# mmacklin/tinsel

Hardware: AMD Instinct MI355X
Metric: Msamples/s (cornell.tin 1024x1024 maxDepth=4 spp=2126, wavefront path; Mrays/s alongside) (higher is better)
Workload: dtype f32; 1 GPU; cornell.tin 1024x1024 maxDepth=4, 1 pass(es) per step, pipeline=auto; scene_pack=tests/golden/cornell.pack, parallelism=1 GPU

## Files before the change

include/tinsel_hip.h:

```cpp
#ifndef TINSEL_HIP_H
#define TINSEL_HIP_H

#include <stddef.h>
#include <stdint.h>

#ifdef __cplusplus
extern "C" {
#endif


typedef struct tinsel_vec3 { float x, y, z; } tinsel_vec3;
typedef struct tinsel_vec4 { float x, y, z, w; } tinsel_vec4;

typedef struct tinsel_transform {
    tinsel_vec3 p;
    tinsel_vec4 r;
    float s;
} tinsel_transform;

typedef struct tinsel_bvh_node {
    tinsel_vec3 lower;
    tinsel_vec3 upper;
    uint32_t left_index;
    uint32_t right_index_leaf;
} tinsel_bvh_node;

typedef struct tinsel_camera {
    tinsel_vec3 position;
    tinsel_vec4 rotation;
    float fov;
    float shutter_start;
    float shutter_end;
} tinsel_camera;

typedef struct tinsel_texture {
    float* data;
    int32_t width, height, depth;
    int32_t _pad;
} tinsel_texture;

typedef struct tinsel_material {
    tinsel_vec3 emission;
    tinsel_vec3 color;
    tinsel_vec3 absorption;
    float eta;
    float metallic;
    float subsurface;
    float specular;
    float roughness;
    float specular_tint;
    float anisotropic;
    float sheen;
    float sheen_tint;
    float clearcoat;
    float clearcoat_gloss;
    float transmission;
    int32_t _pad0;
    tinsel_texture bump_map;
    float bump;
    tinsel_vec3 bump_tile;
} tinsel_material;

enum { TINSEL_GEOM_SPHERE = 0, TINSEL_GEOM_PLANE = 1, TINSEL_GEOM_MESH = 2 };

typedef struct tinsel_mesh_geometry {
    const tinsel_vec3* positions;
    const tinsel_vec3* normals;
    const int32_t* indices;
    const tinsel_bvh_node* nodes;
    const float* cdf;
    int32_t num_vertices;
    int32_t num_indices;
    int32_t num_nodes;
    float area;
    uint64_t id;
} tinsel_mesh_geometry;

typedef struct tinsel_primitive {
    tinsel_transform start_transform;
    tinsel_transform end_transform;
    int32_t type;
    int32_t _pad0;
    union {
        struct { float radius; } sphere;
        struct { float plane[4]; } plane;
        tinsel_mesh_geometry mesh;
    } geo;
    tinsel_material material;
    int32_t light_samples;
    int32_t _pad1;
} tinsel_primitive;

enum { TINSEL_FILTER_BOX = 0, TINSEL_FILTER_GAUSSIAN = 1 };

typedef struct tinsel_filter {
    int32_t type;
    float width;
    float falloff;
    float offset;
} tinsel_filter;

enum { TINSEL_MODE_NORMALS = 0, TINSEL_MODE_COMPLEXITY = 1, TINSEL_MODE_PATHTRACE = 2 };

typedef struct tinsel_options {
    int32_t mode;
    int32_t width;
    int32_t height;
    tinsel_filter filter;
    float exposure;
    float limit;
    float clamp;
    int32_t max_depth;
    int32_t max_samples;
} tinsel_options;

typedef struct tinsel_scene_desc {
    const tinsel_primitive* primitives;
    int32_t num_primitives;
    int32_t num_bvh_nodes;
    const tinsel_bvh_node* bvh_nodes;
    tinsel_vec3 sky_horizon;
    tinsel_vec3 sky_zenith;
    int32_t probe_valid;
    int32_t probe_width;
    int32_t probe_height;
    int32_t _pad;
    const tinsel_vec4* probe_data;
    const float* probe_pdf_x;
    const float* probe_cdf_x;
    const float* probe_pdf_y;
    const float* probe_cdf_y;
} tinsel_scene_desc;


typedef struct tinsel_hip tinsel_hip;

enum { TINSEL_PIPELINE_WAVEFRONT = 0, TINSEL_PIPELINE_MEGAKERNEL = 1, TINSEL_PIPELINE_WAVEFRONT_SPLIT = 2,
       TINSEL_PIPELINE_WAVEFRONT_PAIRED = 4,
       TINSEL_PIPELINE_AUTO = 3 };

tinsel_hip* tinsel_hip_create(const tinsel_scene_desc* scene, int device_index);

typedef struct tinsel_hip_tuning {
    uint32_t struct_bytes;
    int32_t flat_scan;
    int32_t lds_scene;
    int32_t walk;
    int32_t inline_max_tris;
    int32_t walk_min_tris;
    int64_t small_mesh_bytes;
    int64_t arena_lds_limit;
    int64_t batch_paths;
    int32_t grid_mult;
    int32_t bounce_share;
    int32_t repack;
    int32_t tail_split;
    float tail_share;
    int32_t tail_divide;
    int32_t shade_sorted;
    int32_t overlap;
    int32_t scene_walk;
    int32_t swalk_lds;
    int32_t accumulate;
    int32_t walk_block;
    int32_t walk_single;
    int32_t walk_lds_stack;
    int32_t walk_refill_min;
    int32_t walk_leaf_min;
    int32_t walk_grid_mult;
    int32_t quads_in_scan;
    int32_t bounce_fit;
} tinsel_hip_tuning;
enum { TINSEL_ACCUMULATE_AUTO = 0, TINSEL_ACCUMULATE_TILED = 1, TINSEL_ACCUMULATE_WIDE = 2, TINSEL_ACCUMULATE_PIPED = 3, TINSEL_ACCUMULATE_FULL_WINDOW = 4 };

void tinsel_hip_tuning_init(tinsel_hip_tuning* t);
tinsel_hip* tinsel_hip_create_tuned(const tinsel_scene_desc* scene, int device_index, const tinsel_hip_tuning* tuning);
int tinsel_hip_set_tuning(tinsel_hip* r, const tinsel_hip_tuning* tuning);
int tinsel_hip_get_tuning(tinsel_hip* r, tinsel_hip_tuning* out);

void tinsel_hip_destroy(tinsel_hip* r);

int tinsel_hip_init(tinsel_hip* r, int width, int height);

int tinsel_hip_init_external(tinsel_hip* r, int width, int height, float* device_accum);

int tinsel_hip_render(tinsel_hip* r, const tinsel_camera* camera, const tinsel_options* options,
                      float* out_rgba, int passes);

enum { TINSEL_LOOKAHEAD_OFF = 0, TINSEL_LOOKAHEAD_ON = 1, TINSEL_LOOKAHEAD_PIN_OUTPUT = 2 };
int tinsel_hip_set_lookahead(tinsel_hip* r, int enable);

int tinsel_hip_render_async(tinsel_hip* r, const tinsel_camera* camera, const tinsel_options* options,
                            int passes, void* stream);

float* tinsel_hip_accum_device_ptr(tinsel_hip* r);

int tinsel_hip_read_accum(tinsel_hip* r, float* out_rgba);

enum { TINSEL_BVH_REFERENCE = 0, TINSEL_BVH_LBVH = 1, TINSEL_BVH_PLOC = 2 };
int tinsel_hip_set_mesh_bvh(tinsel_hip* r, int mode, double* build_ms);

int tinsel_hip_refit_mesh(tinsel_hip* r, int primitive, const float* positions_xyz, int num_vertices, const float* normals_xyz);

enum { TINSEL_SCENE_BVH_NODES = 0, TINSEL_SCENE_BVH_DEVICE = 1 };
int tinsel_hip_set_primitive_transform(tinsel_hip* r, int index, const tinsel_transform* start, const tinsel_transform* end);
int tinsel_hip_rebuild_scene(tinsel_hip* r, int mode, const tinsel_bvh_node* nodes, int num_nodes, double* build_ms);

enum { TINSEL_PROBE_CDF = 0, TINSEL_PROBE_ALIAS = 1 };
int tinsel_hip_set_probe_sampling(tinsel_hip* r, int mode);

int tinsel_hip_set_russian_roulette(tinsel_hip* r, int start_bounce);

int tinsel_hip_write_accum(tinsel_hip* r, const float* rgba, uint32_t next_pass_index);

int tinsel_hip_present(tinsel_hip* r, const tinsel_options* options, int nlm_width, float nlm_falloff, float* out_rgba);
int tinsel_hip_present_async(tinsel_hip* r, const tinsel_options* options, int nlm_width, float nlm_falloff, void* stream);
const float* tinsel_hip_present_device_ptr(tinsel_hip* r);

int tinsel_image_quantize_rgb8(const float* rgba, int width, int height, unsigned char* rgb);

int tinsel_hip_set_shard(tinsel_hip* r, int rank, int world, int tile);

int tinsel_hip_set_pipeline(tinsel_hip* r, int pipeline);

enum { TINSEL_ARITH_EXACT = 0, TINSEL_ARITH_FAST = 1 };
int tinsel_hip_set_arithmetic(tinsel_hip* r, int mode);
int tinsel_hip_get_arithmetic(tinsel_hip* r);

int tinsel_hip_set_pass_index(tinsel_hip* r, uint32_t pass_index);
uint32_t tinsel_hip_get_pass_index(tinsel_hip* r);

void tinsel_hip_stats(tinsel_hip* r, unsigned long long* rays, unsigned long long* samples,
                      double* gpu_seconds);
void tinsel_hip_reset_stats(tinsel_hip* r);

typedef struct tinsel_kernel_time {
    char name[32];
    uint32_t launches;
    float total_ms;
    float busy_ms;
} tinsel_kernel_time;
int tinsel_hip_kernel_times(tinsel_hip* r, tinsel_kernel_time* out, int max_entries);
int tinsel_hip_kernel_time_bytes(void);
int tinsel_hip_enable_kernel_timing(tinsel_hip* r, int enable);

int tinsel_hip_stats_detail(tinsel_hip* r, unsigned long long* out8);
int tinsel_hip_set_detail_counters(tinsel_hip* r, int enable);

int tinsel_hip_render_cost(tinsel_hip* r, const tinsel_camera* camera, const tinsel_options* options,
                           uint32_t pass_begin, int passes, uint32_t* out_host);

#define TINSEL_FEATURE_ALBEDO 1u
#define TINSEL_FEATURE_NORMAL 2u
#define TINSEL_FEATURE_DEPTH  4u

int tinsel_hip_render_features(tinsel_hip* r, const tinsel_camera* camera, const tinsel_options* options,
                               uint32_t pass_begin, int passes, unsigned features, float* out_host);
int tinsel_hip_render_features_device(tinsel_hip* r, const tinsel_camera* camera, const tinsel_options* options,
                                      uint32_t pass_begin, int passes, unsigned features, float* out_dev, void* stream);

#define TINSEL_ID_MISS   (-1)
#define TINSEL_ID_EMPTY  (-2)
#define TINSEL_ID_MAX_SLOTS 8

int tinsel_hip_render_id_mattes(tinsel_hip* r, const tinsel_camera* camera, const tinsel_options* options,
                                uint32_t pass_begin, int passes, int slots, int32_t* out_ids_host, float* out_weights_host);
int tinsel_hip_render_id_mattes_device(tinsel_hip* r, const tinsel_camera* camera, const tinsel_options* options,
                                       uint32_t pass_begin, int passes, int slots, int32_t* out_ids_dev, float* out_weights_dev, void* stream);

#define TINSEL_MAX_LIGHT_GROUPS 8

int tinsel_hip_render_light_groups(tinsel_hip* r, const tinsel_camera* camera, const tinsel_options* options,
                                   uint32_t pass_begin, int passes, int num_groups, const int32_t* group_of_primitive, int env_group,
                                   float* out_host);
int tinsel_hip_render_light_groups_device(tinsel_hip* r, const tinsel_camera* camera, const tinsel_options* options,
                                          uint32_t pass_begin, int passes, int num_groups, const int32_t* group_of_primitive, int env_group,
                                          float* out_dev, void* stream);

typedef struct tinsel_hip_denoise_params {
    int radius;
    int patch_radius;
    float k_color, k_albedo, k_normal, k_depth;
    int demodulate;
    float albedo_floor;
} tinsel_hip_denoise_params;

void tinsel_hip_denoise_params_init(tinsel_hip_denoise_params* p);

int tinsel_hip_denoise(tinsel_hip* r, const float* beauty_host, const float* planes_host,
                       unsigned features, int width, int height,
                       const tinsel_hip_denoise_params* p, float* out_host);
int tinsel_hip_denoise_device(tinsel_hip* r, const float* beauty_dev, const float* planes_dev,
                              unsigned features, int width, int height,
                              const tinsel_hip_denoise_params* p, float* out_dev, void* stream);

int tinsel_hip_present_image_device(tinsel_hip* r, const float* image_dev,
                                    const tinsel_options* options, int nlm_width,
                                    float nlm_falloff, void* stream);

typedef struct tinsel_ray     { float ox, oy, oz, time;  float dx, dy, dz, tmax; } tinsel_ray;
typedef struct tinsel_ray_hit { float t; int32_t primitive; float nx, ny, nz; uint32_t reserved[3]; } tinsel_ray_hit;

#define TINSEL_QUERY_CLOSEST  0
#define TINSEL_QUERY_OCCLUDED 1

int tinsel_hip_trace_rays(tinsel_hip* r, int mode, long long n, const tinsel_ray* rays_host, void* out_host);
int tinsel_hip_trace_rays_device(tinsel_hip* r, int mode, long long n, const tinsel_ray* rays_dev, void* out_dev, void* stream);
int tinsel_hip_trace_camera(tinsel_hip* r, const tinsel_camera* camera, int width, int height, float time, tinsel_ray_hit* out_host);

typedef struct tinsel_path_start { float ox, oy, oz, time;  float dx, dy, dz, reserved0;  uint32_t rng1, rng2, reserved1, reserved2; } tinsel_path_start;

int tinsel_hip_trace_radiance(tinsel_hip* r, long long n, const tinsel_path_start* starts_host, int max_depth, float* out_rgbx_host);
int tinsel_hip_trace_radiance_device(tinsel_hip* r, long long n, const tinsel_path_start* starts_dev, int max_depth, float* out_rgbx_dev, void* stream);

typedef struct tinsel_gather_point { float px, py, pz, time;  float nx, ny, nz;  uint32_t seed; } tinsel_gather_point;

#define TINSEL_GATHER_COSINE 0
#define TINSEL_GATHER_SPHERE 1

int tinsel_hip_gather_radiance(tinsel_hip* r, int mode, long long n, const tinsel_gather_point* points_host, int samples, int max_depth,
                               float* out_rgbx_host, tinsel_path_start* starts_out_host );
int tinsel_hip_gather_radiance_device(tinsel_hip* r, int mode, long long n, const tinsel_gather_point* points_dev, int samples, int max_depth,
                                      float* out_rgbx_dev, tinsel_path_start* starts_out_dev , void* stream);

#define TINSEL_GATHER_SH_MAX_ORDER 2

int tinsel_hip_gather_sh(tinsel_hip* r, int mode, int order, long long n, const tinsel_gather_point* points_host,
                         int samples, int max_depth, float* out_host, tinsel_path_start* starts_out_host );
int tinsel_hip_gather_sh_device(tinsel_hip* r, int mode, int order, long long n, const tinsel_gather_point* points_dev,
                                int samples, int max_depth, float* out_dev, tinsel_path_start* starts_out_dev , void* stream);

int tinsel_hip_reserve(tinsel_hip* r, int passes, int max_depth);

int tinsel_hip_set_batch_paths(tinsel_hip* r, unsigned long long max_paths);

long long tinsel_hip_read_batch_radiance(tinsel_hip* r, float* out_rgbx, unsigned long long max_paths);

int tinsel_hip_leaf(tinsel_hip* r, int op, int index, int n, const float* in, int in_stride, const uint32_t* seeds,
                    float* out, int out_stride, const tinsel_camera* camera, int width, int height);

int tinsel_hip_mesh_tree(tinsel_hip* r, int primitive, void* out_nodes, int capacity, int* out_meta);

int tinsel_hip_stack_entries(tinsel_hip* r);
int tinsel_hip_nee_per_path(tinsel_hip* r);
int tinsel_hip_walked_prims(tinsel_hip* r);
int tinsel_hip_walk_tops(tinsel_hip* r, int* out_counts, int capacity);
int tinsel_hip_queue_counts(tinsel_hip* r, uint32_t* out, int max_bounces);
int tinsel_hip_bounce_plan(tinsel_hip* r, uint32_t* out2);
unsigned int tinsel_hip_scene_features(const tinsel_scene_desc* scene);
int tinsel_hip_scene_slim(const tinsel_scene_desc* scene);
enum { TINSEL_BOUNCE_MEDIA = 1, TINSEL_BOUNCE_PROBE = 2, TINSEL_BOUNCE_MOTION = 4, TINSEL_BOUNCE_MESH_WALK = 8, TINSEL_BOUNCE_SPHERE = 16,
       TINSEL_BOUNCE_TRANSMISSION = 32, TINSEL_BOUNCE_POOLS = 64, TINSEL_BOUNCE_SHARE = 128, TINSEL_BOUNCE_SORT = 256, TINSEL_BOUNCE_ROULETTE = 512 };

const char* tinsel_hip_last_error(void);


typedef struct tinsel_hip_group tinsel_hip_group;

tinsel_hip_group* tinsel_hip_group_create(const tinsel_scene_desc* scene, int num_gpus, int tile);
tinsel_hip_group* tinsel_hip_group_create_tuned(const tinsel_scene_desc* scene, int num_gpus, int tile, const tinsel_hip_tuning* tuning);
void tinsel_hip_group_destroy(tinsel_hip_group* g);
int tinsel_hip_group_init(tinsel_hip_group* g, int width, int height);
int tinsel_hip_group_render(tinsel_hip_group* g, const tinsel_camera* camera, const tinsel_options* options, float* out_rgba, int passes);
int tinsel_hip_group_set_lookahead(tinsel_hip_group* g, int enable);
int tinsel_hip_group_present(tinsel_hip_group* g, const tinsel_options* options, int nlm_width, float nlm_falloff, float* out_rgba);
int tinsel_hip_group_size(tinsel_hip_group* g);
tinsel_hip* tinsel_hip_group_member(tinsel_hip_group* g, int rank);

#define TINSEL_HIP_COMM_ID_BYTES 128
int tinsel_hip_comm_unique_id(unsigned char* id_bytes, int capacity);
int tinsel_hip_comm_init(tinsel_hip* r, const unsigned char* id_bytes, int rank, int world);
int tinsel_hip_comm_size(tinsel_hip* r);
int tinsel_hip_comm_reduce_accum(tinsel_hip* r, float* out_device, int root, void* stream);

int tinsel_hip_plan_regions(unsigned long long slots, int num_cus, int nee_per_path, int fused, unsigned int* out);

int tinsel_hip_selftest_arith(int device_index, int op, int variant, unsigned long long* out_counts, unsigned int* out_first_bad);
int tinsel_hip_selftest_sort(int device_index, unsigned long long* keys, unsigned long long n, int begin_bit, int end_bit);
int tinsel_hip_selftest_scan(int device_index, const int* in, int* out, unsigned long long n);
int tinsel_hip_accumulate_support(int filter_type, float filter_width, float filter_falloff, float filter_offset, float* out_arg_zero);
int tinsel_hip_selftest_accumulate(int device_index, int width, int height, int filter_type, float filter_width, float filter_falloff, float filter_offset,
                                   float clamp, const unsigned int* pass_seeds, int passes, const float* radiance, float* accum, int choice, int form,
                                   int* out_form);

int tinsel_hip_ubench(int device_index, int kind, unsigned long long bytes, int steps, double* out_ms, double* out_units);


#define TINSEL_PACK_MAGIC "TINPACK1"

typedef struct tinsel_pack_header {
    char magic[8];
    uint32_t version;
    uint32_t num_primitives;
    uint32_t num_bvh_nodes;
    uint32_t num_meshes;
    uint64_t total_bytes;
    uint64_t off_primitives;
    uint64_t off_bvh_nodes;
    uint64_t off_probe_data;
    uint64_t off_probe_pdf_x;
    uint64_t off_probe_cdf_x;
    uint64_t off_probe_pdf_y;
    uint64_t off_probe_cdf_y;
    int32_t probe_width;
    int32_t probe_height;
    tinsel_vec3 sky_horizon;
    tinsel_vec3 sky_zenith;
    tinsel_camera camera;
    tinsel_options options;
    uint8_t _reserved[48];
} tinsel_pack_header;

int tinsel_pack_open(void* blob, size_t size, tinsel_scene_desc* out_scene,
                     tinsel_camera* out_camera, tinsel_options* out_options);

#ifdef __cplusplus
}

static_assert(sizeof(tinsel_vec3) == 12, "Vec3");
static_assert(sizeof(tinsel_transform) == 32, "Transform");
static_assert(sizeof(tinsel_bvh_node) == 32, "BVHNode");
static_assert(sizeof(tinsel_camera) == 40, "Camera");
static_assert(sizeof(tinsel_texture) == 24, "Texture");
static_assert(sizeof(tinsel_material) == 128, "Material");
static_assert(offsetof(tinsel_material, eta) == 36, "Material.eta");
static_assert(offsetof(tinsel_material, transmission) == 80, "Material.transmission");
static_assert(offsetof(tinsel_material, bump_map) == 88, "Material.bumpMap");
static_assert(offsetof(tinsel_material, bump) == 112, "Material.bump");
static_assert(sizeof(tinsel_mesh_geometry) == 64, "MeshGeometry");
static_assert(offsetof(tinsel_mesh_geometry, num_vertices) == 40, "MeshGeometry.numVertices");
static_assert(offsetof(tinsel_mesh_geometry, area) == 52, "MeshGeometry.area");
static_assert(offsetof(tinsel_mesh_geometry, id) == 56, "MeshGeometry.id");
static_assert(sizeof(tinsel_primitive) == 272, "Primitive");
static_assert(offsetof(tinsel_primitive, type) == 64, "Primitive.type");
static_assert(offsetof(tinsel_primitive, geo) == 72, "Primitive.geo");
static_assert(offsetof(tinsel_primitive, material) == 136, "Primitive.material");
static_assert(offsetof(tinsel_primitive, light_samples) == 264, "Primitive.lightSamples");
static_assert(sizeof(tinsel_filter) == 16, "Filter");
static_assert(sizeof(tinsel_options) == 48, "Options");
static_assert(offsetof(tinsel_options, max_depth) == 40, "Options.maxDepth");
static_assert(sizeof(tinsel_pack_header) == 256, "pack header");
static_assert(sizeof(tinsel_hip_tuning) == 128, "tuning");
static_assert(sizeof(tinsel_ray) == 32, "ray");
static_assert(sizeof(tinsel_ray_hit) == 32, "ray hit");
static_assert(sizeof(tinsel_path_start) == 48, "path start");
static_assert(sizeof(tinsel_gather_point) == 32, "gather point");
#endif

#endif
```

tinsel_amd/abi.py:

```python
import ctypes as C


class Vec3(C.Structure):
    _fields_ = [("x", C.c_float), ("y", C.c_float), ("z", C.c_float)]

    def __iter__(self):
        return iter((self.x, self.y, self.z))


class Vec4(C.Structure):
    _fields_ = [("x", C.c_float), ("y", C.c_float), ("z", C.c_float), ("w", C.c_float)]

    def __iter__(self):
        return iter((self.x, self.y, self.z, self.w))


class Transform(C.Structure):
    _fields_ = [("p", Vec3), ("r", Vec4), ("s", C.c_float)]


class BVHNode(C.Structure):
    _fields_ = [("lower", Vec3), ("upper", Vec3), ("left_index", C.c_uint32), ("right_index_leaf", C.c_uint32)]


# ... 3 lines not shown


LEAF_BIT = 0x80000000
MESH_TREE_META = ("root", "numInternal", "numTris", "stackNeed", "topCount", "twoLeaves", "inArena")


class Camera(C.Structure):
    _fields_ = [("position", Vec3), ("rotation", Vec4), ("fov", C.c_float),
                ("shutter_start", C.c_float), ("shutter_end", C.c_float)]


class Texture(C.Structure):
    _fields_ = [("data", C.c_void_p), ("width", C.c_int32), ("height", C.c_int32),
                ("depth", C.c_int32), ("_pad", C.c_int32)]


class Material(C.Structure):
    _fields_ = [("emission", Vec3), ("color", Vec3), ("absorption", Vec3),
                ("eta", C.c_float), ("metallic", C.c_float), ("subsurface", C.c_float),
                ("specular", C.c_float), ("roughness", C.c_float), ("specular_tint", C.c_float),
                ("anisotropic", C.c_float), ("sheen", C.c_float), ("sheen_tint", C.c_float),
                ("clearcoat", C.c_float), ("clearcoat_gloss", C.c_float), ("transmission", C.c_float),
                ("_pad0", C.c_int32), ("bump_map", Texture), ("bump", C.c_float), ("bump_tile", Vec3)]


class MeshGeometry(C.Structure):
    _fields_ = [("positions", C.c_void_p), ("normals", C.c_void_p), ("indices", C.c_void_p),
                ("nodes", C.c_void_p), ("cdf", C.c_void_p),
                ("num_vertices", C.c_int32), ("num_indices", C.c_int32), ("num_nodes", C.c_int32),
                ("area", C.c_float), ("id", C.c_uint64)]


class _Sphere(C.Structure):
    _fields_ = [("radius", C.c_float)]


class _Plane(C.Structure):
    _fields_ = [("plane", C.c_float * 4)]


class _Geo(C.Union):
    _fields_ = [("sphere", _Sphere), ("plane", _Plane), ("mesh", MeshGeometry)]


class Primitive(C.Structure):
    _fields_ = [("start_transform", Transform), ("end_transform", Transform),
                ("type", C.c_int32), ("_pad0", C.c_int32), ("geo", _Geo),
                ("material", Material), ("light_samples", C.c_int32), ("_pad1", C.c_int32)]


class Filter(C.Structure):
    _fields_ = [("type", C.c_int32), ("width", C.c_float), ("falloff", C.c_float), ("offset", C.c_float)]


class Options(C.Structure):
    _fields_ = [("mode", C.c_int32), ("width", C.c_int32), ("height", C.c_int32), ("filter", Filter),
                ("exposure", C.c_float), ("limit", C.c_float), ("clamp", C.c_float),
                ("max_depth", C.c_int32), ("max_samples", C.c_int32)]

    def copy(self):
        o = Options()
        C.memmove(C.byref(o), C.byref(self), C.sizeof(Options))
        return o


class SceneDesc(C.Structure):
    _fields_ = [("primitives", C.c_void_p), ("num_primitives", C.c_int32), ("num_bvh_nodes", C.c_int32),
                ("bvh_nodes", C.c_void_p), ("sky_horizon", Vec3), ("sky_zenith", Vec3),
                ("probe_valid", C.c_int32), ("probe_width", C.c_int32), ("probe_height", C.c_int32),
                ("_pad", C.c_int32), ("probe_data", C.c_void_p), ("probe_pdf_x", C.c_void_p),
                ("probe_cdf_x", C.c_void_p), ("probe_pdf_y", C.c_void_p), ("probe_cdf_y", C.c_void_p)]


class PackHeader(C.Structure):
    _fields_ = [("magic", C.c_char * 8), ("version", C.c_uint32), ("num_primitives", C.c_uint32),
                ("num_bvh_nodes", C.c_uint32), ("num_meshes", C.c_uint32), ("total_bytes", C.c_uint64),
                ("off_primitives", C.c_uint64), ("off_bvh_nodes", C.c_uint64), ("off_probe_data", C.c_uint64),
                ("off_probe_pdf_x", C.c_uint64), ("off_probe_cdf_x", C.c_uint64),
                ("off_probe_pdf_y", C.c_uint64), ("off_probe_cdf_y", C.c_uint64),
                ("probe_width", C.c_int32), ("probe_height", C.c_int32),
                ("sky_horizon", Vec3), ("sky_zenith", Vec3), ("camera", Camera), ("options", Options),
                ("_reserved", C.c_uint8 * 48)]


class KernelTime(C.Structure):
    _fields_ = [("name", C.c_char * 32), ("launches", C.c_uint32), ("total_ms", C.c_float), ("busy_ms", C.c_float)]


class Ray(C.Structure):
    _fields_ = [("ox", C.c_float), ("oy", C.c_float), ("oz", C.c_float), ("time", C.c_float),
                ("dx", C.c_float), ("dy", C.c_float), ("dz", C.c_float), ("tmax", C.c_float)]


class RayHit(C.Structure):
    _fields_ = [("t", C.c_float), ("primitive", C.c_int32), ("nx", C.c_float), ("ny", C.c_float), ("nz", C.c_float),
                ("reserved", C.c_uint32 * 3)]


RAY_DTYPE = [("ox", "<f4"), ("oy", "<f4"), ("oz", "<f4"), ("time", "<f4"), ("dx", "<f4"), ("dy", "<f4"), ("dz", "<f4"), ("tmax", "<f4")]
RAY_HIT_DTYPE = [("t", "<f4"), ("primitive", "<i4"), ("nx", "<f4"), ("ny", "<f4"), ("nz", "<f4"), ("reserved", "<u4", (3,))]
QUERY_CLOSEST, QUERY_OCCLUDED = 0, 1


class PathStart(C.Structure):
    _fields_ = [("ox", C.c_float), ("oy", C.c_float), ("oz", C.c_float), ("time", C.c_float),
                ("dx", C.c_float), ("dy", C.c_float), ("dz", C.c_float), ("reserved0", C.c_float),
                ("rng1", C.c_uint32), ("rng2", C.c_uint32), ("reserved1", C.c_uint32), ("reserved2", C.c_uint32)]


PATH_START_DTYPE = [("ox", "<f4"), ("oy", "<f4"), ("oz", "<f4"), ("time", "<f4"), ("dx", "<f4"), ("dy", "<f4"), ("dz", "<f4"), ("reserved0", "<f4"),
                    ("rng1", "<u4"), ("rng2", "<u4"), ("reserved1", "<u4"), ("reserved2", "<u4")]


class GatherPoint(C.Structure):
    _fields_ = [("px", C.c_float), ("py", C.c_float), ("pz", C.c_float), ("time", C.c_float),
                ("nx", C.c_float), ("ny", C.c_float), ("nz", C.c_float), ("seed", C.c_uint32)]


GATHER_POINT_DTYPE = [("px", "<f4"), ("py", "<f4"), ("pz", "<f4"), ("time", "<f4"), ("nx", "<f4"), ("ny", "<f4"), ("nz", "<f4"), ("seed", "<u4")]
GATHER_COSINE, GATHER_SPHERE = 0, 1
GATHER_SH_MAX_ORDER = 2
FEATURE_ALBEDO, FEATURE_NORMAL, FEATURE_DEPTH = 1, 2, 4
FEATURE_NAMES = ("albedo", "normal", "depth")
ID_MISS, ID_EMPTY, ID_MAX_SLOTS = -1, -2, 8
MAX_LIGHT_GROUPS = 8


class DenoiseParams(C.Structure):
    _fields_ = [("radius", C.c_int32), ("patch_radius", C.c_int32),
                ("k_color", C.c_float), ("k_albedo", C.c_float), ("k_normal", C.c_float), ("k_depth", C.c_float),
                ("demodulate", C.c_int32), ("albedo_floor", C.c_float)]

    def as_dict(self):
        return {k: getattr(self, k) for k, _ in self._fields_}


class KernelTimeV1(C.Structure):
    _fields_ = [("name", C.c_char * 32), ("launches", C.c_uint32), ("total_ms", C.c_float)]


BOUNCE_GENERAL, BOUNCE_COUNT, BOUNCE_FIT_CLOSED, BOUNCE_FIT_DEFERRED = 0, 1, 2, 3
BOUNCE_MEDIA, BOUNCE_PROBE, BOUNCE_MOTION, BOUNCE_MESH_WALK, BOUNCE_SPHERE = 1, 2, 4, 8, 16
BOUNCE_TRANSMISSION, BOUNCE_POOLS, BOUNCE_SHARE, BOUNCE_SORT, BOUNCE_ROULETTE = 32, 64, 128, 256, 512


class Tuning(C.Structure):
    _fields_ = [("struct_bytes", C.c_uint32),
                ("flat_scan", C.c_int32), ("lds_scene", C.c_int32), ("walk", C.c_int32), ("inline_max_tris", C.c_int32), ("walk_min_tris", C.c_int32),
                ("small_mesh_bytes", C.c_int64), ("arena_lds_limit", C.c_int64),
                ("batch_paths", C.c_int64), ("grid_mult", C.c_int32), ("bounce_share", C.c_int32), ("repack", C.c_int32),
                ("tail_split", C.c_int32), ("tail_share", C.c_float), ("tail_divide", C.c_int32),
                ("shade_sorted", C.c_int32), ("overlap", C.c_int32), ("scene_walk", C.c_int32), ("swalk_lds", C.c_int32), ("accumulate", C.c_int32),
                ("walk_block", C.c_int32), ("walk_single", C.c_int32), ("walk_lds_stack", C.c_int32), ("walk_refill_min", C.c_int32), ("walk_leaf_min", C.c_int32),
                ("walk_grid_mult", C.c_int32), ("quads_in_scan", C.c_int32), ("bounce_fit", C.c_int32)]
    CREATE_FIELDS = ("flat_scan", "lds_scene", "walk", "inline_max_tris", "walk_min_tris", "small_mesh_bytes", "arena_lds_limit")
    _DEFAULTS = dict(flat_scan=-1, lds_scene=-1, walk=-1, inline_max_tris=-1, walk_min_tris=-1, small_mesh_bytes=-1, arena_lds_limit=-1,
                     batch_paths=0, grid_mult=0, bounce_share=-1, repack=-1, tail_split=-1, tail_share=0.0, tail_divide=4,
                     shade_sorted=-1, overlap=-1, scene_walk=-1, swalk_lds=-1, accumulate=0,
                     walk_block=0, walk_single=-1, walk_lds_stack=-1, walk_refill_min=0, walk_leaf_min=0, walk_grid_mult=0, quads_in_scan=-1, bounce_fit=-1)

    def __init__(self, **over):
        super().__init__()
        self.struct_bytes = C.sizeof(Tuning)
        for k, v in self._DEFAULTS.items():
            setattr(self, k, v)
        for k, v in over.items():
            if k not in self._DEFAULTS:
                raise TypeError("tinsel_hip_tuning has no field %r" % k)
            setattr(self, k, v)

    def replace(self, **over):
        t = Tuning(**{k: getattr(self, k) for k in self._DEFAULTS})
        for k, v in over.items():
            if k not in self._DEFAULTS:
                raise TypeError("tinsel_hip_tuning has no field %r" % k)
            setattr(t, k, v)
        return t

    def as_dict(self):
        return {k: getattr(self, k) for k in self._DEFAULTS}


ACCUMULATE_AUTO, ACCUMULATE_TILED, ACCUMULATE_WIDE, ACCUMULATE_PIPED, ACCUMULATE_FULL_WINDOW = 0, 1, 2, 3, 4
ACCUMULATE_FORM_AUTO, ACCUMULATE_FORM_FULL_WINDOW, ACCUMULATE_FORM_SUPPORT = 0, 1, 2
ACCUMULATE_RAN_UNTILED, ACCUMULATE_RAN_TILED, ACCUMULATE_RAN_WIDE, ACCUMULATE_RAN_PIPED, ACCUMULATE_RAN_SUPPORT_TILED, ACCUMULATE_RAN_SUPPORT_WIDE = 0, 1, 2, 3, 4, 5
SELFTEST_ACCUMULATE_ARGTYPES = [C.c_int, C.c_int, C.c_int, C.c_int, C.c_float, C.c_float, C.c_float, C.c_float, C.c_void_p, C.c_int, C.c_void_p, C.c_void_p,
                                C.c_int, C.c_int, C.POINTER(C.c_int)]


def accumulate_arg_zero(offset):
    import math
    import numpy as np
    z = math.log(float(np.float32(offset))) - 1e-6
    f = np.float32(z)
    if float(f) > z:
        f = np.nextafter(f, np.float32(-np.inf))
    return f


def accumulate_takes_support_form(filter_type, width, falloff, offset):
    import numpy as np
    width, falloff, offset = np.float32(width), np.float32(falloff), np.float32(offset)
    if filter_type == FILTER_BOX or not (offset > 0 and np.isfinite(offset)) or not (falloff > 0 and np.isfinite(falloff)) or not (0 < width <= 1):
        return False
    return bool(-falloff <= accumulate_arg_zero(offset))
COMM_ID_BYTES = 128
MODE_NORMALS, MODE_COMPLEXITY, MODE_PATHTRACE = 0, 1, 2
BVH_REFERENCE, BVH_LBVH, BVH_PLOC = 0, 1, 2
SCENE_BVH_NODES, SCENE_BVH_DEVICE = 0, 1
ARITH_EXACT, ARITH_FAST = 0, 1
PROBE_CDF, PROBE_ALIAS = 0, 1
LOOKAHEAD_OFF, LOOKAHEAD_ON, LOOKAHEAD_PIN_OUTPUT = 0, 1, 2
FILTER_BOX, FILTER_GAUSSIAN = 0, 1
GEOM_SPHERE, GEOM_PLANE, GEOM_MESH = 0, 1, 2
PIPELINE_WAVEFRONT, PIPELINE_MEGAKERNEL, PIPELINE_WAVEFRONT_SPLIT, PIPELINE_AUTO, PIPELINE_WAVEFRONT_PAIRED = 0, 1, 2, 3, 4

assert C.sizeof(Transform) == 32 and C.sizeof(BVHNode) == 32 and C.sizeof(Camera) == 40 and C.sizeof(Node64) == 64
assert C.sizeof(Material) == 128 and C.sizeof(MeshGeometry) == 64 and C.sizeof(Primitive) == 272
assert C.sizeof(Filter) == 16 and C.sizeof(Options) == 48 and C.sizeof(PackHeader) == 256
assert C.sizeof(Ray) == 32 and C.sizeof(RayHit) == 32 and C.sizeof(DenoiseParams) == 32
assert Primitive.geo.offset == 72 and Primitive.material.offset == 136 and Primitive.light_samples.offset == 264
```

tinsel_amd/csrc/tn_host_api.h:

```cpp
#pragma once

extern "C" {

int tinsel_hip_init(tinsel_hip* r, int width, int height)
{
    if (r)
        lookahead_release(r);
    if (!r || width <= 0 || height <= 0)
        return fail("init: bad arguments");
    HIP_TRY(hipSetDevice(r->device));
    HIP_TRY(hipDeviceSynchronize());
    r->accum = nullptr;
    if (r->accumOwn.alloc((size_t)width*height))
        return -1;
    r->accum = r->accumOwn.get();
    HIP_TRY(hipMemset(r->accum, 0, sizeof(float4)*(size_t)width*height));
    HIP_TRY(hipStreamSynchronize(nullptr));
    r->width = width;
    r->height = height;
    return 0;
}

int tinsel_hip_init_external(tinsel_hip* r, int width, int height, float* device_accum)
{
// ... 563 lines not shown
    return 0;
}

void tinsel_hip_stats(tinsel_hip* r, unsigned long long* rays, unsigned long long* samples, double* gpu_seconds)
{
    unsigned long long s[8] = { 0 };
    if (r && r->statsDev)
        (void)read_stats(r, s);
    if (rays) *rays = s[0];
    if (samples) *samples = s[1];
    if (gpu_seconds) *gpu_seconds = r ? r->gpuSeconds : 0.0;
}

int tinsel_hip_stats_detail(tinsel_hip* r, unsigned long long* out8)
{
    if (!r || !out8)
        return fail("stats_detail: bad arguments");
    return read_stats(r, out8);
}

int tinsel_hip_set_detail_counters(tinsel_hip* r, int enable)
{
    lookahead_cancel(r);
    if (!r)
        return fail("set_detail_counters: null");
    r->countDetail = enable != 0;
    return 0;
}

void tinsel_hip_reset_stats(tinsel_hip* r)
{
    lookahead_cancel(r);
    if (!r)
        return;
    (void)hipSetDevice(r->device);
    (void)hipDeviceSynchronize();
    (void)hipMemset(r->statsDev.get(), 0, sizeof(unsigned long long)*kStatShards*kStatWords);
    (void)hipStreamSynchronize(nullptr);
    r->gpuSeconds = 0.0;
}

int tinsel_hip_enable_kernel_timing(tinsel_hip* r, int enable)
{
    lookahead_cancel(r);
    if (!r)
        return fail("enable_kernel_timing: null");
    r->timing = enable != 0;
    return 0;
}

int tinsel_hip_kernel_time_bytes(void) { return (int)sizeof(tinsel_kernel_time); }

int tinsel_hip_kernel_times(tinsel_hip* r, tinsel_kernel_time* out, int max_entries)
{
    lookahead_cancel(r);
    if (!r || !out)
        return fail("kernel_times: bad arguments");
    HIP_TRY(hipSetDevice(r->device));
    HIP_TRY(hipDeviceSynchronize());
    float total[KN_COUNT] = { 0 };
    uint32_t launches[KN_COUNT] = { 0 };
    std::vector<std::pair<float, float>> intervals[KN_COUNT];
    for (const TimedSpan& s : r->spans)
    {
        float ms = 0.0f, at = 0.0f;
        if (hipEventElapsedTime(&ms, s.start, s.stop) == hipSuccess)
        {
            total[s.kernel] += ms;
            launches[s.kernel]++;
            if (hipEventElapsedTime(&at, r->spans.front().start, s.start) == hipSuccess)
                intervals[s.kernel].push_back(std::make_pair(at, at + ms));
        }
    }
    float busy[KN_COUNT] = { 0 };
    for (int k = 0; k < KN_COUNT; ++k)
    {
        std::sort(intervals[k].begin(), intervals[k].end());
        float end = -1e30f;
        for (const auto& iv : intervals[k])
        {
            if (iv.second > end)
                busy[k] += iv.second - std::max(iv.first, end);
            end = std::max(end, iv.second);
        }
        if (intervals[k].size() != launches[k])
            busy[k] = total[k];
    }
    int n = 0;
    double sum = 0.0;
    for (int k = 0; k < KN_COUNT && n < max_entries; ++k)
    {
        if (!launches[k])
            continue;
        memset(&out[n], 0, sizeof(out[n]));
        strncpy(out[n].name, kKernelNames[k], sizeof(out[n].name) - 1);
        out[n].launches = launches[k];
        out[n].total_ms = total[k];
        out[n].busy_ms = busy[k];
        sum += total[k];
        ++n;
    }
    r->gpuSeconds += sum*1e-3;
    return n;
}

int tinsel_hip_reserve(tinsel_hip* r, int passes, int max_depth)
{
    lookahead_cancel(r);
    if (!r || !r->accum || passes < 1 || max_depth < 1)
        return fail("reserve: bad arguments (Init first)");
    HIP_TRY(hipSetDevice(r->device));
    const size_t perPass = slots_per_pass(r, r->width, r->height);
    return ensure_batch(r, plan_batch(r, perPass, passes_per_batch(batch_slots(r), perPass, passes),  false), max_depth);
}

int tinsel_hip_set_batch_paths(tinsel_hip* r, unsigned long long max_paths)
{
    lookahead_cancel(r);
    if (!r || max_paths < 1024)
        return fail("set_batch_paths: bad arguments");
    r->maxBatchSlots = (size_t)max_paths;
    r->batchSlotsExplicit = true;
    r->tune.batch_paths = (int64_t)max_paths;
    return 0;
}

int tinsel_hip_set_tuning(tinsel_hip* r, const tinsel_hip_tuning* tuning)
{
    if (!r || !tuning)
        return fail("set_tuning: null argument");
    lookahead_cancel(r);
    tinsel_hip_tuning t = tuning_from_caller(tuning);
    if (t.grid_mult < 0 || t.grid_mult > 256 || (t.walk_block != 0 && t.walk_block != 256 && t.walk_block != 1024) ||
        t.accumulate < TINSEL_ACCUMULATE_AUTO || t.accumulate > TINSEL_ACCUMULATE_FULL_WINDOW || t.walk_refill_min > 64 || t.walk_leaf_min > 64 || t.walk_grid_mult < 0 || t.walk_grid_mult > 64 ||
        (t.tail_split > 0 && (!(t.tail_share >= 0.0f) || t.tail_divide < 1)) || (t.batch_paths != 0 && t.batch_paths < 1024))
        return fail("set_tuning: a field is out of range");
    HIP_TRY(hipSetDevice(r->device));
    HIP_TRY(hipDeviceSynchronize());
    const tinsel_hip_tuning was = r->tune;
    t.flat_scan = was.flat_scan; t.lds_scene = was.lds_scene; t.walk = was.walk; t.inline_max_tris = was.inline_max_tris;
    t.walk_min_tris = was.walk_min_tris; t.small_mesh_bytes = was.small_mesh_bytes; t.arena_lds_limit = was.arena_lds_limit;
    r->tune = t;
    if (t.batch_paths > 0)
    {
        r->maxBatchSlots = (size_t)t.batch_paths;
        r->batchSlotsExplicit = true;
    }
    else
    {
        r->maxBatchSlots = 8u << 20;
        r->batchSlotsExplicit = false;
    }
    free_batch(r);
    return 0;
}

int tinsel_hip_get_tuning(tinsel_hip* r, tinsel_hip_tuning* out)
{
    if (!r || !out)
        return fail("get_tuning: null argument");
    *out = r->tune;
    return 0;
}

long long tinsel_hip_read_batch_radiance(tinsel_hip* r, float* out_rgbx, unsigned long long max_paths)
{
    lookahead_cancel(r);
    if (!r || !out_rgbx)
        return fail("read_batch_radiance: bad arguments");
    HIP_TRY(hipSetDevice(r->device));
    HIP_TRY(hipDeviceSynchronize());
    const size_t n = std::min<size_t>((size_t)max_paths, r->lastBatchSlots);
    if (n)
        HIP_TRY(hipMemcpy(out_rgbx, r->ps.rad, sizeof(float4)*n, hipMemcpyDeviceToHost));
    return (long long)n;
}

int tinsel_hip_leaf(tinsel_hip* r, int op, int index, int n, const float* in, int in_stride, const uint32_t* seeds,
                    float* out, int out_stride, const tinsel_camera* camera, int width, int height)
{
    lookahead_cancel(r);
    if (!r || n <= 0 || !out || out_stride <= 0 || op < 0 || op > kLeafDisplay)
        return fail("leaf: bad arguments");
    if ((op == kLeafBsdfEval || op == kLeafBsdfSample || op == kLeafPrimIntersect || op == kLeafPrimSample) &&
        (index < 0 || index >= r->scene.numPrims))
        return fail("leaf: primitive index out of range");
    HIP_TRY(hipSetDevice(r->device));
    DevBuf<float> dIn, dOut;
    DevBuf<uint32_t> dSeeds;
    CameraParams cam;
    memset(&cam, 0, sizeof(cam));
    if (camera && width > 0 && height > 0)
        make_camera(*camera, width, height, cam);
    if (in && in_stride > 0 && dIn.upload(in, (size_t)n*in_stride))
        return fail("leaf: input upload failed");
    if (seeds && dSeeds.upload(seeds, (size_t)n))
        return fail("leaf: seed upload failed");
    if (dOut.alloc((size_t)n*out_stride))
        return fail("leaf: output allocation failed");
    hipLaunchKernelGGL(k_leaf, dim3((n + kBlock - 1)/kBlock), dim3(kBlock), stack_bytes(r), nullptr, r->scene, op, index, n, dIn.get(), in_stride,
                       dSeeds.get(), dOut.get(), out_stride, cam, r->stackNeed);
    if (hipDeviceSynchronize() != hipSuccess || hipGetLastError() != hipSuccess)
        return fail("leaf: kernel failed");
    if (hipMemcpy(out, dOut.get(), sizeof(float)*(size_t)n*out_stride, hipMemcpyDeviceToHost) != hipSuccess)
        return fail("leaf: download failed");
    return 0;
}

int tinsel_hip_stack_entries(tinsel_hip* r) { return r ? r->stackNeed : 0; }

int tinsel_hip_mesh_tree(tinsel_hip* r, int primitive, void* out_nodes, int capacity, int* out_meta)
{
    lookahead_cancel(r);
    if (!r || !out_meta || capacity < 0 || primitive < 0 || primitive >= r->scene.numPrims || r->primMesh[(size_t)primitive] < 0)
        return fail("mesh_tree: bad arguments (a mesh primitive and a meta array of 7 ints)");
    const DevMesh& dm = r->meshesNow[(size_t)r->primMesh[(size_t)primitive]];
    const int meta[7] = { (int)dm.root, dm.numInternal, dm.numTris, dm.stackNeed, dm.topCount, dm.twoLeaves, dm.inArena };
    memcpy(out_meta, meta, sizeof(meta));
    if (!out_nodes)
        return dm.numInternal;
    if (capacity < dm.numInternal)
        return fail("mesh_tree: capacity is smaller than the tree's node count");
    const unsigned char* src = dm.inArena ? r->scene.arena + dm.offNodes : reinterpret_cast<const unsigned char*>(dm.nodes);
    HIP_TRY(hipSetDevice(r->device));
    HIP_TRY(hipDeviceSynchronize());
    if (dm.numInternal > 0)
        HIP_TRY(hipMemcpy(out_nodes, src, sizeof(Node64)*(size_t)dm.numInternal, hipMemcpyDeviceToHost));
    return dm.numInternal;
}
int tinsel_hip_walked_prims(tinsel_hip* r) { return (r && r->walkEnabled) ? r->walkPrims.count : 0; }
int tinsel_hip_nee_per_path(tinsel_hip* r) { return r ? r->neePerPath : 0; }

int tinsel_hip_walk_tops(tinsel_hip* r, int* out_counts, int capacity)
{
    if (!r || !out_counts || capacity < 0)
        return fail("walk_tops: bad arguments");
    const int n = r->walkEnabled ? r->walkPrims.count : 0;
    if (capacity < n)
        return fail("walk_tops: capacity is smaller than the number of walked primitives");
    const WalkPlan w = plan_walk(r);
    for (int k = 0; k < n; ++k)
        out_counts[k] = w.job.topCount[k];
    return n;
}

unsigned int tinsel_hip_scene_features(const tinsel_scene_desc* scene)
{
    if (!scene || !scene->primitives)
        return 0u;
    uint32_t f = scene->probe_valid ? kFeatProbe : 0u;
    for (int i = 0; i < scene->num_primitives; ++i)
    {
        const tinsel_primitive& p = scene->primitives[i];
        const tinsel_material& m = p.material;
        f |= (m.absorption.x != 0.0f || m.absorption.y != 0.0f || m.absorption.z != 0.0f) ? kFeatMedia : 0u;
        f |= m.transmission != 0.0f ? kFeatTransmission : 0u;
        f |= memcmp(&p.start_transform, &p.end_transform, sizeof(tinsel_transform)) != 0 ? kFeatMotion : 0u;
        f |= p.type == TINSEL_GEOM_SPHERE ? kFeatSphere : 0u;
        if (p.type == TINSEL_GEOM_MESH)
        {
            const tinsel_bvh_node* n = p.geo.mesh.nodes;
            const bool twoLeaves = n && p.geo.mesh.num_nodes == 3 && !ref_is_leaf(n[0]) && n[0].left_index < 3u && ref_right(n[0]) < 3u &&
                                   ref_is_leaf(n[n[0].left_index]) && ref_is_leaf(n[ref_right(n[0])]);
            f |= twoLeaves ? 0u : kFeatMeshWalk;
        }
    }
    return f;
}

int tinsel_hip_scene_slim(const tinsel_scene_desc* scene)
{
    if (!scene || !scene->primitives)
        return 0;
    bool anySubsurface = false;
    for (int i = 0; i < scene->num_primitives; ++i)
        anySubsurface = anySubsurface || !is_plus_zero(scene->primitives[i].material.subsurface);
    return scene_slim(tinsel_hip_scene_features(scene), anySubsurface) ? 1 : 0;
}

int tinsel_hip_bounce_plan(tinsel_hip* r, uint32_t* out2)
{
    if (!r || !out2)
        return fail("bounce_plan: bad arguments");
    if (r->lastBounceKind < 0)
        return fail("bounce_plan: the fused kernel has not run yet");
    out2[0] = (uint32_t)r->lastBounceKind;
    out2[1] = r->lastBounceFeatures;
    return 0;
}

int tinsel_hip_queue_counts(tinsel_hip* r, uint32_t* out, int max_bounces)
{
    if (!r || !out || max_bounces < 1)
        return fail("queue_counts: bad arguments");
    if (r->batchPipeline < 0 || r->batchDepth < 1)
        return fail("queue_counts: nothing rendered yet");
    HIP_TRY(hipSetDevice(r->device));
    HIP_TRY(hipDeviceSynchronize());
    const int n = std::min(max_bounces, std::min(r->batchDepth, r->lastFp.maxDepth));
    if (r->lastPipeline == TINSEL_PIPELINE_MEGAKERNEL || r->batchPipeline != r->lastPipeline)
        return fail("queue_counts: the last batch did not run a wavefront pipeline");
    const tinsel_hip::DenseLane& lane = r->lane[r->lastLane];
    const bool split = r->lastPipeline == TINSEL_PIPELINE_WAVEFRONT_SPLIT && r->neePerPath > 0;
    const size_t W = lane.regions;
    std::vector<uint32_t> seg(W*(size_t)n*4, 0u);
    uint32_t* const src[4] = { lane.ss.segFront, lane.ss.segBack, lane.ss.neeFront, lane.ss.neeBack };
    for (int a = 0; a < (split ? 4 : 2); ++a)
        HIP_TRY(hipMemcpy(seg.data() + (size_t)a*W*n, src[a], W*(size_t)n*sizeof(uint32_t), hipMemcpyDeviceToHost));
    for (int b = 0; b < n; ++b)
    {
        unsigned long long live = 0, nee = 0;
        for (size_t g = 0; g < W; ++g)
        {
            live += seg[(size_t)b*W + g] + seg[W*n + (size_t)b*W + g];
            nee += seg[2*W*n + (size_t)b*W + g] + seg[3*W*n + (size_t)b*W + g];
        }
        out[b] = (b == 0 && r->lastPipeline == TINSEL_PIPELINE_WAVEFRONT) ? lane.paths : (uint32_t)live;
        out[max_bounces + b] = (uint32_t)nee;
    }
    return n;
}


int tinsel_hip_plan_regions(unsigned long long slots, int num_cus, int nee_per_path, int fused, unsigned int* out)
{
    if (!out || slots == 0 || slots >= 0xffffffffull || num_cus < 1 || num_cus > 4096)
        return fail("plan_regions: bad arguments");
    RegionSpec s = region_spec(tuning_defaults(), num_cus, nee_per_path, fused != 0, kBounceWaves);
    s.capacity = (size_t)slots + s.maxRegions*kWave;
    RegionCut c;
    const int rc = cut_regions(s, (size_t)slots, streaming_grid(s, (size_t)slots), c) ? 0 : fail("render: path buffers too small for this batch");
    out[0] = c.numRegions; out[1] = c.regionLen; out[2] = c.bigRegions; out[3] = c.shortLen;
    out[4] = (unsigned int)c.grid(); out[5] = (unsigned int)s.maxRegions;
    return rc;
}

int tinsel_hip_selftest_arith(int device_index, int op, int variant, unsigned long long* out_counts, unsigned int* out_first_bad)
{
    if (!out_counts || !out_first_bad || op < 0 || op > 2)
        return fail("selftest_arith: bad arguments");
    if (variant < 0)
        variant = op == 0 ? kRcpVariant : op == 1 ? kSqrtVariant : kRsqrtVariant;
    HIP_TRY(hipSetDevice(device_index));
    DevBuf<unsigned long long> countsDev;
    DevBuf<uint32_t> firstDev;
    if (countsDev.alloc(260))
        return -1;
    if (firstDev.alloc(1))
        return fail("selftest_arith: allocation failed");
    unsigned long long* const counts = countsDev.get();
    uint32_t* const first = firstDev.get();
    (void)hipMemset(counts, 0, 260*sizeof(unsigned long long));
    (void)hipMemset(first, 0xff, sizeof(uint32_t));
    bool known = true;
    switch (op*100 + variant)
    {
    case 0: launch_selftest_arith<0, 0>(counts, first); break;
    case 1: launch_selftest_arith<0, 1>(counts, first); break;
    case 11: launch_selftest_arith<0, 11>(counts, first); break;
    case 100: launch_selftest_arith<1, 0>(counts, first); break;
    case 101: launch_selftest_arith<1, 1>(counts, first); break;
    case 111: launch_selftest_arith<1, 11>(counts, first); break;
    case 121: launch_selftest_arith<1, 21>(counts, first); break;
    case 200: launch_selftest_arith<2, 0>(counts, first); break;
    case 201: launch_selftest_arith<2, 1>(counts, first); break;
    case 202: launch_selftest_arith<2, 2>(counts, first); break;
    case 203: launch_selftest_arith<2, 3>(counts, first); break;
    default: known = false; break;
    }
    if (!known)
        return fail("selftest_arith: unknown variant");
    if (hipDeviceSynchronize() != hipSuccess || hipGetLastError() != hipSuccess ||
             hipMemcpy(out_counts, counts, 260*sizeof(unsigned long long), hipMemcpyDeviceToHost) != hipSuccess ||
             hipMemcpy(out_first_bad, first, sizeof(uint32_t), hipMemcpyDeviceToHost) != hipSuccess)
        return fail("selftest_arith: kernel failed");
    return 0;
}

int tinsel_hip_selftest_sort(int device_index, unsigned long long* keys, unsigned long long n, int begin_bit, int end_bit)
{
    if (!keys || n == 0 || n >= (1ull << 31) || begin_bit < 0 || end_bit > 64 || begin_bit >= end_bit || (begin_bit & 7) || (end_bit & 7))
        return fail("selftest_sort: bad arguments");
    HIP_TRY(hipSetDevice(device_index));
    DevBuf<unsigned long long> a, b;
    DevBuf<int> scratch;
    if (a.alloc((size_t)n) || b.alloc((size_t)n) || scratch.alloc(sort_scratch_ints((size_t)n)))
        return fail("selftest_sort: allocation failed");
    if (hipMemcpy(a.get(), keys, n*8, hipMemcpyHostToDevice) != hipSuccess)
        return fail("selftest_sort: upload failed");
    radix_sort_keys(a.get(), b.get(), (size_t)n, begin_bit, end_bit, scratch.get(), nullptr);
    if (hipDeviceSynchronize() != hipSuccess || hipGetLastError() != hipSuccess || hipMemcpy(keys, b.get(), n*8, hipMemcpyDeviceToHost) != hipSuccess)
        return fail("selftest_sort: kernels failed");
    return 0;
}

int tinsel_hip_selftest_scan(int device_index, const int* in, int* out, unsigned long long n)
{
    if (!in || !out || n == 0 || n >= (1ull << 31))
        return fail("selftest_scan: bad arguments");
    HIP_TRY(hipSetDevice(device_index));
    DevBuf<int> a, scratch;
    if (a.alloc((size_t)n) || scratch.alloc(scan_scratch_ints((size_t)n)))
        return fail("selftest_scan: allocation failed");
    if (hipMemcpy(a.get(), in, n*sizeof(int), hipMemcpyHostToDevice) != hipSuccess)
        return fail("selftest_scan: upload failed");
    exclusive_scan(a.get(), a.get(), (size_t)n, scratch.get(), nullptr);
    if (hipDeviceSynchronize() != hipSuccess || hipGetLastError() != hipSuccess || hipMemcpy(out, a.get(), n*sizeof(int), hipMemcpyDeviceToHost) != hipSuccess)
        return fail("selftest_scan: kernels failed");
    return 0;
}

int tinsel_hip_accumulate_support(int filter_type, float filter_width, float filter_falloff, float filter_offset, float* out_arg_zero)
{
    float z = 0.0f;
    const bool takes = accumulate_support_rule(filter_type, filter_width, filter_falloff, filter_offset, &z);
    if (out_arg_zero)
        *out_arg_zero = z;
    return takes ? 1 : 0;
}

// ... 208 lines not shown
```

tinsel_amd/csrc/tn_host_create.h:

```cpp
#pragma once

namespace {

void comm_release(tinsel_hip* r);


struct SceneBuild
{
    tinsel_hip* r;
    DevScene& sc;
    const tinsel_scene_desc* desc;
    const tinsel_hip_tuning& tune;
    int P;
    std::vector<Prim64> prims;
    std::vector<Mat128> mats;
    std::vector<Moving64> moving;
    std::vector<DevMesh> meshes;
    std::vector<int32_t> lights;
    std::map<uint64_t, uint32_t> meshIndex;
    ArenaBuilder arena;
    int maxMeshNeed = 0;
    int totalLightSamples = 0;
    bool sceneHasBigMesh = false;
    SceneLevel lvl;
// ... 25 lines not shown
    void mark_walked_and_quads();
    int assemble_arena();
    void set_scene_flags();
    int upload_probe();
    int stats_and_fit();
};

void create_limits(tinsel_hip* r, int device_index, const tinsel_hip_tuning* tuning)
{
    r->device = device_index;
    r->tune = tuning_from_caller(tuning);
    hipDeviceProp_t prop;
    if (hipGetDeviceProperties(&prop, device_index) == hipSuccess)
    {
        r->numCUs = prop.multiProcessorCount;
        r->sharedMemLimit = (int)prop.sharedMemPerBlock;
    }
    prepare_kernels_once(r);
    if (!r->prepRefused.empty() && r->sharedMemLimit > 65536)
    {
        fprintf(stderr, "tinsel_hip: the runtime refused %d B of dynamic LDS for %s: planning within 65536 B per workgroup\n", r->sharedMemLimit, r->prepRefused.c_str());
        r->sharedMemLimit = 65536;
        r->segPrefixLds = std::min(r->segPrefixLds, 65536 - 1024);
    }

    if (r->tune.batch_paths >= 65536)
    {
        r->maxBatchSlots = (size_t)r->tune.batch_paths;
        r->batchSlotsExplicit = true;
    }
}

int SceneBuild::add_mesh(const tinsel_mesh_geometry& g, Prim64& o)
{
    const int numTris = g.num_indices/3;
    if (numTris <= 0 || !g.positions || !g.normals || !g.indices || !g.nodes || !g.cdf)
        return fail("create: mesh primitive with missing arrays");
    ConvertedBvh cb;
    if (!convert_bvh(g.nodes, g.num_nodes, numTris, lives_in_arena(mesh_bytes_estimate(g), numTris) ? 0 : kWalkTopNodes, cb))
        return fail("create: malformed mesh BVH");
    std::vector<Tri48> tris((size_t)numTris);
    for (int t = 0; t < numTris; ++t)
    {
        const int i0 = g.indices[t*3 + 0], i1 = g.indices[t*3 + 1], i2 = g.indices[t*3 + 2];
        if (i0 < 0 || i1 < 0 || i2 < 0 || i0 >= g.num_vertices || i1 >= g.num_vertices || i2 >= g.num_vertices)
            return fail("create: mesh index out of range");
        Tri48& T = tris[(size_t)t];
        T.ax = g.positions[i0].x; T.ay = g.positions[i0].y; T.az = g.positions[i0].z; T.i0 = i0;
        T.bx = g.positions[i1].x; T.by = g.positions[i1].y; T.bz = g.positions[i1].z; T.i1 = i1;
        T.cx = g.positions[i2].x; T.cy = g.positions[i2].y; T.cz = g.positions[i2].z; T.i2 = i2;
    }

    DevMesh dm;
    memset(&dm, 0, sizeof(dm));
    dm.root = cb.root;
    dm.numTris = numTris;
    dm.stackNeed = cb.maxLeafDepth + 1;
    dm.topCount = cb.topCount;
    dm.numInternal = (int32_t)cb.nodes.size();
    dm.twoLeaves = (cb.nodes.size() == 1 && !(cb.root & kLeafBit) && (cb.nodes[0].left & kLeafBit) && (cb.nodes[0].right & kLeafBit)) ? 1 : 0;
    const size_t meshBytes = cb.nodes.size()*sizeof(Node64) + tris.size()*sizeof(Tri48) + (size_t)g.num_vertices*12 + (size_t)numTris*4;
    if (lives_in_arena(meshBytes, numTris))
    {
        dm.inArena = 1;
        dm.offNodes = (uint32_t)arena.add(cb.nodes.data(), cb.nodes.size());
        dm.offTris = (uint32_t)arena.add(tris.data(), tris.size());
        dm.offNormals = (uint32_t)arena.add(&g.normals[0].x, (size_t)g.num_vertices*3);
        dm.offCdf = (uint32_t)arena.add(g.cdf, (size_t)numTris);
    }
    else
    {
        dm.nodes = r->sceneMem.upload(cb.nodes.data(), cb.nodes.size());
        dm.tris = r->sceneMem.upload(tris.data(), tris.size());
        dm.normals = r->sceneMem.upload(&g.normals[0].x, (size_t)g.num_vertices*3);
        dm.cdf = r->sceneMem.upload(g.cdf, (size_t)numTris);
        if ((!cb.nodes.empty() && !dm.nodes) || !dm.tris || !dm.normals || !dm.cdf)
            return fail("create: device allocation failed (mesh)");
    }
    if (dm.stackNeed > maxMeshNeed)
        maxMeshNeed = dm.stackNeed;
    r->meshNumVertices.push_back(g.num_vertices);
    r->meshIndices.emplace_back(g.indices, g.indices + (size_t)numTris*3);
    r->meshRootLo.push_back(V3(g.nodes[0].lower.x, g.nodes[0].lower.y, g.nodes[0].lower.z));
    r->meshRootHi.push_back(V3(g.nodes[0].upper.x, g.nodes[0].upper.y, g.nodes[0].upper.z));
    r->meshArea.push_back(g.area);
    o.mesh = (uint32_t)meshes.size();
    meshIndex[g.id] = o.mesh;
    meshes.push_back(dm);
    return 0;
}

int SceneBuild::add_primitives()
{
    for (int i = 0; i < P; ++i)
    {
        const tinsel_primitive& p = desc->primitives[i];
        Prim64& o = prims[(size_t)i];
        memset(&o, 0, sizeof(o));

        make_material(p, mats[(size_t)i]);
        r->primEndScale.push_back(p.end_transform.s);
        if (p.light_samples > 0)
        {
            if (p.type == TINSEL_GEOM_PLANE)
                return fail("create: a plane cannot be a light (PrimitiveSample asserts, intersection.h:871-875)");
            lights.push_back(i);
            totalLightSamples += p.light_samples;
        }

        const bool isStatic = memcmp(&p.start_transform, &p.end_transform, sizeof(tinsel_transform)) == 0;
        const Xform xs = to_xform(p.start_transform), xe = to_xform(p.end_transform);
        r->primStart.push_back(xs);
        r->primEnd.push_back(xe);
        set_prim_pose(o, xs, xe, isStatic);
        o.moving = (uint32_t)i;
        moving[(size_t)i] = make_moving(xs, xe);

        if (p.type == TINSEL_GEOM_SPHERE)
        {
            o.type = kPrimSphere;
            o.g0 = p.geo.sphere.radius;
        }
        else if (p.type == TINSEL_GEOM_PLANE)
        {
            o.type = kPrimPlane;
            o.g0 = p.geo.plane.plane[0]; o.g1 = p.geo.plane.plane[1]; o.g2 = p.geo.plane.plane[2]; o.g3 = p.geo.plane.plane[3];
        }
        else if (p.type == TINSEL_GEOM_MESH)
        {
            o.type = kPrimMesh;
            const tinsel_mesh_geometry& g = p.geo.mesh;
            auto it = meshIndex.find(g.id);
            if (it != meshIndex.end())
                o.mesh = it->second;
            else if (add_mesh(g, o))
                return -1;
        }
        else
            return fail("create: unknown primitive type");
    }
    r->primMesh.assign((size_t)P, -1);
    r->lightPrims = lights;
    for (int i = 0; i < P; ++i)
    {
        set_prim_derived(prims[(size_t)i]);
        if (prims[(size_t)i].type == kPrimMesh)
            r->primMesh[(size_t)i] = (int)prims[(size_t)i].mesh;
    }
    return 0;
}

int SceneBuild::scene_level()
{
    if (!build_scene_level(std::vector<tinsel_bvh_node>(desc->bvh_nodes, desc->bvh_nodes + desc->num_bvh_nodes), prims, {}, lvl))
        return fail("create: malformed scene BVH");
    const int need = lvl.bvh.maxLeafDepth + 1 + maxMeshNeed;
    r->stackNeed = pick_stack(need);
    if (r->stackNeed < 0)
        return fail("create: BVH too deep for the 156-entry LDS traversal stack");
    flatScan = lvl.everyPrimHasALeaf && P <= 64 && tune.flat_scan != 0;
    return 0;
}

void SceneBuild::mark_walked_and_quads()
{
    const int walkMinTris = tune.walk_min_tris >= 0 ? tune.walk_min_tris : kInlineMaxTris + 1;
    r->binPrims.count = 0;
    r->walkPrims.count = 0;
    if (flatScan)
        for (int k = 0; k < P && r->binPrims.count < 7; ++k)
            if (prims[(size_t)k].type == kPrimMesh && !meshes[prims[(size_t)k].mesh].inArena)
            {
                r->binPrims.prim[r->binPrims.count++] = k;
                if (meshes[prims[(size_t)k].mesh].numTris >= walkMinTris)
                {
                    prims[(size_t)k].flags |= kPrimWalked | ((uint32_t)r->walkPrims.count << kPrimWalkLaneShift);
                    r->walkPrimMesh[r->walkPrims.count] = (int)prims[(size_t)k].mesh;
                    r->walkPrims.prim[r->walkPrims.count++] = k;
                }
            }
    for (int k = 0; k < P; ++k)
        if (prims[(size_t)k].type == kPrimMesh && meshes[prims[(size_t)k].mesh].twoLeaves && meshes[prims[(size_t)k].mesh].inArena)
        {
            const DevMesh& qm = meshes[prims[(size_t)k].mesh];
            if (((qm.offNodes | qm.offTris | qm.offNormals | qm.offCdf) & 127u) != 0u || ((qm.offNodes | qm.offTris | qm.offNormals | qm.offCdf) >> 7) > 0xffffu)
                continue;
            Prim64& qp = prims[(size_t)k];
            qp.flags |= kPrimQuadArena;
            const uint32_t w0 = (qm.offNodes >> 7) | ((qm.offTris >> 7) << 16), w1 = (qm.offNormals >> 7) | ((qm.offCdf >> 7) << 16);
            memcpy(&qp.g0, &w0, 4); memcpy(&qp.g1, &w1, 4);
        }
    r->walkEnabled = tune.walk != 0;
#ifdef TN_WALK_PROF
    if (r->walkProf.alloc(16) == 0)
        (void)hipMemset(r->walkProf.get(), 0, 16*sizeof(unsigned long long));
#endif
}

int SceneBuild::assemble_arena()
{
    const size_t offNodes = arena.add(lvl.bvh.nodes.data(), lvl.bvh.nodes.size());
    const size_t offPrims = arena.add(prims.data(), prims.size());
    const size_t offMats = arena.add(mats.data(), mats.size());
    const size_t offMoving = arena.add(moving.data(), moving.size());
    std::vector<LightRec> lightRecs(lights.size());
    for (size_t l = 0; l < lights.size(); ++l)
        lightRecs[l] = { lights[l], mats[(size_t)lights[l]].lightSamples, mats[(size_t)lights[l]].rcpLightSamples, 0 };
    const size_t offLights = arena.add(lightRecs.data(), lightRecs.size());
    const size_t offMeshes = arena.add(meshes.data(), meshes.size());

    int alwaysHitPlanes = 0;
    bool anyMeshInHbm = false;
    for (int k = 0; k < P; ++k)
    {
        alwaysHitPlanes += (prims[(size_t)k].type == kPrimPlane && lvl.boxes[(size_t)k].alwaysHit) ? 1 : 0;
        anyMeshInHbm = anyMeshInHbm || (prims[(size_t)k].type == kPrimMesh && !meshes[prims[(size_t)k].mesh].inArena);
    }
    if (flatScan && (alwaysHitPlanes >= 4 || anyMeshInHbm))
    {
        for (int k = 0; k < P; ++k)
            if (prims[(size_t)k].type == kPrimPlane && lvl.boxes[(size_t)k].alwaysHit)
                r->planeTablePrims.push_back(k);
        mark_plane_table(lvl, prims, r->planeTablePrims);
    }
    std::vector<float> planeEq = lvl.planeEq;
    std::vector<int32_t> planeIdx = r->planeTablePrims;
    while (planeIdx.size() % 4)
    {
        planeEq.insert(planeEq.end(), { 0.0f, 0.0f, 0.0f, 0.0f });
        planeIdx.push_back(0);
    }
    const size_t offBoxes = arena.add(lvl.boxes.data(), lvl.boxes.size());
    const size_t offPlaneEq = arena.add(planeEq.data(), planeEq.size());
    const size_t offPlaneIdx = arena.add(planeIdx.data(), planeIdx.size());
    arena.bytes.resize((arena.bytes.size() + 127) & ~size_t(127), 0);

    unsigned char* arenaDev = r->sceneMem.upload(arena.bytes.data(), arena.bytes.size());
    if (!arenaDev)
        return fail("create: device allocation failed (scene arena)");
    DevMesh* hm = reinterpret_cast<DevMesh*>(&arena.bytes[offMeshes]);
    for (size_t m = 0; m < meshes.size(); ++m)
    {
        if (hm[m].inArena)
        {
            hm[m].nodes = reinterpret_cast<const Node64*>(arenaDev + hm[m].offNodes);
            hm[m].tris = reinterpret_cast<const Tri48*>(arenaDev + hm[m].offTris);
            hm[m].normals = reinterpret_cast<const float*>(arenaDev + hm[m].offNormals);
            hm[m].cdf = reinterpret_cast<const float*>(arenaDev + hm[m].offCdf);
        }
    }
    if (!meshes.empty() && hipMemcpy(arenaDev + offMeshes, hm, sizeof(DevMesh)*meshes.size(), hipMemcpyHostToDevice) != hipSuccess)
        return fail("create: device allocation failed (scene arena)");
    r->meshesRef.assign(hm, hm + meshes.size());
    r->meshesNow = r->meshesRef;

    sc.arena = arenaDev;
    sc.arenaBytes = (uint32_t)arena.bytes.size();
    const size_t ldsLimit = tune.arena_lds_limit >= 0 ? (size_t)tune.arena_lds_limit : kArenaLdsLimit;
    sc.arenaLdsBytes = (arena.bytes.size() <= ldsLimit && tune.lds_scene != 0) ? sc.arenaBytes : 0u;
    sc.nodes = reinterpret_cast<const Node64*>(arenaDev + offNodes);
    sc.prims = reinterpret_cast<const Prim64*>(arenaDev + offPrims);
    sc.mats = reinterpret_cast<const Mat128*>(arenaDev + offMats);
    sc.moving = reinterpret_cast<const Moving64*>(arenaDev + offMoving);
    sc.lights = reinterpret_cast<const LightRec*>(arenaDev + offLights);
    sc.meshes = reinterpret_cast<const DevMesh*>(arenaDev + offMeshes);
    sc.numMeshes = (int)meshes.size();
    sc.primBoxes = reinterpret_cast<const PrimBox*>(arenaDev + offBoxes);
    sc.planeEq = reinterpret_cast<const float4*>(arenaDev + offPlaneEq);
    sc.planeIdx = reinterpret_cast<const int32_t*>(arenaDev + offPlaneIdx);
    sc.numPlanes = (int32_t)r->planeTablePrims.size();
    adopt_scene_level(r, lvl);
    r->arenaOffNodes = offNodes;
    r->arenaOffBoxes = offBoxes;
    r->arenaOffPrims = offPrims;
    r->arenaOffMoving = offMoving;
    r->arenaOffMats = offMats;
    r->primsHost = prims;
    return 0;
}

void SceneBuild::set_scene_flags()
{
    sc.hasMedia = 0;
    for (const Mat128& mm : mats)
        if (mm.absorption[0] != 0.0f || mm.absorption[1] != 0.0f || mm.absorption[2] != 0.0f)
            sc.hasMedia = 1;
    r->anyTransmission = std::any_of(mats.begin(), mats.end(), [](const Mat128& mm) { return mm.transmission != 0.0f; });
    r->anySubsurface = std::any_of(mats.begin(), mats.end(), [](const Mat128& mm) { return !is_plus_zero(mm.subsurface); });
    sc.flatScan = flatScan ? 1 : 0;
    {
        int meshPrimCount = 0;
        for (int k = 0; k < P; ++k)
            meshPrimCount += prims[(size_t)k].type == kPrimMesh ? 1 : 0;
        sc.deferMeshes = (meshPrimCount >= 2) ? 1 : 0;
    }
    {
        int planes = 0;
        for (int k = 0; k < P; ++k)
            planes += lvl.boxes[(size_t)k].alwaysHit ? 1 : 0;
        sc.sortQueues = (sc.flatScan && planes <= 2 && planes < P) ? 1 : 0;
    }
    for (int i = 0; i < P && !r->sceneEnclosed; ++i)
        for (int j = i + 1; j < P && !r->sceneEnclosed; ++j)
            if (prims[(size_t)i].type == kPrimPlane && prims[(size_t)j].type == kPrimPlane)
            {
                const Prim64 &a = prims[(size_t)i], &b = prims[(size_t)j];
                const float d = a.g0*b.g0 + a.g1*b.g1 + a.g2*b.g2;
                const float la = sqrtf(a.g0*a.g0 + a.g1*a.g1 + a.g2*a.g2), lb = sqrtf(b.g0*b.g0 + b.g1*b.g1 + b.g2*b.g2);
                r->sceneEnclosed = la > 0.0f && lb > 0.0f && d < -0.99f*la*lb;
            }
    bool all = sc.arenaLdsBytes != 0;
    for (const DevMesh& dmesh : meshes)
        all = all && dmesh.inArena;
    sc.allInArena = all ? 1 : 0;
    sc.numPrims = P;
    sc.numLights = (int)lights.size();
    sc.horizon[0] = desc->sky_horizon.x; sc.horizon[1] = desc->sky_horizon.y; sc.horizon[2] = desc->sky_horizon.z;
    sc.zenith[0] = desc->sky_zenith.x; sc.zenith[1] = desc->sky_zenith.y; sc.zenith[2] = desc->sky_zenith.z;
}

int SceneBuild::upload_probe()
{
    const size_t n = (size_t)desc->probe_width*desc->probe_height;
    if (!desc->probe_data || !desc->probe_pdf_x || !desc->probe_cdf_x || !desc->probe_pdf_y || !desc->probe_cdf_y || n == 0)
        return fail("create: probe marked valid but arrays missing");
    sc.probe.data = (const float4*)r->sceneMem.upload((const float*)desc->probe_data, n*4);
    sc.probe.pdfX = r->sceneMem.upload(desc->probe_pdf_x, n);
    sc.probe.cdfX = r->sceneMem.upload(desc->probe_cdf_x, n);
    sc.probe.pdfY = r->sceneMem.upload(desc->probe_pdf_y, (size_t)desc->probe_height);
    sc.probe.cdfY = r->sceneMem.upload(desc->probe_cdf_y, (size_t)desc->probe_height);
    sc.probe.width = desc->probe_width;
    sc.probe.height = desc->probe_height;
    sc.probe.valid = 1;
    if (!sc.probe.data || !sc.probe.pdfX || !sc.probe.cdfX || !sc.probe.pdfY || !sc.probe.cdfY)
        return fail("create: device allocation failed (probe)");
    return 0;
}

int SceneBuild::stats_and_fit()
{
    r->neePerPath = totalLightSamples + (r->scene.probe.valid ? 1 : 0);
    r->scene.totalLightSamples = r->neePerPath;
    if (r->statsDev.alloc((size_t)kStatShards*kStatWords) ||
        hipMemset(r->statsDev.get(), 0, sizeof(unsigned long long)*kStatShards*kStatWords) != hipSuccess)
        return fail("create: device allocation failed (stats)");
    if (stack_bytes(r) > (size_t)r->sharedMemLimit && r->scene.arenaLdsBytes)
    {
        r->scene.arenaLdsBytes = 0;
        r->scene.allInArena = 0;
    }
    if (stack_bytes(r) > (size_t)r->sharedMemLimit)
        return fail("create: the traversal stacks of this scene need " + std::to_string(stack_bytes(r)) + " B of LDS per workgroup, the device offers " + std::to_string(r->sharedMemLimit));
    return 0;
}

}

extern "C" {


const char* tinsel_hip_last_error(void) { return g_error.c_str(); }

void tinsel_hip_tuning_init(tinsel_hip_tuning* t)
{
    if (t)
        *t = tuning_defaults();
}

tinsel_hip* tinsel_hip_create(const tinsel_scene_desc* desc, int device_index) { return tinsel_hip_create_tuned(desc, device_index, nullptr); }

tinsel_hip* tinsel_hip_create_tuned(const tinsel_scene_desc* desc, int device_index, const tinsel_hip_tuning* tuning)
{
    if (!desc || !desc->primitives || desc->num_primitives <= 0 || !desc->bvh_nodes || desc->num_bvh_nodes <= 0)
    {
        fail("create: empty scene (Scene::Build must have run)");
        return nullptr;
    }

    int ndev = 0;
    if (hipGetDeviceCount(&ndev) != hipSuccess || ndev <= 0)
    {
        fail("create: no HIP device visible -- this library has no CPU fallback");
        return nullptr;
    }
    if (device_index < 0 || device_index >= ndev)
    {
        fail("create: bad device index");
        return nullptr;
    }
    HIP_TRY_NULL(hipSetDevice(device_index));

    std::unique_ptr<tinsel_hip> r(new tinsel_hip());
    create_limits(r.get(), device_index, tuning);
    memset(&r->scene, 0, sizeof(r->scene));
    SceneBuild b(r.get(), desc);
    if (b.add_primitives() || b.scene_level())
        return nullptr;
    b.mark_walked_and_quads();
    if (b.assemble_arena())
        return nullptr;
    b.set_scene_flags();
    if ((desc->probe_valid && b.upload_probe()) || b.stats_and_fit())
        return nullptr;
    return r.release();
}

void tinsel_hip_destroy(tinsel_hip* r)
{
    if (!r)
        return;
    (void)hipSetDevice(r->device);
    lookahead_release(r);
    (void)hipDeviceSynchronize();
    comm_release(r);
    if (r->walkProf)
    {
        unsigned long long wp[16] = { 0 };
        (void)hipMemcpy(wp, r->walkProf.get(), sizeof(wp), hipMemcpyDeviceToHost);
        const double tot = (double)(wp[0] + wp[1] + wp[2] + wp[3] + wp[4]);
        fprintf(stderr, "k_walk profile: cycles refill %.1f%% node %.1f%% tri %.1f%% pop %.1f%% loop %.1f%% | iterations %llu refills %llu node-phases %llu tri-phases %llu | "
                "lanes/node-phase %.1f lanes/tri-phase %.1f lanes/refill %.1f | waves %llu cycles/wave %.0f cycles/iteration %.0f cycles/refill %.0f cycles/node-phase %.0f cycles/tri-phase %.0f\n",
                100.0*wp[0]/tot, 100.0*wp[1]/tot, 100.0*wp[2]/tot, 100.0*wp[3]/tot, 100.0*wp[4]/tot, wp[5], wp[6], wp[7], wp[8],
                (double)wp[9]/std::max(1ull, wp[7]), (double)wp[10]/std::max(1ull, wp[8]), (double)wp[11]/std::max(1ull, wp[6]),
// ... 8 lines not shown
```

tinsel_amd/csrc/tn_host_scene.h:

```cpp
#pragma once

namespace {

void primitive_bounds(const tinsel_hip* r, int i, V3& lower, V3& upper)
{
    const Prim64& p = r->primsHost[(size_t)i];
    V3 lo, hi;
    if (p.type == kPrimSphere)      { lo = V3(-p.g0); hi = V3(p.g0); }
    else if (p.type == kPrimPlane)  { lo = V3(-1.e+8f); hi = V3(1.e+8f); }
    else                            { lo = r->meshRootLo[(size_t)r->primMesh[(size_t)i]]; hi = r->meshRootHi[(size_t)r->primMesh[(size_t)i]]; }
    V3 sl, su, el, eu;
    transform_bounds(r->primStart[(size_t)i], lo, hi, sl, su);
    transform_bounds(r->primEnd[(size_t)i], lo, hi, el, eu);
    lower = V3(minT(sl.x, el.x), minT(sl.y, el.y), minT(sl.z, el.z));
    upper = V3(maxT(su.x, eu.x), maxT(su.y, eu.y), maxT(su.z, eu.z));
}

void node64_to_reference(const std::vector<Node64>& nodes, uint32_t ref, float lminx, float lminy, float lminz, float lmaxx, float lmaxy, float lmaxz,
                         std::vector<tinsel_bvh_node>& out, uint32_t at)
{
    tinsel_bvh_node& me = out[at];
    me.lower.x = lminx; me.lower.y = lminy; me.lower.z = lminz;
    me.upper.x = lmaxx; me.upper.y = lmaxy; me.upper.z = lmaxz;
    if (ref & kLeafBit)
    {
        me.left_index = ref & ~kLeafBit;
        me.right_index_leaf = 0x80000000u;
        return;
    }
    const Node64 n = nodes[ref];
    const uint32_t l = (uint32_t)out.size();
    out.push_back(tinsel_bvh_node());
    out.push_back(tinsel_bvh_node());
    out[at].left_index = l;
    out[at].right_index_leaf = l + 1u;
    node64_to_reference(nodes, n.left, n.lminx, n.lminy, n.lminz, n.lmaxx, n.lmaxy, n.lmaxz, out, l);
    node64_to_reference(nodes, n.right, n.rminx, n.rminy, n.rminz, n.rmaxx, n.rmaxy, n.rmaxz, out, l + 1u);
}

void union_ancestors(std::vector<tinsel_bvh_node>& tree)
{
    std::vector<uint32_t> order, stack(1, 0u);
    while (!stack.empty())
    {
        const uint32_t k = stack.back();
        stack.pop_back();
        order.push_back(k);
        if (!ref_is_leaf(tree[k]))
        {
            stack.push_back(tree[k].left_index);
            stack.push_back(ref_right(tree[k]));
        }
    }
    for (size_t q = order.size(); q-- > 0; )
    {
        tinsel_bvh_node& n = tree[order[q]];
        if (ref_is_leaf(n))
            continue;
        const tinsel_bvh_node& a = tree[n.left_index];
        const tinsel_bvh_node& b = tree[ref_right(n)];
        n.lower.x = minT(a.lower.x, b.lower.x); n.lower.y = minT(a.lower.y, b.lower.y); n.lower.z = minT(a.lower.z, b.lower.z);
        n.upper.x = maxT(a.upper.x, b.upper.x); n.upper.y = maxT(a.upper.y, b.upper.y); n.upper.z = maxT(a.upper.z, b.upper.z);
    }
}

struct SceneLevel
{
    std::vector<tinsel_bvh_node> tree;
    ConvertedBvh bvh;
    std::vector<PrimBox> boxes;
    std::vector<float> planeEq;
    unsigned long long scanMask = 0;
    bool everyPrimHasALeaf = true;
};

void mark_plane_table(SceneLevel& lvl, const std::vector<Prim64>& prims, const std::vector<int32_t>& planeTable)
{
    lvl.planeEq.assign(planeTable.size()*4, 0.0f);
    for (size_t t = 0; t < planeTable.size(); ++t)
    {
        const int32_t k = planeTable[t];
        if (lvl.boxes[(size_t)k].alwaysHit)
        {
            lvl.boxes[(size_t)k].alwaysHit = 2u;
            const Prim64& pp = prims[(size_t)k];
            lvl.planeEq[t*4 + 0] = pp.g0; lvl.planeEq[t*4 + 1] = pp.g1; lvl.planeEq[t*4 + 2] = pp.g2; lvl.planeEq[t*4 + 3] = pp.g3;
        }
    }
    lvl.scanMask = 0;
    for (size_t k = 0; k < lvl.boxes.size() && k < 64; ++k)
        if (lvl.boxes[k].alwaysHit != 2u)
            lvl.scanMask |= 1ull << k;
}

bool build_scene_level(std::vector<tinsel_bvh_node> tree, const std::vector<Prim64>& prims, const std::vector<int32_t>& planeTable, SceneLevel& out)
{
    const int P = (int)prims.size();
    if (!convert_bvh(tree.data(), (int)tree.size(), P, 0, out.bvh))
        return false;
    out.boxes.assign((size_t)P, PrimBox());
    std::vector<char> seen((size_t)P, 0);
    for (const tinsel_bvh_node& nd : tree)
        if (ref_is_leaf(nd) && nd.left_index < (uint32_t)P)
        {
            out.boxes[nd.left_index] = make_prim_box(nd);
            seen[nd.left_index] = 1;
        }
    out.everyPrimHasALeaf = std::find(seen.begin(), seen.end(), 0) == seen.end();
    mark_plane_table(out, prims, planeTable);
    out.tree = std::move(tree);
    return true;
}

void adopt_scene_level(tinsel_hip* r, SceneLevel& lvl)
{
    r->scene.root = lvl.bvh.root;
    r->scene.scanMask = lvl.scanMask;
    r->sceneStackNeed = lvl.bvh.maxLeafDepth + 1;
    r->sceneBvhHost = std::move(lvl.tree);
}

int upload_scene_level(tinsel_hip* r, SceneLevel& lvl)
{
    unsigned char* arenaDev = const_cast<unsigned char*>(r->scene.arena);
    if (!lvl.bvh.nodes.empty())
        HIP_TRY(hipMemcpy(arenaDev + r->arenaOffNodes, lvl.bvh.nodes.data(), sizeof(Node64)*lvl.bvh.nodes.size(), hipMemcpyHostToDevice));
    HIP_TRY(hipMemcpy(arenaDev + r->arenaOffBoxes, lvl.boxes.data(), sizeof(PrimBox)*lvl.boxes.size(), hipMemcpyHostToDevice));
    if (!lvl.planeEq.empty())
        HIP_TRY(hipMemcpy(const_cast<float4*>(r->scene.planeEq), lvl.planeEq.data(), sizeof(float)*lvl.planeEq.size(), hipMemcpyHostToDevice));
    adopt_scene_level(r, lvl);
    return 0;
}

int fitting_stack(const tinsel_hip* r, int sceneNeed, const std::vector<DevMesh>& meshes)
{
    int maxMeshNeed = 0;
    for (const DevMesh& dm : meshes)
        maxMeshNeed = std::max(maxMeshNeed, dm.stackNeed);
    const int stack = pick_stack(sceneNeed + maxMeshNeed);
    return stack >= 0 && stack_bytes(r, stack) <= (size_t)r->sharedMemLimit ? stack : -1;
}

template <class Build>
int timed_build(double* ms, Build&& build)
{
    Event e0, e1;
    if (e0.create(true) || e1.create(true))
        return -1;
    (void)hipEventRecord(e0, nullptr);
    const int rc = build();
    (void)hipEventRecord(e1, nullptr);
    (void)hipEventSynchronize(e1);
    float t = 0.0f;
    (void)hipEventElapsedTime(&t, e0, e1);
    if (!rc && ms)
        *ms = t;
    return rc;
}

int write_mesh_prim_area(tinsel_hip* r, int p)
{
    const float area = r->meshArea[(size_t)r->primMesh[(size_t)p]]*r->primEndScale[(size_t)p];
    const float rcpArea = 1.0f/area;
    unsigned char* mat = const_cast<unsigned char*>(r->scene.arena) + r->arenaOffMats + sizeof(Mat128)*(size_t)p;
    HIP_TRY(hipMemcpy(mat + offsetof(Mat128, area), &area, sizeof(float), hipMemcpyHostToDevice));
    HIP_TRY(hipMemcpy(mat + offsetof(Mat128, rcpArea), &rcpArea, sizeof(float), hipMemcpyHostToDevice));
    return 0;
}

}

extern "C" {

int tinsel_hip_set_mesh_bvh(tinsel_hip* r, int mode, double* build_ms)
{
    lookahead_cancel(r);
    if (!r || (mode != TINSEL_BVH_REFERENCE && mode != TINSEL_BVH_LBVH && mode != TINSEL_BVH_PLOC))
        return fail("set_mesh_bvh: bad arguments");
    HIP_TRY(hipSetDevice(r->device));
    HIP_TRY(hipDeviceSynchronize());
    if (build_ms)
        *build_ms = 0.0;

    std::vector<DevMesh> next = r->meshesRef;
    DevPool built;
    const int rc = mode == TINSEL_BVH_REFERENCE ? 0 : timed_build(build_ms, [&] {
        int rc = 0;
        for (size_t m = 0; m < next.size() && !rc; ++m)
            if (!next[m].inArena && next[m].numTris >= 2)
                rc = build_device_bvh(built, r->meshesRef[m], next[m], mode);
        return rc;
    });
    const int stack = rc ? -1 : fitting_stack(r, r->sceneStackNeed, next);
    if (stack < 0)
        return rc ? rc : fail("set_mesh_bvh: tree too deep for the LDS traversal stack (previous trees kept)");
    if (!next.empty())
        HIP_TRY(hipMemcpy((void*)r->scene.meshes, next.data(), sizeof(DevMesh)*next.size(), hipMemcpyHostToDevice));
    r->meshesNow = next;
    r->stackNeed = stack;
    r->bvhMode = mode;
    r->lbvhTrees = std::move(built);
    return 0;
}

int tinsel_hip_refit_mesh(tinsel_hip* r, int primitive, const float* positions_xyz, int num_vertices, const float* normals_xyz)
{
    lookahead_cancel(r);
    if (!r || !positions_xyz || primitive < 0 || primitive >= r->scene.numPrims || r->primMesh[(size_t)primitive] < 0)
        return fail("refit_mesh: bad arguments (a mesh primitive and its new positions)");
    const int mi = r->primMesh[(size_t)primitive];
    DevMesh& dm = r->meshesNow[(size_t)mi];
    if (num_vertices != r->meshNumVertices[(size_t)mi])
        return fail("refit_mesh: the topology must not change (vertex count differs)");
    HIP_TRY(hipSetDevice(r->device));
    HIP_TRY(hipDeviceSynchronize());

    const int numTris = dm.numTris;
    const int numNodes = numTris - 1;
    {
        DevBuf<float> posDev, own;
        DevBuf<int> gen;
        if (posDev.upload(positions_xyz, 3*(size_t)num_vertices))
            return fail("refit_mesh: upload failed");
        hipLaunchKernelGGL(k_refit_tris, dim3((unsigned)((numTris + 255)/256)), dim3(256), 0, nullptr, const_cast<Tri48*>(dm.tris), numTris, posDev.get());
        if (normals_xyz && hipMemcpy(const_cast<float*>(dm.normals), normals_xyz, sizeof(float)*3*(size_t)num_vertices, hipMemcpyHostToDevice) != hipSuccess)
            return fail("refit_mesh: normals upload failed");
        if (numNodes > 0)
        {
            if (own.alloc(6*(size_t)numNodes) || gen.alloc((size_t)numNodes))
                return fail("refit_mesh: device allocation failed");
            const DevMesh* trees[2] = { &dm, r->meshesRef[(size_t)mi].nodes != dm.nodes ? &r->meshesRef[(size_t)mi] : nullptr };
            for (const DevMesh* tree : trees)
                if (tree && refit_device_bvh(*tree, dm.tris, own.get(), gen.get()))
                    return -1;
        }
        if (hipDeviceSynchronize() != hipSuccess || hipGetLastError() != hipSuccess)
            return fail("refit_mesh: kernels failed");
    }

    const std::vector<int32_t>& idx = r->meshIndices[(size_t)mi];
    std::vector<float> cdf((size_t)numTris);
    float totalArea = 0.0f;
    for (int t = 0; t < numTris; ++t)
    {
        const float* a = positions_xyz + (size_t)idx[(size_t)t*3 + 0]*3;
        const float* b = positions_xyz + (size_t)idx[(size_t)t*3 + 1]*3;
        const float* c = positions_xyz + (size_t)idx[(size_t)t*3 + 2]*3;
        const V3 ab(b[0] - a[0], b[1] - a[1], b[2] - a[2]), ac(c[0] - a[0], c[1] - a[1], c[2] - a[2]);
        const float area = 0.5f*length(cross(ab, ac));
        totalArea += area;
        cdf[(size_t)t] = totalArea;
    }
    for (int t = 0; t < numTris; ++t)
        cdf[(size_t)t] /= totalArea;
    HIP_TRY(hipMemcpy(const_cast<float*>(dm.cdf), cdf.data(), sizeof(float)*(size_t)numTris, hipMemcpyHostToDevice));
    r->meshArea[(size_t)mi] = totalArea;
    for (int p = 0; p < r->scene.numPrims; ++p)
        if (r->primMesh[(size_t)p] == mi && write_mesh_prim_area(r, p))
            return -1;

    V3 lo(kFltMax, kFltMax, kFltMax), hi(-kFltMax, -kFltMax, -kFltMax);
    for (size_t k = 0; k < (size_t)numTris*3; ++k)
    {
        const float* v = positions_xyz + (size_t)idx[k]*3;
        lo = V3(minT(lo.x, v[0]), minT(lo.y, v[1]), minT(lo.z, v[2]));
        hi = V3(maxT(hi.x, v[0]), maxT(hi.y, v[1]), maxT(hi.z, v[2]));
    }
    r->meshRootLo[(size_t)mi] = lo;
    r->meshRootHi[(size_t)mi] = hi;
    std::vector<tinsel_bvh_node> tree = r->sceneBvhHost;
    for (tinsel_bvh_node& nd : tree)
        if (ref_is_leaf(nd) && nd.left_index < (uint32_t)r->scene.numPrims && r->primMesh[nd.left_index] == mi)
        {
            V3 l, u;
            primitive_bounds(r, (int)nd.left_index, l, u);
            nd.lower.x = l.x; nd.lower.y = l.y; nd.lower.z = l.z;
            nd.upper.x = u.x; nd.upper.y = u.y; nd.upper.z = u.z;
        }
    union_ancestors(tree);
    SceneLevel lvl;
    if (!build_scene_level(std::move(tree), r->primsHost, r->planeTablePrims, lvl))
        return fail("refit_mesh: the scene BVH could not be refitted");
    return upload_scene_level(r, lvl);
}

int tinsel_hip_set_primitive_transform(tinsel_hip* r, int index, const tinsel_transform* start, const tinsel_transform* end)
{
    lookahead_cancel(r);
    if (!r || !start || !end || index < 0 || index >= r->scene.numPrims)
        return fail("set_primitive_transform: bad arguments");
    HIP_TRY(hipSetDevice(r->device));
    HIP_TRY(hipDeviceSynchronize());
    const Xform xs = to_xform(*start), xe = to_xform(*end);
    const bool isStatic = memcmp(start, end, sizeof(tinsel_transform)) == 0;
    r->primStart[(size_t)index] = xs;
    r->primEnd[(size_t)index] = xe;
    r->primEndScale[(size_t)index] = xe.s;
    Prim64& o = r->primsHost[(size_t)index];
    set_prim_pose(o, xs, xe, isStatic);
    set_prim_derived(o);
    const Moving64 mv = make_moving(xs, xe);
    unsigned char* arenaDev = const_cast<unsigned char*>(r->scene.arena);
    HIP_TRY(hipMemcpy(arenaDev + r->arenaOffPrims + sizeof(Prim64)*(size_t)index, &o, sizeof(Prim64), hipMemcpyHostToDevice));
    HIP_TRY(hipMemcpy(arenaDev + r->arenaOffMoving + sizeof(Moving64)*(size_t)index, &mv, sizeof(Moving64), hipMemcpyHostToDevice));
    if (o.type == kPrimMesh && write_mesh_prim_area(r, index))
        return -1;
    r->sceneDirty = true;
    return 0;
}

int tinsel_hip_rebuild_scene(tinsel_hip* r, int mode, const tinsel_bvh_node* nodes, int num_nodes, double* build_ms)
{
    lookahead_cancel(r);
    if (!r || (mode != TINSEL_SCENE_BVH_NODES && mode != TINSEL_SCENE_BVH_DEVICE) || (mode == TINSEL_SCENE_BVH_NODES && (!nodes || num_nodes <= 0)))
        return fail("rebuild_scene: bad arguments");
    HIP_TRY(hipSetDevice(r->device));
    HIP_TRY(hipDeviceSynchronize());
    if (build_ms)
        *build_ms = 0.0;
    const int P = r->scene.numPrims;

    std::vector<tinsel_bvh_node> ref;
    if (mode == TINSEL_SCENE_BVH_NODES)
        ref.assign(nodes, nodes + num_nodes);
    else
    {
        std::vector<V3> lo((size_t)P), hi((size_t)P);
        for (int i = 0; i < P; ++i)
            primitive_bounds(r, i, lo[(size_t)i], hi[(size_t)i]);
        ref.resize(1);
        if (P == 1)
            node64_to_reference({}, kLeafBit | 0u, lo[0].x, lo[0].y, lo[0].z, hi[0].x, hi[0].y, hi[0].z, ref, 0u);
        else
        {
            std::vector<Tri48> items((size_t)P);
            for (int i = 0; i < P; ++i)
            {
                Tri48& T = items[(size_t)i];
                T.ax = lo[(size_t)i].x; T.ay = lo[(size_t)i].y; T.az = lo[(size_t)i].z; T.i0 = i;
                T.bx = hi[(size_t)i].x; T.by = hi[(size_t)i].y; T.bz = hi[(size_t)i].z; T.i1 = i;
                T.cx = lo[(size_t)i].x; T.cy = lo[(size_t)i].y; T.cz = lo[(size_t)i].z; T.i2 = i;
            }
            DevBuf<Tri48> itemsDev;
            DevPool tree;
            if (itemsDev.alloc((size_t)P))
                return -1;
            std::vector<Node64> built((size_t)P - 1);
            DevMesh fake, out;
            memset(&fake, 0, sizeof(fake));
            fake.tris = itemsDev.get();
            fake.numTris = P;
            fake.inArena = 1;
            if (hipMemcpy(itemsDev.get(), items.data(), sizeof(Tri48)*(size_t)P, hipMemcpyHostToDevice) != hipSuccess)
                return fail("rebuild_scene: upload failed");
            if (timed_build(build_ms, [&] { return build_device_bvh(tree, fake, out, TINSEL_BVH_PLOC); }))
                return -1;
            if (hipMemcpy(built.data(), out.nodes, sizeof(Node64)*((size_t)P - 1), hipMemcpyDeviceToHost) != hipSuccess)
                return fail("rebuild_scene: read-back failed");
            const Node64& rt = built[0];
            ref.reserve((size_t)2*P - 1);
            node64_to_reference(built, 0u, minT(rt.lminx, rt.rminx), minT(rt.lminy, rt.rminy), minT(rt.lminz, rt.rminz),
                                maxT(rt.lmaxx, rt.rmaxx), maxT(rt.lmaxy, rt.rmaxy), maxT(rt.lmaxz, rt.rmaxz), ref, 0u);
        }
    }

    SceneLevel lvl;
    if (!build_scene_level(std::move(ref), r->primsHost, r->planeTablePrims, lvl))
        return fail("rebuild_scene: malformed scene BVH");
    if ((int)lvl.bvh.nodes.size() != (P > 1 ? P - 1 : 0))
        return fail("rebuild_scene: the scene BVH must have one leaf per primitive");
    if (!lvl.everyPrimHasALeaf)
        return fail("rebuild_scene: a primitive has no leaf in the scene BVH");
    const int stack = fitting_stack(r, lvl.bvh.maxLeafDepth + 1, r->meshesNow);
    if (stack < 0)
        return fail("rebuild_scene: tree too deep for the LDS traversal stack (previous tree kept)");
    if (upload_scene_level(r, lvl))
        return -1;
    r->stackNeed = stack;
    r->sceneDirty = false;
    return 0;
}

}
```

tinsel_amd/csrc/tn_host_state.h:

```cpp
#pragma once

inline tinsel_hip_tuning tuning_defaults()
{
    tinsel_hip_tuning t;
    memset(&t, 0, sizeof(t));
    t.struct_bytes = (uint32_t)sizeof(t);
    t.flat_scan = t.lds_scene = t.walk = t.inline_max_tris = t.walk_min_tris = -1;
    t.small_mesh_bytes = t.arena_lds_limit = -1;
    t.batch_paths = 0;
    t.grid_mult = 0;
    t.bounce_share = t.repack = t.tail_split = t.shade_sorted = t.overlap = t.scene_walk = t.swalk_lds = -1;
    t.tail_share = 0.0f;
    t.tail_divide = 4;
    t.accumulate = TINSEL_ACCUMULATE_AUTO;
    t.walk_block = 0;
    t.walk_single = t.walk_lds_stack = t.quads_in_scan = t.bounce_fit = -1;
    t.walk_refill_min = t.walk_leaf_min = t.walk_grid_mult = 0;
    return t;
}

inline tinsel_hip_tuning tuning_from_caller(const tinsel_hip_tuning* in)
{
    tinsel_hip_tuning t = tuning_defaults();
    if (in && in->struct_bytes >= sizeof(uint32_t))
        memcpy(&t, in, std::min<size_t>(in->struct_bytes, sizeof(t)));
    t.struct_bytes = (uint32_t)sizeof(t);
    return t;
}

struct tinsel_hip
{
    int device = 0;
    int numCUs = 256;
    tinsel_hip_tuning tune = tuning_defaults();

    DevPool sceneMem;
    DevScene scene;
    int stackNeed = 16;
    int neePerPath = 0;

    std::vector<DevMesh> meshesRef, meshesNow;
    std::vector<int> meshNumVertices;
    std::vector<std::vector<int32_t>> meshIndices;
    std::vector<int> primMesh;
    std::vector<int32_t> lightPrims;
    std::vector<float> primEndScale;
    std::vector<Prim64> primsHost;
    size_t arenaOffPrims = 0, arenaOffMoving = 0, arenaOffMats = 0;
    std::vector<V3> meshRootLo, meshRootHi;
    std::vector<float> meshArea;
    bool sceneDirty = false;
    std::vector<Xform> primStart, primEnd;
    std::vector<tinsel_bvh_node> sceneBvhHost;
    size_t arenaOffNodes = 0, arenaOffBoxes = 0;
    std::vector<int32_t> planeTablePrims;
    int sceneStackNeed = 1;
    std::string prepRefused;
    bool sceneEnclosed = false;
    int bvhMode = TINSEL_BVH_REFERENCE;
    int rrStart = 0;
    bool anyTransmission = false;
    bool anySubsurface = false;
    int lastBounceKind = -1;
    uint32_t lastBounceFeatures = 0;
    DevPool lbvhTrees;

    int width = 0, height = 0;
    float4* accum = nullptr;
    DevBuf<float4> accumOwn;

    DevBuf<int> accTilesDev;
    int accTilesCount = 0;
    int accTilesKey[6] = { 0, 0, 0, 0, 0, 0 };

    DevBuf<float4> display[3];
    const float4* presented = nullptr;

    size_t batchSlots = 0;
    int batchNee = -1;
    int batchDepth = -1;
    DevPool batchMem;
    PathState ps;
    QueueCtl ctl;
    int batchPipeline = -1;
    BinPrims binPrims = { 0, { 0, 0, 0, 0, 0, 0, 0 } };
    BinPrims walkPrims = { 0, { 0, 0, 0, 0, 0, 0, 0 } };
    int walkPrimMesh[7] = { 0, 0, 0, 0, 0, 0, 0 };
    struct DenseLane
    {
        SplitState ss;
        size_t splitCap = 0;
        uint32_t splitMaxRegions = 0;
        uint32_t* regionOrder = nullptr;
        uint32_t* regionOrderNee = nullptr;
        uint32_t* walkList = nullptr;
        uint32_t* segPrefix = nullptr;
        float4* walkRec = nullptr;
        uint32_t regions = 0, paths = 0;
    } lane[2];
    DevBuf<uint32_t> walkOverflow[2];
    int lastLane = 0;
    int batchLanes = 1;
    size_t batchStateSlots = 0;
    struct LaneSync
    {
        Stream stream;
        Event fork, join, accDone;
        int create() { return stream.create() || fork.create() || join.create() || accDone.create() ? -1 : 0; }
    } laneSync;
    bool walkEnabled = true;
    DevBuf<unsigned long long> walkProf;
    DevBuf<uint2> probeAlias;
    int sharedMemLimit = 65536;
    DevBuf<uint32_t> passSeedsDev;
    size_t passSeedsCount = 0;
    uint32_t passSeedsBase = 0;
    const uint32_t* passSeeds = nullptr;
    Event passSeedsReady;
    hipStream_t passSeedsStream = nullptr;
    DevBuf<unsigned long long> statsDev;
    DevBuf<unsigned char> queryRaysDev, queryOutDev;
    static constexpr uint32_t kQueryCursors = 64;
    struct QueryCursors
    {
        DevBuf<uint32_t> words;
        Event done[kQueryCursors];
        bool used[kQueryCursors] = {};
        uint32_t next = 0;
        int create()
        {
            if (words.alloc(kQueryCursors))
                return -1;
            for (Event& e : done)
                if (e.create())
                    return -1;
            return 0;
        }
    };
    std::unique_ptr<QueryCursors> queryCursors;
    Event batchFence, queryFork[2];
    hipStream_t batchFenceStream = nullptr;
    bool batchFencePending = false;
    DevBuf<unsigned char> gatherRad, gatherStartsDev;
    DevBuf<unsigned char> featRec, featOut;
    DevBuf<uint32_t> featSeeds;
    Event featFence;
    hipStream_t featFenceStream = nullptr;
    bool featFencePending = false;
    DevBuf<unsigned char> idsRec, idsState, idsOut;
    DevBuf<uint32_t> idsSeeds;
    Event idsFence;
    hipStream_t idsFenceStream = nullptr;
    bool idsFencePending = false;
    DevBuf<unsigned char> groupsRec, groupsOut;
    DevBuf<uint32_t> groupsSeeds;
    DevBuf<int8_t> groupsTable;
    std::vector<int8_t> groupsTableHost;
    DevBuf<unsigned long long> groupsStats;
    Event groupsFence;
    hipStream_t groupsFenceStream = nullptr;
    bool groupsFencePending = false;
    DevBuf<float4> denoise[4];
    DevBuf<unsigned char> denoiseIn, denoiseOut;
    Event denoiseFence;
    hipStream_t denoiseFenceStream = nullptr;
    bool denoiseFencePending = false;

    size_t lastBatchSlots = 0;
    int lastPipeline = TINSEL_PIPELINE_WAVEFRONT;
    size_t maxBatchSlots = 8u << 20;
    bool batchSlotsExplicit = false;
    int pipeline = TINSEL_PIPELINE_AUTO;
    int arith = TINSEL_ARITH_EXACT;
    bool pathKernelsPrepared = false;
    int segPrefixLds = 0;
    bool countDetail = false;

    uint32_t passIndex = 0;
    Rng seedRng = Rng::seeded(1u);
    uint32_t seedRngIndex = 0;
    int shardRank = 0, shardWorld = 1, shardTile = 32;

    int lookahead = 0;
    FrameParams lastFp;
    struct SpecShot { DevBuf<float4> buf; Event ready; };
    std::vector<DevBuf<float4>> specFree;
    std::deque<SpecShot> specQueue;
    uint32_t specNextPass = 0;
    tinsel_camera specCamera;
    tinsel_options specOptions;
    int specPasses = 0;
    int lookaheadDepth = 0;
    Stream workStream, copyStream;
    PinnedOutput pinned;

    void* comm = nullptr;
    int commRank = 0, commWorld = 0;

    bool timing = false;
    std::vector<TimedSpan> spans;
    std::vector<Event> eventPool;
    double gpuSeconds = 0.0;
};
```

tinsel_amd/csrc/tn_isect.h:

```cpp
#pragma once

#include "tn_scene.h"

namespace tn {

template <int STRIDE>
struct LdsStack
{
    uint32_t* base;
    TN_D void set(int i, uint32_t v) { base[i*STRIDE] = v; }
    TN_D uint32_t get(int i) const { return base[i*STRIDE]; }
};

struct TraceCounters
{
    uint32_t internal;
    uint32_t tris;
    uint32_t prims;
};

#if TN_FAST
TN_D float minf_ref(float a, float b) { return fminf(a, b); }
TN_D float maxf_ref(float a, float b) { return fmaxf(a, b); }
#else
TN_D float minf_ref(float a, float b) { return a < b ? a : b; }
TN_D float maxf_ref(float a, float b) { return a > b ? a : b; }
#endif

TN_D bool ray_aabb(V3 pos, V3 rcp, float minx, float miny, float minz, float maxx, float maxy, float maxz, float& t)
{
    float l1 = (minx - pos.x)*rcp.x;
    float l2 = (maxx - pos.x)*rcp.x;
    float lmin = minf_ref(l1, l2);
    float lmax = maxf_ref(l1, l2);

    l1 = (miny - pos.y)*rcp.y;
    l2 = (maxy - pos.y)*rcp.y;
    lmin = maxf_ref(minf_ref(l1, l2), lmin);
    lmax = minf_ref(maxf_ref(l1, l2), lmax);

    l1 = (minz - pos.z)*rcp.z;
    l2 = (maxz - pos.z)*rcp.z;
    lmin = maxf_ref(minf_ref(l1, l2), lmin);
    lmax = minf_ref(maxf_ref(l1, l2), lmax);

    bool hit = ((lmax >= 0.f) & (lmax >= lmin));
    if (hit)
        t = lmin;
    return hit;
}

TN_D bool ray_aabb_minmax(V3 pos, V3 rcp, float minx, float miny, float minz, float maxx, float maxy, float maxz, float& t)
{
    float l1 = (minx - pos.x)*rcp.x;
    float l2 = (maxx - pos.x)*rcp.x;
    float lmin = fminf(l1, l2);
    float lmax = fmaxf(l1, l2);

    l1 = (miny - pos.y)*rcp.y;
    l2 = (maxy - pos.y)*rcp.y;
    lmin = fmaxf(fminf(l1, l2), lmin);
    lmax = fminf(fmaxf(l1, l2), lmax);

    l1 = (minz - pos.z)*rcp.z;
    l2 = (maxz - pos.z)*rcp.z;
    lmin = fmaxf(fminf(l1, l2), lmin);
    lmax = fminf(fmaxf(l1, l2), lmax);

    t = lmin;
    return (lmax >= 0.f) & (lmax >= lmin);
}

TN_D bool finite_bits(float x) { return (__float_as_uint(x) & 0x7f800000u) != 0x7f800000u; }

TN_D Node64 load_node(const Node64* nodes, uint32_t idx)
{
    const float4* p = reinterpret_cast<const float4*>(nodes + idx);
    float4 a = p[0], b = p[1], c = p[2], d = p[3];
    Node64 n;
    n.lminx = a.x; n.lminy = a.y; n.lminz = a.z; n.lmaxx = a.w;
    n.lmaxy = b.x; n.lmaxz = b.y; n.rminx = b.z; n.rminy = b.w;
    n.rminz = c.x; n.rmaxx = c.y; n.rmaxy = c.z; n.rmaxz = c.w;
    n.left = __float_as_uint(d.x);
    n.right = __float_as_uint(d.y);
    return n;
}

TN_D bool ray_sphere(V3 center, float radius, V3 o, V3 d, float& outT, V3& outN)
{
    V3 q = o - center;
    float a = 1.0f;
    float b = 2.0f*dot(q, d);
    float c = dot(q, q) - (radius*radius);

    float disc = b*b - 4.0f*a*c;
    if (disc < 0.0f)
        return false;

    float sgn = (b < 0.0f) ? -1.0f : 1.0f;
    float tt = -0.5f*(b + sgn*sqrtf_cr(disc));
    float t0 = tt/a;
    float t1 = c/tt;
    if (t1 < t0) { float tmp = t0; t0 = t1; t1 = tmp; }

    if (t0 < 0.0f && t1 < 0.0f)
        return false;
    if (t0 < 0.0f && t1 > 0.0f)
        t0 = t1;

    outN = normalize((o + d*t0) - center);
    outT = t0;
    return true;
}

TN_D bool ray_plane(V3 p, V3 dir, float px, float py, float pz, float pw, float& t)
{
    float d = px*dir.x + py*dir.y + pz*dir.z + pw*0.0f;
    if (d == 0.0f)
        return false;
    t = -(px*p.x + py*p.y + pz*p.z + pw*1.0f)/d;
    return t > 0.0f;
}

TN_D bool ray_tri(V3 p, V3 dir, V3 a, V3 b, V3 c, float& t, float& u, float& v, float& w, float& sign, V3& n)
{
    V3 ab = b - a;
    V3 ac = c - a;
    n = cross(ab, ac);

    V3 nd = -dir;
    float d = dot(nd, n);
    float ood = rcpf_cr(d);
    V3 ap = p - a;

    t = dot(ap, n)*ood;
    if (t < 0.0f)
        return false;

    V3 e = cross(nd, ap);
    v = dot(ac, e)*ood;
    if (v < 0.0f || v > 1.0f)
        return false;
    w = -dot(ab, e)*ood;
    if (w < 0.0f || v + w > 1.0f)
        return false;

    u = 1.0f - v - w;
    sign = d;
    return true;
}

struct MeshHit
{
    float t, u, v, w;
    int tri;
    V3 n;
};

template <bool COUNT>
TN_D bool ray_mesh_two_leaves(const Node64* mnodes, const Tri48* mtris, uint32_t mroot, V3 o, V3 d, V3 rcp, MeshHit& hit, TraceCounters& ctr)
{
    const Node64 nd = load_node(mnodes, mroot);
    if (COUNT) ctr.internal++;

    float tL, tR;
    const bool hL = ray_aabb(o, rcp, nd.lminx, nd.lminy, nd.lminz, nd.lmaxx, nd.lmaxy, nd.lmaxz, tL) && tL < kFltMax;
    const bool hR = ray_aabb(o, rcp, nd.rminx, nd.rminy, nd.rminz, nd.rmaxx, nd.rmaxy, nd.rmaxz, tR) && tR < kFltMax;

    uint32_t first = nd.left, second = nd.right;
    if (hL && hR && (tL < tR))
    {
        first = nd.right;
        second = nd.left;
    }
    float closestT = kFltMax;
    auto leaf = [&](uint32_t ref) {
        const int i = (int)(ref & ~kLeafBit);
        const float4* tp = reinterpret_cast<const float4*>(mtris + i);
        const float4 ta = tp[0], tb = tp[1], tc = tp[2];
        if (COUNT) ctr.tris++;
        float t, u, v, w, sign;
        V3 n;
        if (ray_tri(o, d, V3(ta.x, ta.y, ta.z), V3(tb.x, tb.y, tb.z), V3(tc.x, tc.y, tc.z), t, u, v, w, sign, n))
        {
            if (t > 0.0f && t < closestT)
            {
                closestT = t;
                hit.t = t; hit.u = u; hit.v = v; hit.w = w;
                hit.tri = i;
                hit.n = n*sign;
            }
        }
    };
    if (hR)
        leaf(second);
    if (hL)
        leaf(first);
    return closestT < kFltMax;
}

template <class Stack, bool COUNT, bool ANYHIT = false>
TN_D bool ray_mesh(const Node64* mnodes, const Tri48* mtris, uint32_t mroot, Stack& st, int sp, V3 o, V3 d, V3 rcp, MeshHit& hit, TraceCounters& ctr, float tStop = 0.0f)
{
    float closestT = kFltMax;
    float tmax = kFltMax;

    const int base = sp;
    st.set(sp++, mroot);

    while (sp > base)
    {
        uint32_t ref = st.get(--sp);

        if (ref & kLeafBit)
        {
            const int i = (int)(ref & ~kLeafBit);
            const float4* tp = reinterpret_cast<const float4*>(mtris + i);
            float4 ta = tp[0], tb = tp[1], tc = tp[2];
            if (COUNT) ctr.tris++;

            float t, u, v, w, sign;
            V3 n;
            if (ray_tri(o, d, V3(ta.x, ta.y, ta.z), V3(tb.x, tb.y, tb.z), V3(tc.x, tc.y, tc.z), t, u, v, w, sign, n))
            {
                if (t > 0.0f && t < closestT)
                {
                    closestT = t;
                    hit.t = t; hit.u = u; hit.v = v; hit.w = w;
                    hit.tri = i;
                    hit.n = n*sign;
                    if (ANYHIT && t < tStop)
                        break;
                }
            }
            tmax = closestT;
        }
        else
        {
            Node64 nd = load_node(mnodes, ref);
            if (COUNT) ctr.internal++;

            float tL, tR;
            bool hL = ray_aabb(o, rcp, nd.lminx, nd.lminy, nd.lminz, nd.lmaxx, nd.lmaxy, nd.lmaxz, tL) && tL < tmax;
            bool hR = ray_aabb(o, rcp, nd.rminx, nd.rminy, nd.rminz, nd.rmaxx, nd.rmaxy, nd.rmaxz, tR) && tR < tmax;

            uint32_t first = nd.left, second = nd.right;
            if (hL && hR && (tL < tR))
            {
                first = nd.right;
                second = nd.left;
            }
            if (hL)
                st.set(sp++, first);
            if (hR)
                st.set(sp++, second);
        }
    }
    return closestT < kFltMax;
}

TN_D Xform prim_pose(const DevScene& sc, const Prim64& p, float time)
{
    Xform x;
    if (p.flags & kPrimMoving)
    {
        const float4* mp = reinterpret_cast<const float4*>(sc.moving + p.moving);
        float4 a0 = mp[0], a1 = mp[1], b0 = mp[2], b1 = mp[3];
        Xform s, e;
        s.p = V3(a0.x, a0.y, a0.z); s.s = a0.w; s.r = { a1.x, a1.y, a1.z, a1.w };
        e.p = V3(b0.x, b0.y, b0.z); e.s = b0.w; e.r = { b1.x, b1.y, b1.z, b1.w };
        x = interpolate_xform(s, e, time);
    }
    else
    {
// ... 35 lines not shown
    {
        const Q4 c = qconj(x.r);
        lo = rs*qrotate(c, op);
        ld = rs*qrotate(c, d);
    }
    lrcp = rcp3_cr(ld);
}

template <class F4>
TN_D Prim64 unpack_prim(const F4& a, const F4& b, const F4& c, const F4& d)
{
    Prim64 p;
    p.px = a.x; p.py = a.y; p.pz = a.z; p.s = a.w;
    p.rx = b.x; p.ry = b.y; p.rz = b.z; p.rw = b.w;
    p.g0 = c.x; p.g1 = c.y; p.g2 = c.z; p.g3 = c.w;
    p.type = __float_as_uint(d.x); p.flags = __float_as_uint(d.y);
    p.mesh = __float_as_uint(d.z); p.moving = __float_as_uint(d.w);
    return p;
}

TN_D Prim64 load_prim(const Prim64* prims, int idx)
{
    const float4* pp = reinterpret_cast<const float4*>(prims + idx);
    float4 a = pp[0], b = pp[1], c = pp[2], d = pp[3];
    return unpack_prim(a, b, c, d);
}

TN_D Prim64 load_prim_uniform(ConstF4 prims, int idx)
{
    ConstF4 pp = prims + (size_t)idx*4;
    const ConstF4V a = pp[0], b = pp[1], c = pp[2], d = pp[3];
    return unpack_prim(a, b, c, d);
}

template <class SC, class Stack, bool COUNT, bool ANYHIT = false, bool UNIFORM = false>
TN_D bool prim_intersect(const SC& sc, int index, Stack& st, int sp, V3 o, V3 d, float time, float& outT, V3& outN, TraceCounters& ctr, float tStop = 0.0f,
                         V3 rcpWorld = V3(0.0f), bool haveRcpWorld = false, const Prim64* fetched = nullptr)
{
    Prim64 p = fetched ? *fetched : UNIFORM ? load_prim_uniform(sc.kPrims, index) : load_prim(sc.prims, index);
    if constexpr (!(SC::kFeatures & kFeatMotion))
        p.flags &= ~(uint32_t)kPrimMoving;
    if (COUNT) ctr.prims++;

    if (p.type == kPrimPlane)
    {
        bool hit = ray_plane(o, d, p.g0, p.g1, p.g2, p.g3, outT);
        if (hit)
            outN = V3(p.g0, p.g1, p.g2);
        return hit;
    }

    const Xform x = prim_pose(sc, p, time);

    if (p.type == kPrimSphere)
    {
        return ray_sphere(x.p, p.g0*x.s, o, d, outT, outN);
    }

    V3 lo, ld, lrcp;
    pose_inv_ray(p, x, o, d, lo, ld, lrcp, rcpWorld, haveRcpWorld);

    MeshHit h;
    const Tri48* mtris;
    const float* nr;
    if (!(SC::kWalkedOnly && !SC::kQuadsInline) && (p.flags & kPrimQuadArena))
    {
        const unsigned char* base = (SC::kLds || sc.arenaLdsBytes != 0u) ? sc.ldsBase : sc.arena;
        const QuadOffsets q = quad_offsets(__float_as_uint(p.g0), __float_as_uint(p.g1));
        mtris = reinterpret_cast<const Tri48*>(base + q.tris);
        nr = reinterpret_cast<const float*>(base + q.normals);
        if (!ray_mesh_two_leaves<COUNT>(reinterpret_cast<const Node64*>(base + q.nodes), mtris, 0u, lo, ld, lrcp, h, ctr))
            return false;
    }
    else
    {
    const DevMesh m = sc.meshes[p.mesh];
    mtris = mesh_tris(sc, m);
    nr = mesh_normals(sc, m);
    const bool fromRecord = SC::kQuadsInline ? (p.flags & kPrimWalked) != 0u
                          : SC::kWalkedOnly || (!COUNT && sc.walkRec != nullptr && (p.flags & kPrimWalked));
    if (fromRecord)
    {
        const uint32_t kb = (p.flags >> kPrimWalkLaneShift) & 7u;
        const float4* rp = sc.walkRec + (size_t)(sc.walkItem + kb)*2;
        const float4 ra = rp[0];
        if (!(ra.x < kFltMax))
            return false;
        const float4 rb = rp[1];
        h.t = ra.x; h.u = ra.y; h.v = ra.z; h.w = ra.w;
        h.n = V3(rb.x, rb.y, rb.z);
        h.tri = __float_as_int(rb.w);
    }
    else if (SC::kWalkedOnly && !SC::kQuadsInline)
        return false;
    else if (m.twoLeaves)
    {
        if (!ray_mesh_two_leaves<COUNT>(mesh_nodes(sc, m), mtris, m.root, lo, ld, lrcp, h, ctr))
            return false;
    }
    else if (SC::kWalkedOnly || !(SC::kFeatures & kFeatMeshWalk))
        return false;
    else if (!ray_mesh<Stack, COUNT, ANYHIT>(mesh_nodes(sc, m), mtris, m.root, st, sp, lo, ld, lrcp, h, ctr, tStop))
        return false;
    }

    const float4* tp = reinterpret_cast<const float4*>(mtris + h.tri);
    const int i0 = __float_as_int(tp[0].w), i1 = __float_as_int(tp[1].w), i2 = __float_as_int(tp[2].w);
    V3 n1(nr[i0*3 + 0], nr[i0*3 + 1], nr[i0*3 + 2]);
    V3 n2(nr[i1*3 + 0], nr[i1*3 + 1], nr[i1*3 + 2]);
    V3 n3(nr[i2*3 + 0], nr[i2*3 + 1], nr[i2*3 + 2]);

    V3 smooth = h.u*n1 + h.v*n2 + h.w*n3;
    if (dot(smooth, h.n) < 0.0f)
        smooth = smooth*(-1.0f);

    outT = h.t;
    outN = safe_normalize(pose_xform_vector(p, x, smooth), h.n);
    return true;
}

TN_D unsigned long long wave_uniform64(unsigned long long v)
{
    const uint32_t lo = (uint32_t)__builtin_amdgcn_readfirstlane((int)(uint32_t)v), hi = (uint32_t)__builtin_amdgcn_readfirstlane((int)(uint32_t)(v >> 32));
    return ((unsigned long long)hi << 32) | lo;
}

template <class SC, class Stack, bool COUNT, bool ANYHIT = false>
TN_D int trace_flat(const SC& sc, Stack& st, V3 o, V3 d, V3 rcp, float time, float& outT, V3& outN, bool& tie, TraceCounters& ctr, float tStop = 0.0f)
{
    float minT = kFltMax;
    int closest = -1;
    V3 cn;
    tie = false;

    auto accept = [&](int i, float t, V3 n) {
        if (t > 0.0f)
        {
            if (fabsf(t - minT) <= 1e-5f*fabsf(t))
                tie = true;
            if (t < minT)
            {
                minT = t;
                closest = i;
                cn = n;
            }
        }
    };

    unsigned long long meshes = 0;
    const bool finiteAll = __all(finite_bits(rcp.x) && finite_bits(rcp.y) && finite_bits(rcp.z) &&
                                 finite_bits(o.x) && finite_bits(o.y) && finite_bits(o.z));
    const int numPlanes = sc.numPlanes;
    int pk = 0;
    for (; pk + 4 <= numPlanes; pk += 4)
    {
        const ConstF4V e0 = sc.kPlaneEq[pk], e1 = sc.kPlaneEq[pk + 1], e2 = sc.kPlaneEq[pk + 2], e3 = sc.kPlaneEq[pk + 3];
        const ConstF4V id = sc.kPlaneIdx[pk >> 2];
        float t0, t1, t2, t3;
        const bool h0 = ray_plane(o, d, e0.x, e0.y, e0.z, e0.w, t0);
        const bool h1 = ray_plane(o, d, e1.x, e1.y, e1.z, e1.w, t1);
        const bool h2 = ray_plane(o, d, e2.x, e2.y, e2.z, e2.w, t2);
        const bool h3 = ray_plane(o, d, e3.x, e3.y, e3.z, e3.w, t3);
        if (h0) accept(__float_as_int(id.x), t0, V3(e0.x, e0.y, e0.z));
        if (h1) accept(__float_as_int(id.y), t1, V3(e1.x, e1.y, e1.z));
        if (h2) accept(__float_as_int(id.z), t2, V3(e2.x, e2.y, e2.z));
        if (h3) accept(__float_as_int(id.w), t3, V3(e3.x, e3.y, e3.z));
    }
    if (pk < numPlanes)
    {
        const ConstF4V id = sc.kPlaneIdx[pk >> 2];
        const int left = numPlanes - pk;
        if (left >= 2)
        {
            const ConstF4V e0 = sc.kPlaneEq[pk], e1 = sc.kPlaneEq[pk + 1];
            float t0, t1;
            const bool h0 = ray_plane(o, d, e0.x, e0.y, e0.z, e0.w, t0);
            const bool h1 = ray_plane(o, d, e1.x, e1.y, e1.z, e1.w, t1);
            if (h0) accept(__float_as_int(id.x), t0, V3(e0.x, e0.y, e0.z));
            if (h1) accept(__float_as_int(id.y), t1, V3(e1.x, e1.y, e1.z));
        }
        if (left & 1)
        {
            const ConstF4V e0 = sc.kPlaneEq[pk + (left & 2)];
            float t0;
            if (ray_plane(o, d, e0.x, e0.y, e0.z, e0.w, t0))
                accept(__float_as_int(left == 1 ? id.x : id.z), t0, V3(e0.x, e0.y, e0.z));
        }
    }
    for (unsigned long long todo = wave_uniform64(sc.scanMask); todo != 0ull; todo &= todo - 1ull)
    {
        const int i = (int)__builtin_ctzll(todo);
        ConstF4V b0 = sc.kBoxes[i*2], b1 = sc.kBoxes[i*2 + 1];
        ConstF4V ra = sc.kPrims[i*4], rb = sc.kPrims[i*4 + 1], rc = sc.kPrims[i*4 + 2], rd = sc.kPrims[i*4 + 3];
        asm volatile("" : "+s"(b0), "+s"(b1), "+s"(ra), "+s"(rb), "+s"(rc), "+s"(rd));
        Prim64 rec = unpack_prim(ra, rb, rc, rd);
        if (__float_as_uint(b1.z) == 0u)
        {
            float tb;
            if (!(finiteAll ? ray_aabb_minmax(o, rcp, b0.x, b0.y, b0.z, b0.w, b1.x, b1.y, tb) : ray_aabb(o, rcp, b0.x, b0.y, b0.z, b0.w, b1.x, b1.y, tb)))
                continue;
        }
        if (SC::kDefer != 0 && (SC::kDefer == 1 || sc.deferMeshes) && rec.type == (uint32_t)kPrimMesh)
        {
            meshes |= 1ull << i;
            continue;
        }
        float t;
        V3 n;
        const bool primHit = prim_intersect<SC, Stack, COUNT, ANYHIT, true>(sc, i, st, 0, o, d, time, t, n, ctr, tStop, rcp, true, &rec);
        if (primHit)
            accept(i, t, n);
        if (ANYHIT && minT < tStop)
        {
            meshes = 0;
            break;
        }
    }
    if (SC::kDefer != 0)
    {
        while (meshes)
        {
            const int i = (int)__builtin_ctzll(meshes);
            meshes &= meshes - 1ull;
            float t;
            V3 n;
            if (prim_intersect<SC, Stack, COUNT, ANYHIT>(sc, i, st, 0, o, d, time, t, n, ctr, tStop, rcp, true))
                accept(i, t, n);
            if (ANYHIT && minT < tStop)
                break;
        }
    }

    outT = minT;
    outN = face_forward(cn, -d);
    return closest;
}

template <class SC>
TN_D bool ray_meets_bounded_prim(const SC& sc, V3 o, V3 d)
{
    const V3 rcp = rcp3_cr(d);
    bool any = false;
    for (int i = 0; i < sc.numPrims; ++i)
    {
        const float4* bp = reinterpret_cast<const float4*>(sc.primBoxes + i);
        const float4 b0 = bp[0], b1 = bp[1];
        if (__float_as_uint(b1.z) != 0u)
            continue;
        float tb;
        any = any || ray_aabb(o, rcp, b0.x, b0.y, b0.z, b0.w, b1.x, b1.y, tb);
    }
    return any;
}

TN_D bool ray_sane(V3 o) { return fabsf(o.x) < 1e6f && fabsf(o.y) < 1e6f && fabsf(o.z) < 1e6f; }

TN_D float shadow_stop(float dist)
{
    return dist < 0.0f ? kFltMax : dist - 0.02f - 1e-5f*dist;
}

template <class SC, class Stack, bool COUNT, bool ANYHIT = false>
TN_D int trace(const SC& sc, Stack& st, V3 o, V3 d, float time, float& outT, V3& outN, TraceCounters& ctr, float tStop = 0.0f)
{
    float minT = kFltMax;
    int closest = -1;
    V3 cn;

    V3 rcp = rcp3_cr(d);

    if (!COUNT && sc.flatScan)
    {
        const bool sane = ray_sane(o);
        bool tie = false;
        int prim = -1;
        if (sane)
            prim = trace_flat<SC, Stack, COUNT, false>(sc, st, o, d, rcp, time, outT, outN, tie, ctr, 0.0f);
        if (sane && !tie)
            return prim;
    }

    int sp = 0;
    st.set(sp++, sc.root);

    while (sp)
    {
        uint32_t ref = st.get(--sp);

        if (ref & kLeafBit)
        {
            float t;
            V3 n;
            const int index = (int)(ref & ~kLeafBit);
            if (prim_intersect<SC, Stack, COUNT, ANYHIT>(sc, index, st, sp, o, d, time, t, n, ctr, tStop, rcp, true))
            {
                if (t < minT && t > 0.0f)
                {
                    minT = t;
                    closest = index;
                    cn = n;
                    if (ANYHIT && t < tStop)
                        break;
                }
            }
        }
        else
        {
            Node64 nd = load_node(sc.nodes, ref);
            if (COUNT) ctr.internal++;

            float tL, tR;
            bool hL = ray_aabb(o, rcp, nd.lminx, nd.lminy, nd.lminz, nd.lmaxx, nd.lmaxy, nd.lmaxz, tL);
            bool hR = ray_aabb(o, rcp, nd.rminx, nd.rminy, nd.rminz, nd.rmaxx, nd.rmaxy, nd.rmaxz, tR);

            uint32_t first = nd.left, second = nd.right;
            if (hL && hR && (tL < tR))
            {
                first = nd.right;
                second = nd.left;
            }
            if (hL)
// ... 13 lines not shown
```

tinsel_amd/csrc/tn_scene.h:

```cpp
#pragma once

#include "tn_math.h"

namespace tn {

constexpr uint32_t kLeafBit = 0x80000000u;
constexpr uint32_t kNoNode = 0xffffffffu;
struct alignas(64) Node64
{
    float lminx, lminy, lminz, lmaxx;
    float lmaxy, lmaxz, rminx, rminy;
    float rminz, rmaxx, rmaxy, rmaxz;
    uint32_t left, right;
    uint32_t pad0, pad1;
};
static_assert(sizeof(Node64) == 64, "Node64");

struct alignas(16) Tri48
{
    float ax, ay, az; int32_t i0;
    float bx, by, bz; int32_t i1;
    float cx, cy, cz; int32_t i2;
};
static_assert(sizeof(Tri48) == 48, "Tri48");

enum : uint32_t
{
    kPrimSphere = 0,
    kPrimPlane = 1,
    kPrimMesh = 2,
};

enum : uint32_t
{
    kPrimMoving = 1u,
    kPrimWalked = 2u,
    kPrimQuadArena = 8u,
    kPrimNoRot = 4u,
    kPrimWalkLaneShift = 8,
};

struct alignas(64) Prim64
{
    float px, py, pz, s;
    float rx, ry, rz, rw;
    float g0, g1, g2, g3;
    uint32_t type;
    uint32_t flags;
    uint32_t mesh;
    uint32_t moving;
};
static_assert(sizeof(Prim64) == 64, "Prim64");

struct QuadOffsets { uint32_t nodes, tris, normals, cdf; };
TN_HD QuadOffsets quad_offsets(uint32_t w0, uint32_t w1)
{
    QuadOffsets q = { (w0 & 0xffffu) << 7, (w0 >> 16) << 7, (w1 & 0xffffu) << 7, (w1 >> 16) << 7 };
    return q;
}

struct alignas(64) Moving64
{
    float spx, spy, spz, ss; float srx, sry, srz, srw;
    float epx, epy, epz, es; float erx, ery, erz, erw;
};
static_assert(sizeof(Moving64) == 64, "Moving64");

struct alignas(128) Mat128
{
    float emission[3]; float ior;
    float color[3];    float metallic;
    float absorption[3]; float subsurface;
    float cspec0[3];   float roughness;
    float sqrtColor[3]; float transmission;
    float clearcoat;
    float clearcoatAlpha;
    float area;
    int32_t lightSamples;
    float clearcoatA2;
    float clearcoatLogA2;
    float rcpArea, rcpLightSamples;
    float cbsdf, clight;
    float pad[2];
};
static_assert(sizeof(Mat128) == 128, "Mat128");

struct alignas(32) PrimBox
{
    float minx, miny, minz, maxx, maxy, maxz;
    uint32_t alwaysHit;
    uint32_t pad;
};
static_assert(sizeof(PrimBox) == 32, "PrimBox");

struct alignas(16) LightRec
{
    int32_t prim;
    int32_t lightSamples;
    float rcpLightSamples;
    int32_t pad;
};

struct DevMesh
{
    const Node64* nodes;
    const Tri48* tris;
    const float* normals;
    const float* cdf;
    uint32_t root;
    int32_t numTris;
    int32_t stackNeed;
    int32_t inArena;
    uint32_t offNodes, offTris, offNormals, offCdf;
    int32_t topCount;
    int32_t twoLeaves;
    int32_t numInternal;
    int32_t pad0;
};

struct DevProbe
{
    const float4* data;
    const float* pdfX;
    const float* cdfX;
    const float* pdfY;
    const float* cdfY;
    int32_t width, height;
    int32_t valid;
    int32_t pad;
    const uint2* alias;
};

struct DevScene
{
    const Node64* nodes;
    const Prim64* prims;
    const Mat128* mats;
    const Moving64* moving;
    const DevMesh* meshes;
    const LightRec* lights;
    uint32_t root;
    int32_t numPrims;
    int32_t numLights;
    int32_t totalLightSamples;
    float horizon[3];
    float zenith[3];
    DevProbe probe;
    const unsigned char* arena;
    uint32_t arenaBytes;
    uint32_t arenaLdsBytes;
    int32_t numMeshes;
    int32_t allInArena;
    const PrimBox* primBoxes;
    int32_t flatScan;
    int32_t hasMedia;
    int32_t sortQueues;
    int32_t deferMeshes;
    const float4* planeEq;
    const int32_t* planeIdx;
    int32_t numPlanes;
    unsigned long long scanMask;
};

typedef float ConstF4V __attribute__((ext_vector_type(4)));
typedef const __attribute__((address_space(4))) ConstF4V* ConstF4;

enum BounceFeature : uint32_t
{
    kFeatMedia = 1u,
    kFeatProbe = 2u,
    kFeatMotion = 4u,
    kFeatMeshWalk = 8u,
    kFeatSphere = 16u,
    kFeatTransmission = 32u,
    kFeatPools = 64u,
    kFeatShare = 128u,
    kFeatSort = 256u,
    kFeatRoulette = 512u,
    kFeatAll = 1023u
};

template <bool LDS, int WALKED_ONLY = 0, int DEFER = 2, bool MIXED = false, uint32_t FEATURES = kFeatAll>
struct SceneT : DevScene
{
    static constexpr uint32_t kFeatures = FEATURES;
    static constexpr bool kLds = LDS;
    static constexpr bool kMixed = MIXED;
    static constexpr bool kWalkedOnly = WALKED_ONLY != 0;
    static constexpr bool kQuadsInline = WALKED_ONLY == 2;
    static constexpr int kDefer = DEFER;
    const unsigned char* ldsBase;
    ConstF4 kPrims, kBoxes, kPlaneEq, kPlaneIdx;
    const float4* walkRec;
    uint32_t walkItem;
};

template <class SC> TN_D const Node64* mesh_nodes(const SC& sc, const DevMesh& m)
{
    if constexpr (SC::kLds && SC::kMixed) return m.inArena ? reinterpret_cast<const Node64*>(sc.ldsBase + m.offNodes) : m.nodes;
    else if constexpr (SC::kLds) return reinterpret_cast<const Node64*>(sc.ldsBase + m.offNodes); else return m.nodes;
}
template <class SC> TN_D const Tri48* mesh_tris(const SC& sc, const DevMesh& m)
{
    if constexpr (SC::kLds && SC::kMixed) return m.inArena ? reinterpret_cast<const Tri48*>(sc.ldsBase + m.offTris) : m.tris;
    else if constexpr (SC::kLds) return reinterpret_cast<const Tri48*>(sc.ldsBase + m.offTris); else return m.tris;
}
template <class SC> TN_D const float* mesh_normals(const SC& sc, const DevMesh& m)
{
    if constexpr (SC::kLds && SC::kMixed) return m.inArena ? reinterpret_cast<const float*>(sc.ldsBase + m.offNormals) : m.normals;
    else if constexpr (SC::kLds) return reinterpret_cast<const float*>(sc.ldsBase + m.offNormals); else return m.normals;
}
template <class SC> TN_D const float* mesh_cdf(const SC& sc, const DevMesh& m)
{
    if constexpr (SC::kLds && SC::kMixed) return m.inArena ? reinterpret_cast<const float*>(sc.ldsBase + m.offCdf) : m.cdf;
    else if constexpr (SC::kLds) return reinterpret_cast<const float*>(sc.ldsBase + m.offCdf); else return m.cdf;
}

}
```

tinsel_amd/renderer.py:

```python
import ctypes as C
import os

import numpy as np

from . import abi

_HERE = os.path.dirname(os.path.abspath(__file__))
LIB_PATH = os.environ.get("TINSEL_HIP_LIB", os.path.join(_HERE, "libtinsel_hip.so"))

_lib = None
DEFAULT_TUNING = None


class TinselHipError(RuntimeError):
    pass


def load_library():
    global _lib
    if _lib is not None:
        return _lib
    if not os.path.exists(LIB_PATH):
        raise TinselHipError(
            "%s is missing: build it with `python -m tinsel_amd.build` (hipcc, gfx950). "
            "There is no CPU fallback." % LIB_PATH)
    try:
        import torch
    except Exception:
        pass
    L = C.CDLL(LIB_PATH)
    vp, ci, cf = C.c_void_p, C.c_int, C.c_float
    L.tinsel_hip_create.restype = vp
    L.tinsel_hip_create.argtypes = [C.POINTER(abi.SceneDesc), ci]
    if hasattr(L, "tinsel_hip_create_tuned"):
        L.tinsel_hip_tuning_init.restype = None
        L.tinsel_hip_tuning_init.argtypes = [C.POINTER(abi.Tuning)]
        L.tinsel_hip_create_tuned.restype = vp
        L.tinsel_hip_create_tuned.argtypes = [C.POINTER(abi.SceneDesc), ci, C.POINTER(abi.Tuning)]
        L.tinsel_hip_set_tuning.argtypes = [vp, C.POINTER(abi.Tuning)]
        L.tinsel_hip_get_tuning.argtypes = [vp, C.POINTER(abi.Tuning)]
        L.tinsel_hip_group_create_tuned.restype = vp
        L.tinsel_hip_group_create_tuned.argtypes = [C.POINTER(abi.SceneDesc), ci, ci, C.POINTER(abi.Tuning)]
        L.tinsel_hip_comm_unique_id.argtypes = [vp, ci]
        L.tinsel_hip_comm_init.argtypes = [vp, vp, ci, ci]
        L.tinsel_hip_comm_size.argtypes = [vp]
        L.tinsel_hip_comm_reduce_accum.argtypes = [vp, vp, ci, vp]
    L.tinsel_hip_destroy.restype = None
    L.tinsel_hip_destroy.argtypes = [vp]
    L.tinsel_hip_init.argtypes = [vp, ci, ci]
    L.tinsel_hip_init_external.argtypes = [vp, ci, ci, vp]
    L.tinsel_hip_render.argtypes = [vp, C.POINTER(abi.Camera), C.POINTER(abi.Options), vp, ci]
    L.tinsel_hip_render_async.argtypes = [vp, C.POINTER(abi.Camera), C.POINTER(abi.Options), ci, vp]
    L.tinsel_hip_accum_device_ptr.restype = vp
    L.tinsel_hip_accum_device_ptr.argtypes = [vp]
    L.tinsel_hip_read_accum.argtypes = [vp, vp]
    L.tinsel_hip_set_shard.argtypes = [vp, ci, ci, ci]
    L.tinsel_hip_set_pipeline.argtypes = [vp, ci]
    L.tinsel_hip_set_pass_index.argtypes = [vp, C.c_uint32]
    L.tinsel_hip_get_pass_index.restype = C.c_uint32
    L.tinsel_hip_get_pass_index.argtypes = [vp]
    L.tinsel_hip_stats.restype = None
    L.tinsel_hip_stats.argtypes = [vp, C.POINTER(C.c_ulonglong), C.POINTER(C.c_ulonglong), C.POINTER(C.c_double)]
    L.tinsel_hip_reset_stats.restype = None
    L.tinsel_hip_reset_stats.argtypes = [vp]
    L.tinsel_hip_stats_detail.argtypes = [vp, vp]
    L.tinsel_hip_set_detail_counters.argtypes = [vp, ci]
    L.tinsel_hip_render_cost.argtypes = [vp, C.POINTER(abi.Camera), C.POINTER(abi.Options), C.c_uint32, ci, vp]
    L.tinsel_hip_trace_rays.argtypes = [vp, ci, C.c_longlong, vp, vp]
    L.tinsel_hip_trace_rays_device.argtypes = [vp, ci, C.c_longlong, vp, vp, vp]
    L.tinsel_hip_trace_camera.argtypes = [vp, C.POINTER(abi.Camera), ci, ci, cf, vp]
    if hasattr(L, "tinsel_hip_trace_radiance"):
        L.tinsel_hip_trace_radiance.argtypes = [vp, C.c_longlong, vp, ci, vp]
        L.tinsel_hip_trace_radiance_device.argtypes = [vp, C.c_longlong, vp, ci, vp, vp]
    if hasattr(L, "tinsel_hip_gather_radiance"):
        L.tinsel_hip_gather_radiance.argtypes = [vp, ci, C.c_longlong, vp, ci, ci, vp, vp]
        L.tinsel_hip_gather_radiance_device.argtypes = [vp, ci, C.c_longlong, vp, ci, ci, vp, vp, vp]
    if hasattr(L, "tinsel_hip_gather_sh"):
        L.tinsel_hip_gather_sh.argtypes = [vp, ci, ci, C.c_longlong, vp, ci, ci, vp, vp]
        L.tinsel_hip_gather_sh_device.argtypes = [vp, ci, ci, C.c_longlong, vp, ci, ci, vp, vp, vp]
    if hasattr(L, "tinsel_hip_render_features"):
        L.tinsel_hip_render_features.argtypes = [vp, C.POINTER(abi.Camera), C.POINTER(abi.Options), C.c_uint32, ci, C.c_uint, vp]
        L.tinsel_hip_render_features_device.argtypes = [vp, C.POINTER(abi.Camera), C.POINTER(abi.Options), C.c_uint32, ci, C.c_uint, vp, vp]
    if hasattr(L, "tinsel_hip_render_id_mattes"):
        L.tinsel_hip_render_id_mattes.argtypes = [vp, C.POINTER(abi.Camera), C.POINTER(abi.Options), C.c_uint32, ci, ci, vp, vp]
        L.tinsel_hip_render_id_mattes_device.argtypes = [vp, C.POINTER(abi.Camera), C.POINTER(abi.Options), C.c_uint32, ci, ci, vp, vp, vp]
    if hasattr(L, "tinsel_hip_render_light_groups"):
        L.tinsel_hip_render_light_groups.argtypes = [vp, C.POINTER(abi.Camera), C.POINTER(abi.Options), C.c_uint32, ci, ci, vp, ci, vp]
        L.tinsel_hip_render_light_groups_device.argtypes = [vp, C.POINTER(abi.Camera), C.POINTER(abi.Options), C.c_uint32, ci, ci, vp, ci, vp, vp]
    if hasattr(L, "tinsel_hip_denoise"):
        L.tinsel_hip_denoise_params_init.restype = None
        L.tinsel_hip_denoise_params_init.argtypes = [C.POINTER(abi.DenoiseParams)]
        L.tinsel_hip_denoise.argtypes = [vp, vp, vp, C.c_uint, ci, ci, C.POINTER(abi.DenoiseParams), vp]
        L.tinsel_hip_denoise_device.argtypes = [vp, vp, vp, C.c_uint, ci, ci, C.POINTER(abi.DenoiseParams), vp, vp]
        L.tinsel_hip_present_image_device.argtypes = [vp, vp, C.POINTER(abi.Options), ci, C.c_float, vp]
    L.tinsel_hip_kernel_times.argtypes = [vp, C.POINTER(abi.KernelTime), ci]
    L.tinsel_hip_enable_kernel_timing.argtypes = [vp, ci]
    L.tinsel_hip_set_batch_paths.argtypes = [vp, C.c_ulonglong]
    L.tinsel_hip_read_batch_radiance.restype = C.c_longlong
    L.tinsel_hip_read_batch_radiance.argtypes = [vp, vp, C.c_ulonglong]
    L.tinsel_hip_leaf.argtypes = [vp, ci, ci, ci, vp, ci, vp, vp, ci, C.POINTER(abi.Camera), ci, ci]
    L.tinsel_hip_write_accum.argtypes = [vp, vp, C.c_uint32]
    L.tinsel_hip_reserve.argtypes = [vp, ci, ci]
    L.tinsel_hip_set_russian_roulette.argtypes = [vp, ci]
    L.tinsel_hip_set_mesh_bvh.argtypes = [vp, ci, C.POINTER(C.c_double)]
    L.tinsel_hip_present.argtypes = [vp, C.POINTER(abi.Options), ci, C.c_float, vp]
    L.tinsel_hip_present_async.argtypes = [vp, C.POINTER(abi.Options), ci, C.c_float, vp]
    L.tinsel_hip_present_device_ptr.restype = vp
    L.tinsel_hip_present_device_ptr.argtypes = [vp]
    L.tinsel_image_quantize_rgb8.argtypes = [vp, ci, ci, vp]
    L.tinsel_hip_stack_entries.argtypes = [vp]
    if hasattr(L, "tinsel_hip_mesh_tree"):
        L.tinsel_hip_mesh_tree.argtypes = [vp, ci, vp, ci, C.POINTER(C.c_int)]
    L.tinsel_hip_nee_per_path.argtypes = [vp]
    L.tinsel_hip_walked_prims.argtypes = [vp]
    if hasattr(L, "tinsel_hip_walk_tops"):
        L.tinsel_hip_walk_tops.argtypes = [vp, C.POINTER(C.c_int), ci]
    if hasattr(L, "tinsel_hip_bounce_plan"):
        L.tinsel_hip_bounce_plan.argtypes = [vp, C.POINTER(C.c_uint32)]
        L.tinsel_hip_scene_features.restype = C.c_uint
        L.tinsel_hip_scene_features.argtypes = [C.POINTER(abi.SceneDesc)]
    if hasattr(L, "tinsel_hip_scene_slim"):
        L.tinsel_hip_scene_slim.argtypes = [C.POINTER(abi.SceneDesc)]
    if hasattr(L, "tinsel_hip_queue_counts"):
        L.tinsel_hip_queue_counts.argtypes = [vp, C.POINTER(C.c_uint32), C.c_int]
    L.tinsel_hip_set_lookahead.argtypes = [vp, ci]
    L.tinsel_hip_refit_mesh.argtypes = [vp, ci, vp, ci, vp]
    if hasattr(L, "tinsel_hip_rebuild_scene"):
        L.tinsel_hip_set_primitive_transform.argtypes = [vp, ci, C.POINTER(abi.Transform), C.POINTER(abi.Transform)]
        L.tinsel_hip_rebuild_scene.argtypes = [vp, ci, vp, ci, C.POINTER(C.c_double)]
    L.tinsel_hip_set_probe_sampling.argtypes = [vp, ci]
    L.tinsel_hip_set_arithmetic.argtypes = [vp, ci]
    L.tinsel_hip_get_arithmetic.argtypes = [vp]
    L.tinsel_hip_group_create.restype = vp
    L.tinsel_hip_group_create.argtypes = [C.POINTER(abi.SceneDesc), ci, ci]
    L.tinsel_hip_group_destroy.restype = None
    L.tinsel_hip_group_destroy.argtypes = [vp]
    L.tinsel_hip_group_init.argtypes = [vp, ci, ci]
    L.tinsel_hip_group_render.argtypes = [vp, C.POINTER(abi.Camera), C.POINTER(abi.Options), vp, ci]
    L.tinsel_hip_group_present.argtypes = [vp, C.POINTER(abi.Options), ci, C.c_float, vp]
    L.tinsel_hip_group_size.argtypes = [vp]
    L.tinsel_hip_group_member.restype = vp
    L.tinsel_hip_group_member.argtypes = [vp, ci]
    L.tinsel_hip_group_set_lookahead.argtypes = [vp, ci]
    L.tinsel_hip_ubench.argtypes = [ci, ci, C.c_ulonglong, ci, C.POINTER(C.c_double), C.POINTER(C.c_double)]
    L.tinsel_hip_selftest_arith.argtypes = [ci, ci, ci, C.POINTER(C.c_ulonglong), C.POINTER(C.c_uint)]
    if hasattr(L, "tinsel_hip_selftest_sort"):
        L.tinsel_hip_selftest_sort.argtypes = [ci, vp, C.c_ulonglong, ci, ci]
        L.tinsel_hip_selftest_scan.argtypes = [ci, vp, vp, C.c_ulonglong]
    if hasattr(L, "tinsel_hip_selftest_accumulate"):
        L.tinsel_hip_selftest_accumulate.argtypes = abi.SELFTEST_ACCUMULATE_ARGTYPES
        L.tinsel_hip_accumulate_support.argtypes = [ci, C.c_float, C.c_float, C.c_float, C.POINTER(C.c_float)]
    L.tinsel_hip_plan_regions.argtypes = [C.c_ulonglong, ci, ci, ci, C.POINTER(C.c_uint)]
    L.tinsel_hip_last_error.restype = C.c_char_p
    L.tinsel_pack_open.argtypes = [vp, C.c_size_t, C.POINTER(abi.SceneDesc), C.POINTER(abi.Camera), C.POINTER(abi.Options)]
    _lib = L
    return L


EXPORTED_SYMBOLS = [
    "tinsel_hip_bounce_plan", "tinsel_hip_scene_features", "tinsel_hip_scene_slim", "tinsel_hip_create", "tinsel_hip_destroy", "tinsel_hip_init", "tinsel_hip_init_external", "tinsel_hip_render",
    "tinsel_hip_render_async", "tinsel_hip_accum_device_ptr", "tinsel_hip_read_accum", "tinsel_hip_set_shard",
    "tinsel_hip_set_pipeline", "tinsel_hip_set_pass_index", "tinsel_hip_get_pass_index", "tinsel_hip_stats",
    "tinsel_hip_reset_stats", "tinsel_hip_stats_detail", "tinsel_hip_set_detail_counters", "tinsel_hip_render_cost", "tinsel_hip_kernel_times", "tinsel_hip_kernel_time_bytes",
    "tinsel_hip_enable_kernel_timing", "tinsel_hip_set_batch_paths", "tinsel_hip_stack_entries", "tinsel_hip_mesh_tree",
    "tinsel_hip_nee_per_path", "tinsel_hip_last_error", "tinsel_pack_open", "tinsel_hip_read_batch_radiance", "tinsel_hip_leaf",
    "tinsel_hip_write_accum", "tinsel_hip_reserve", "tinsel_hip_set_russian_roulette", "tinsel_hip_set_mesh_bvh", "tinsel_hip_present", "tinsel_hip_present_async", "tinsel_hip_present_device_ptr", "tinsel_image_quantize_rgb8",
    "tinsel_hip_walked_prims", "tinsel_hip_walk_tops", "tinsel_hip_queue_counts", "tinsel_hip_set_lookahead", "tinsel_hip_set_arithmetic", "tinsel_hip_get_arithmetic", "tinsel_hip_refit_mesh", "tinsel_hip_set_probe_sampling",
    "tinsel_hip_set_primitive_transform", "tinsel_hip_rebuild_scene",
    "tinsel_hip_group_create", "tinsel_hip_group_destroy", "tinsel_hip_group_init", "tinsel_hip_group_render", "tinsel_hip_group_present",
    "tinsel_hip_group_size", "tinsel_hip_group_member", "tinsel_hip_group_set_lookahead", "tinsel_hip_ubench",
    "tinsel_hip_selftest_arith", "tinsel_hip_selftest_sort", "tinsel_hip_selftest_scan", "tinsel_hip_selftest_accumulate", "tinsel_hip_accumulate_support", "tinsel_hip_plan_regions",
    "tinsel_hip_tuning_init", "tinsel_hip_create_tuned", "tinsel_hip_set_tuning", "tinsel_hip_get_tuning", "tinsel_hip_group_create_tuned",
    "tinsel_hip_comm_unique_id", "tinsel_hip_comm_init", "tinsel_hip_comm_size", "tinsel_hip_comm_reduce_accum",
    "tinsel_hip_trace_rays", "tinsel_hip_trace_rays_device", "tinsel_hip_trace_camera",
    "tinsel_hip_trace_radiance", "tinsel_hip_trace_radiance_device",
    "tinsel_hip_gather_radiance", "tinsel_hip_gather_radiance_device",
    "tinsel_hip_gather_sh", "tinsel_hip_gather_sh_device",
    "tinsel_hip_render_features", "tinsel_hip_render_features_device",
    "tinsel_hip_render_id_mattes", "tinsel_hip_render_id_mattes_device",
    "tinsel_hip_render_light_groups", "tinsel_hip_render_light_groups_device",
    "tinsel_hip_denoise_params_init", "tinsel_hip_denoise", "tinsel_hip_denoise_device", "tinsel_hip_present_image_device",
]


def rank_id_lists(ids, weights):
    ids, weights = np.asarray(ids, np.int32), np.asarray(weights, np.float32)
    empty = ids == abi.ID_EMPTY
    order = np.lexsort((ids, -weights.astype(np.float64), empty), axis=0)
    return np.take_along_axis(ids, order, 0), np.take_along_axis(weights, order, 0)


def matte(result, ids):
    wanted = np.isin(np.asarray(result["ids"]), np.atleast_1d(np.asarray(ids, np.int64)))
    wanted &= np.asarray(result["ids"]) != abi.ID_EMPTY
    total = np.asarray(result["total"], np.float32)
    s = np.where(wanted, np.asarray(result["weights"], np.float32), np.float32(0)).sum(axis=0, dtype=np.float32)
    out = np.zeros(total.shape, np.float32)
    np.divide(s, total, out=out, where=total != 0)
    return out


def merge_id_mattes(results, slots):
    results = list(results)
    slots = int(slots)
    if not results or not 1 <= slots:
        raise ValueError("merge_id_mattes: at least one result and one slot")
    H, W = np.asarray(results[0]["total"]).shape
    cap = sum(np.asarray(r["ids"]).shape[0] for r in results)
    ids = np.full((cap, H, W), abi.ID_EMPTY, np.int32)
    weights = np.zeros((cap, H, W), np.float32)
    residual, total = np.zeros((H, W), np.float32), np.zeros((H, W), np.float32)
    for r in results:
        rid, rw = np.asarray(r["ids"], np.int32), np.asarray(r["weights"], np.float32)
        for k in range(rid.shape[0]):
            c, w = rid[k], rw[k]
            todo = c != abi.ID_EMPTY
            held = (ids == c[None]) & todo[None]
            weights = np.where(held, weights + w[None], weights)
            todo &= ~held.any(axis=0)
            first = np.argmax(ids == abi.ID_EMPTY, axis=0)
            jj, ii = np.nonzero(todo)
            ids[first[jj, ii], jj, ii] = c[jj, ii]
            weights[first[jj, ii], jj, ii] = w[jj, ii]
        residual = residual + np.asarray(r["residual"], np.float32)
        total = total + np.asarray(r["total"], np.float32)
    ids, weights = rank_id_lists(ids, weights)
    for k in range(slots, cap):
        residual = residual + weights[k]
    if cap < slots:
        ids = np.concatenate([ids, np.full((slots - cap, H, W), abi.ID_EMPTY, np.int32)])
        weights = np.concatenate([weights, np.zeros((slots - cap, H, W), np.float32)])
    return {"ids": np.ascontiguousarray(ids[:slots]), "weights": np.ascontiguousarray(weights[:slots]), "residual": residual, "total": total}


def rng_state(seed, skip=0):
    shape = np.shape(seed)
    s1 = np.asarray(seed).astype(np.uint32).reshape(-1) + np.uint32(315645664)
    s2 = s1 ^ np.uint32(0x13AB45FE)
    for _ in range(int(skip)):
        s1 = (s2 ^ ((s1 << np.uint32(5)) | (s1 >> np.uint32(27)))) ^ (s1*s2)
        s2 = s1 ^ ((s2 << np.uint32(12)) | (s2 >> np.uint32(20)))
    return s1.reshape(shape), s2.reshape(shape)


RAY_EPSILON = 1e-4


def camera_rays(camera, width, height):
    jj, ii = np.mgrid[0:int(height), 0:int(width)].astype(np.float64)
    f = np.tan(np.float64(camera.fov)*0.5)
    v = np.stack([f*(float(width)/float(height))*(2.0*ii/width - 1.0), f*(1.0 - 2.0*jj/height), -np.ones_like(ii)], axis=-1)
    q = np.array([camera.rotation.x, camera.rotation.y, camera.rotation.z], np.float64)
    w = np.float64(camera.rotation.w)
    t = 2.0*np.cross(q, v)
    d = v + w*t + np.cross(q, t)
    origin = np.array([camera.position.x, camera.position.y, camera.position.z], np.float64)
    return origin, d/np.linalg.norm(d, axis=-1, keepdims=True)


GATHER_MODES = {"cosine": abi.GATHER_COSINE, "sphere": abi.GATHER_SPHERE}


def gather_points(positions, normals, samples, time=1.0, base_seed=0, seeds=None):
    positions = np.asarray(positions, np.float32).reshape(-1, 3)
    n = positions.shape[0]
    pts = np.zeros(n, abi.GATHER_POINT_DTYPE)
    pts["px"], pts["py"], pts["pz"] = positions[:, 0], positions[:, 1], positions[:, 2]
    normals = np.asarray(normals, np.float32).reshape(n, 3)
    pts["nx"], pts["ny"], pts["nz"] = normals[:, 0], normals[:, 1], normals[:, 2]
    pts["time"] = np.asarray(time, np.float32)
    if seeds is None:
        seeds = (int(base_seed) + np.arange(n, dtype=np.uint64)*np.uint64(int(samples))) & np.uint64(0xffffffff)
    pts["seed"] = np.asarray(seeds).astype(np.uint32)
    return pts


def sh_basis(directions, order=2):
    order = int(order)
    if not 0 <= order <= abi.GATHER_SH_MAX_ORDER:
        raise ValueError("sh_basis: order is 0, 1 or 2")
    d = np.asarray(directions, np.float32)
    if d.ndim < 1 or d.shape[-1] != 3:
        raise ValueError("sh_basis: directions [..., 3] are expected")
    x, y, z = d[..., 0], d[..., 1], d[..., 2]
    f = np.float32
    Y = [np.full(x.shape, f(0.28209479), np.float32)]
    if order >= 1:
        Y += [f(0.48860251)*y, f(0.48860251)*z, f(0.48860251)*x]
    if order >= 2:
        Y += [(f(1.0925484)*x)*y, (f(1.0925484)*y)*z, f(0.31539157)*((f(3.0)*z)*z - f(1.0)), (f(1.0925484)*x)*z, f(0.54627422)*(x*x - y*y)]
    out = np.stack(Y, axis=-1)
    assert out.dtype == np.float32
    return out


SH_COSINE_LOBE = (np.pi, 2.0*np.pi/3.0, np.pi/4.0)


def sh_irradiance(coeffs, normals):
    c = np.asarray(coeffs, np.float64)
    nrm = np.asarray(normals, np.float64).reshape(-1, 3)
    if c.ndim == 2:
        c = c[None]
    if c.ndim != 3 or c.shape[1] not in (1, 4, 9) or c.shape[2] != 3 or (c.shape[0] != 1 and c.shape[0] != nrm.shape[0]):
        raise ValueError("sh_irradiance: coeffs [n, C, 3] with C = 1, 4 or 9 and normals [n, 3] (or [m, 3] against one probe) are expected")
    order = {1: 0, 4: 1, 9: 2}[c.shape[1]]
    x, y, z = nrm[:, 0], nrm[:, 1], nrm[:, 2]
    Y = [np.full(x.shape, 0.5*np.sqrt(1.0/np.pi))]
    if order >= 1:
        k = np.sqrt(3.0/(4.0*np.pi))
        Y += [k*y, k*z, k*x]
    if order >= 2:
        k = 0.5*np.sqrt(15.0/np.pi)
        Y += [k*x*y, k*y*z, 0.25*np.sqrt(5.0/np.pi)*(3.0*z*z - 1.0), k*x*z, 0.5*k*(x*x - y*y)]
    band = np.array([SH_COSINE_LOBE[l] for l in (0, 1, 1, 1, 2, 2, 2, 2, 2)][:c.shape[1]])
    return np.einsum("ni,nic->nc", np.stack(Y, axis=-1)*band, np.broadcast_to(c, (nrm.shape[0],) + c.shape[1:]))


def feature_mask(which):
    if isinstance(which, (int, np.integer)):
        mask = int(which)
    else:
        names = [which] if isinstance(which, str) else list(which)
        for n in names:
            if n not in abi.FEATURE_NAMES:
                raise ValueError("features: %r is not one of %s" % (n, ", ".join(abi.FEATURE_NAMES)))
        mask = sum(1 << abi.FEATURE_NAMES.index(n) for n in set(names))
    return mask, [n for k, n in enumerate(abi.FEATURE_NAMES) if 0 <= mask <= 7 and mask >> k & 1]


def feature_images(planes):
    def ratio(num, den):
        den = np.asarray(den, np.float64)
        ok = den != 0.0
        return np.where(ok, np.asarray(num, np.float64)/np.where(ok, den, 1.0), 0.0)

    out = {}
    if "albedo" in planes:
        a = np.asarray(planes["albedo"], np.float64)
        out["albedo"] = ratio(a[..., :3], a[..., 3:4])
    if "normal" in planes:
        a = np.asarray(planes["normal"], np.float64)
        mean = ratio(a[..., :3], a[..., 3:4])
        out["normal"] = ratio(mean, np.sqrt((mean*mean).sum(axis=-1, keepdims=True)))
    if "depth" in planes:
        a = np.asarray(planes["depth"], np.float64)
        mean = ratio(a[..., 0], a[..., 2])
        out["depth"] = mean
        out["depth_variance"] = np.where(a[..., 2] != 0.0, ratio(a[..., 1], a[..., 2]) - mean*mean, 0.0)
        out["coverage"] = ratio(a[..., 2], a[..., 3])
    return out


def default_light_groups(scene, max_groups=abi.MAX_LIGHT_GROUPS):
    max_groups = int(max_groups)
    if not 1 <= max_groups <= abi.MAX_LIGHT_GROUPS:
        raise ValueError("default_light_groups: max_groups is 1 .. %d" % abi.MAX_LIGHT_GROUPS)
    d = scene.desc
    prims = C.cast(d.primitives, C.POINTER(abi.Primitive))
    emitters = [i for i in range(d.num_primitives) if any(v != 0.0 for v in prims[i].material.emission)]
    env = bool(d.probe_valid) or any(v != 0.0 for v in tuple(d.sky_horizon) + tuple(d.sky_zenith))
    room = max_groups - (1 if env else 0)
    if emitters and room < 1:
        raise ValueError("default_light_groups: max_groups = %d leaves no group for the lights beside the environment" % max_groups)
    table = np.full(d.num_primitives, -1, np.int32)
    names = []
    for k, i in enumerate(emitters):
        g = min(k, room - 1)
        table[i] = g
        if g == len(names):
            names.append("prim%d" % i)
        elif not names[g].endswith("+"):
            names[g] += "+"
    env_group = -1
    if env:
        env_group = len(names)
        names.append("env")
    return table, env_group, names


def relight(planes, gains):
    G = int(planes.shape[0])
    if planes.ndim != 4 or planes.shape[-1] != 4 or G < 1:
        raise ValueError("relight: planes [G, H, W, 4] are expected")
    g = np.asarray(gains, np.float32)
    if g.shape not in ((G,), (G, 3)):
        raise ValueError("relight: one gain, or one RGB triple, per group is expected: shape (%d,) or (%d, 3)" % (G, G))
    g = np.broadcast_to(g.reshape(G, -1), (G, 3))
    if _is_tensor(planes):
        import torch
        gt = torch.as_tensor(np.ascontiguousarray(g), device=planes.device)
        out = planes[0].clone()
        out[..., :3] = planes[0][..., :3]*gt[0]
        for k in range(1, G):
            out[..., :3] += planes[k][..., :3]*gt[k]
        return out
    planes = np.asarray(planes, np.float32)
    out = planes[0].copy()
    out[..., :3] = planes[0][..., :3]*g[0]
    for k in range(1, G):
        out[..., :3] += planes[k][..., :3]*g[k]
    return out


def denoise_params(**fields):
    p = abi.DenoiseParams()
    load_library().tinsel_hip_denoise_params_init(C.byref(p))
    names = [k for k, _ in abi.DenoiseParams._fields_]
    for k, v in fields.items():
        if k not in names:
            raise TypeError("tinsel_hip_denoise_params has no field %r" % k)
        setattr(p, k, v)
    return p


def _is_tensor(a):
    return a is not None and not isinstance(a, np.ndarray) and hasattr(a, "data_ptr")


def _check(rc, what):
    if rc != 0:
        msg = load_library().tinsel_hip_last_error()
        raise TinselHipError("%s failed: %s" % (what, msg.decode() if msg else "?"))


def _host_ptr(a):
    return (a if a.size else np.zeros(1, a.dtype)).ctypes.data_as(C.c_void_p)


class Scene:

    def __init__(self, blob: bytes):
        L = load_library()
        self._buf = C.create_string_buffer(blob, len(blob))
        self.desc = abi.SceneDesc()
        self.camera = abi.Camera()
        self.options = abi.Options()
        _check(L.tinsel_pack_open(self._buf, len(blob), C.byref(self.desc), C.byref(self.camera), C.byref(self.options)),
               "tinsel_pack_open")

    @classmethod
    def load_pack(cls, path):
        with open(path, "rb") as fh:
            return cls(fh.read())

    @property
    def num_primitives(self):
        return self.desc.num_primitives

    def bounce_features(self):
        return int(load_library().tinsel_hip_scene_features(C.byref(self.desc)))

    def bounce_slim(self):
        return bool(load_library().tinsel_hip_scene_slim(C.byref(self.desc)))


def _bytes_at(ptr, n):
    return C.string_at(ptr, n) if (ptr and n > 0) else b""


_libc = C.CDLL(None)
_libc.memcmp.argtypes = [C.c_void_p, C.c_void_p, C.c_size_t]


def _same_bytes(pa, pb, n):
    if n <= 0 or pa == pb:
        return True
    return bool(pa) and bool(pb) and _libc.memcmp(pa, pb, n) == 0


def _same_nodes(pa, pb, n):
    if n <= 0 or _same_bytes(pa, pb, n*32):
        return True
    a = np.ctypeslib.as_array((C.c_uint32*(n*8)).from_address(pa)).reshape(n, 8)
    b = np.ctypeslib.as_array((C.c_uint32*(n*8)).from_address(pb)).reshape(n, 8)
    if not np.array_equal(a[:, :7], b[:, :7]):
        return False
    leaf_a, leaf_b = a[:, 7] >> 31, b[:, 7] >> 31
    if not np.array_equal(leaf_a, leaf_b):
        return False
    inner = leaf_a == 0
    return bool(np.array_equal(a[inner, 7], b[inner, 7]))


def scene_delta(old: Scene, new: Scene):
    a, b = old.desc, new.desc
    if a.num_primitives != b.num_primitives or bytes(a.sky_horizon) != bytes(b.sky_horizon) or bytes(a.sky_zenith) != bytes(b.sky_zenith):
        return None
    if (a.probe_valid, a.probe_width, a.probe_height) != (b.probe_valid, b.probe_width, b.probe_height):
        return None
    if a.probe_valid and not _same_bytes(a.probe_data, b.probe_data, a.probe_width*a.probe_height*16):
        return None
    P = a.num_primitives
    pa, pb = (abi.Primitive*P).from_address(a.primitives), (abi.Primitive*P).from_address(b.primitives)
    moves = []
    for i in range(P):
        x, y = pa[i], pb[i]
        mx, my = bytes(x.material), bytes(y.material)
        if x.type != y.type or x.light_samples != y.light_samples or mx[:84] != my[:84] or mx[112:] != my[112:]:
            return None
        if x.type == abi.GEOM_SPHERE and x.geo.sphere.radius != y.geo.sphere.radius:
            return None
        if x.type == abi.GEOM_PLANE and bytes(x.geo.plane) != bytes(y.geo.plane):
            return None
        if x.type == abi.GEOM_MESH:
            g, h = x.geo.mesh, y.geo.mesh
            if (g.num_vertices, g.num_indices, g.num_nodes, g.area) != (h.num_vertices, h.num_indices, h.num_nodes, h.area):
                return None
            for f, n in (("positions", g.num_vertices*12), ("normals", g.num_vertices*12), ("indices", g.num_indices*4), ("cdf", (g.num_indices//3)*4)):
                if not _same_bytes(getattr(g, f), getattr(h, f), n):
                    return None
            if not _same_nodes(g.nodes, h.nodes, g.num_nodes):
                return None
        if bytes(x.start_transform) != bytes(y.start_transform) or bytes(x.end_transform) != bytes(y.end_transform):
            moves.append((i, abi.Transform.from_buffer_copy(bytes(y.start_transform)), abi.Transform.from_buffer_copy(bytes(y.end_transform))))
    nodes = (abi.BVHNode*b.num_bvh_nodes).from_buffer_copy(_bytes_at(b.bvh_nodes, b.num_bvh_nodes*C.sizeof(abi.BVHNode)))
    return moves, nodes


class HipRenderer:

    def __init__(self, scene: Scene, device: int = 0, tuning: "abi.Tuning | None" = None):
        L = load_library()
        self._L = L
        tuning = tuning if tuning is not None else DEFAULT_TUNING
        if tuning is None:
            self._h = L.tinsel_hip_create(C.byref(scene.desc), device)
        else:
            self._h = L.tinsel_hip_create_tuned(C.byref(scene.desc), device, C.byref(tuning))
        if not self._h:
            msg = L.tinsel_hip_last_error()
            raise TinselHipError("tinsel_hip_create failed: %s" % (msg.decode() if msg else "?"))
        self.device = device
        self.num_primitives = int(scene.desc.num_primitives)
        self.width = self.height = 0
        self._accum_tensor = None

    def init(self, width, height, accum_tensor=None):
        if accum_tensor is not None:
            assert tuple(accum_tensor.shape) == (height, width, 4) and accum_tensor.is_contiguous()
            self._accum_tensor = accum_tensor
            _check(self._L.tinsel_hip_init_external(self._h, width, height, accum_tensor.data_ptr()), "tinsel_hip_init_external")
        else:
            self._accum_tensor = None
            _check(self._L.tinsel_hip_init(self._h, width, height), "tinsel_hip_init")
        self.width, self.height = width, height

    def render(self, camera, options, output=None, passes=1, readback=True):
        if output is None and readback:
            output = np.empty((options.height, options.width, 4), np.float32)
        ptr = output.ctypes.data_as(C.c_void_p) if (readback and output is not None) else None
        _check(self._L.tinsel_hip_render(self._h, C.byref(camera), C.byref(options), ptr, passes), "tinsel_hip_render")
        return output

    Init = init
    Render = render

    def render_async(self, camera, options, passes=1, stream=None):
        _check(self._L.tinsel_hip_render_async(self._h, C.byref(camera), C.byref(options), passes, stream), "tinsel_hip_render_async")

    def read_accum(self):
        out = np.empty((self.height, self.width, 4), np.float32)
        _check(self._L.tinsel_hip_read_accum(self._h, out.ctypes.data_as(C.c_void_p)), "tinsel_hip_read_accum")
        return out

    def set_mesh_bvh(self, mode):
        ms = C.c_double(0.0)
        _check(self._L.tinsel_hip_set_mesh_bvh(self._h, int(mode), C.byref(ms)), "tinsel_hip_set_mesh_bvh")
        return ms.value

    def write_accum(self, accum, next_pass_index):
        accum = np.ascontiguousarray(accum, np.float32)
        assert accum.shape == (self.height, self.width, 4)
        _check(self._L.tinsel_hip_write_accum(self._h, accum.ctypes.data_as(C.c_void_p), int(next_pass_index)), "tinsel_hip_write_accum")

    def present(self, options, nlm_width=0, nlm_falloff=200.0, readback=True):
        out = np.empty((self.height, self.width, 4), np.float32) if readback else None
        ptr = out.ctypes.data_as(C.c_void_p) if readback else None
        _check(self._L.tinsel_hip_present(self._h, C.byref(options), int(nlm_width), float(nlm_falloff), ptr), "tinsel_hip_present")
        return out

    @property
    def accum_tensor(self):
        return self._accum_tensor

    def accum_device_ptr(self):
        return self._L.tinsel_hip_accum_device_ptr(self._h)

    def set_shard(self, rank, world, tile=32):
        _check(self._L.tinsel_hip_set_shard(self._h, rank, world, tile), "tinsel_hip_set_shard")

    def set_pipeline(self, pipeline):
        _check(self._L.tinsel_hip_set_pipeline(self._h, pipeline), "tinsel_hip_set_pipeline")

    @staticmethod
    def comm_unique_id():
        buf = (C.c_ubyte*abi.COMM_ID_BYTES)()
        _check(load_library().tinsel_hip_comm_unique_id(buf, abi.COMM_ID_BYTES), "tinsel_hip_comm_unique_id")
        return bytes(buf)

    def comm_init(self, id_bytes, rank, world):
        buf = (C.c_ubyte*abi.COMM_ID_BYTES).from_buffer_copy(bytes(id_bytes))
        _check(self._L.tinsel_hip_comm_init(self._h, buf, int(rank), int(world)), "tinsel_hip_comm_init")

    def comm_size(self):
        return int(self._L.tinsel_hip_comm_size(self._h)) if hasattr(self._L, "tinsel_hip_comm_size") else 0

    def comm_reduce_accum(self, out_ptr, root=0, stream=None):
        _check(self._L.tinsel_hip_comm_reduce_accum(self._h, out_ptr, int(root), stream), "tinsel_hip_comm_reduce_accum")

    def set_tuning(self, tuning=None, **fields):
        t = (tuning if tuning is not None else self.get_tuning()).replace(**fields)
        _check(self._L.tinsel_hip_set_tuning(self._h, C.byref(t)), "tinsel_hip_set_tuning")

    def get_tuning(self):
        t = abi.Tuning()
        _check(self._L.tinsel_hip_get_tuning(self._h, C.byref(t)), "tinsel_hip_get_tuning")
        return t

    def set_arithmetic(self, mode):
        _check(self._L.tinsel_hip_set_arithmetic(self._h, int(mode)), "tinsel_hip_set_arithmetic")

    def refit_mesh(self, primitive, positions, normals=None):
        positions = np.ascontiguousarray(positions, np.float32)
        nptr = None
        if normals is not None:
            normals = np.ascontiguousarray(normals, np.float32)
            nptr = normals.ctypes.data_as(C.c_void_p)
        _check(self._L.tinsel_hip_refit_mesh(self._h, int(primitive), positions.ctypes.data_as(C.c_void_p), int(positions.shape[0]), nptr),
               "tinsel_hip_refit_mesh")

    def set_primitive_transform(self, index, start, end=None):
        end = start if end is None else end
        _check(self._L.tinsel_hip_set_primitive_transform(self._h, int(index), C.byref(start), C.byref(end)), "tinsel_hip_set_primitive_transform")

    def rebuild_scene(self, nodes=None):
        ms = C.c_double(0.0)
        if nodes is None:
            rc = self._L.tinsel_hip_rebuild_scene(self._h, abi.SCENE_BVH_DEVICE, None, 0, C.byref(ms))
        else:
            rc = self._L.tinsel_hip_rebuild_scene(self._h, abi.SCENE_BVH_NODES, C.cast(nodes, C.c_void_p), len(nodes), C.byref(ms))
        _check(rc, "tinsel_hip_rebuild_scene")
        return ms.value

    def update_scene(self, old: Scene, new: Scene):
        d = scene_delta(old, new)
        if d is None:
            return False
        moves, nodes = d
        for i, s, e in moves:
            self.set_primitive_transform(i, s, e)
        self.rebuild_scene(nodes)
        return True

    def set_probe_sampling(self, mode):
        _check(self._L.tinsel_hip_set_probe_sampling(self._h, int(mode)), "tinsel_hip_set_probe_sampling")

    def set_lookahead(self, on):
        _check(self._L.tinsel_hip_set_lookahead(self._h, int(on)), "tinsel_hip_set_lookahead")

    def set_russian_roulette(self, start_bounce):
        _check(self._L.tinsel_hip_set_russian_roulette(self._h, int(start_bounce)), "tinsel_hip_set_russian_roulette")

    def reserve(self, passes, max_depth):
        _check(self._L.tinsel_hip_reserve(self._h, int(passes), int(max_depth)), "tinsel_hip_reserve")

    def get_pass_index(self):
        return int(self._L.tinsel_hip_get_pass_index(self._h))

    def set_pass_index(self, i):
        _check(self._L.tinsel_hip_set_pass_index(self._h, i), "tinsel_hip_set_pass_index")

    def set_batch_paths(self, n):
        _check(self._L.tinsel_hip_set_batch_paths(self._h, n), "tinsel_hip_set_batch_paths")

    def set_detail_counters(self, on):
        _check(self._L.tinsel_hip_set_detail_counters(self._h, int(on)), "tinsel_hip_set_detail_counters")

    def render_cost(self, camera, options, pass_begin=0, passes=1):
        out = np.zeros((options.height, options.width, 4), np.uint32)
        _check(self._L.tinsel_hip_render_cost(self._h, C.byref(camera), C.byref(options), int(pass_begin), int(passes),
                                              out.ctypes.data_as(C.c_void_p)), "tinsel_hip_render_cost")
        return out

    def features(self, camera, options, pass_begin=0, passes=1, which=abi.FEATURE_NAMES, out=None):
        mask, names = feature_mask(which)
        H, W = int(options.height), int(options.width)
        shape = (max(len(names), 1), H, W, 4)
        if out is not None and not isinstance(out, np.ndarray) and hasattr(out, "data_ptr"):
            import torch
            if out.dtype != torch.float32 or tuple(out.shape) != shape or not out.is_contiguous() or not out.is_cuda:
                raise ValueError("features: a contiguous float32 tensor %s on the GPU is expected" % (shape,))
            if out.device.index != self.device:
                raise ValueError("features: the tensor is on %s, the renderer on device %d" % (out.device, self.device))
            _check(self._L.tinsel_hip_render_features_device(self._h, C.byref(camera), C.byref(options), int(pass_begin), int(passes), mask,
                                                             out.data_ptr(), torch.cuda.current_stream(out.device).cuda_stream),
                   "tinsel_hip_render_features_device")
        else:
            if out is None:
                out = np.zeros(shape, np.float32)
            elif out.dtype != np.float32 or out.shape != shape or not out.flags.c_contiguous:
                raise ValueError("features: a C-contiguous float32 array %s is expected" % (shape,))
            _check(self._L.tinsel_hip_render_features(self._h, C.byref(camera), C.byref(options), int(pass_begin), int(passes), mask,
                                                      out.ctypes.data_as(C.c_void_p)), "tinsel_hip_render_features")
        return {n: out[k] for k, n in enumerate(names)}

    def light_groups(self, camera, options, pass_begin, passes, groups, env_group=None, out=None):
        table = np.ascontiguousarray(np.asarray(groups).reshape(-1), np.int32)
        env = -1 if env_group is None else int(env_group)
        if out is not None:
            G = int(out.shape[0])
        else:
            G = max(int(table.max()) if table.size else -1, env) + 1
        if table.size != self.num_primitives:
            raise ValueError("light_groups: groups has %d entries, the scene %d primitives" % (table.size, self.num_primitives))
        H, W = int(options.height), int(options.width)
        shape = (max(G, 1), H, W, 4)
        if _is_tensor(out):
            import torch
            if out.dtype != torch.float32 or tuple(out.shape) != shape or not out.is_contiguous() or not out.is_cuda:
                raise ValueError("light_groups: a contiguous float32 tensor %s on the GPU is expected" % (shape,))
            if out.device.index != self.device:
                raise ValueError("light_groups: the tensor is on %s, the renderer on device %d" % (out.device, self.device))
            _check(self._L.tinsel_hip_render_light_groups_device(self._h, C.byref(camera), C.byref(options), int(pass_begin), int(passes), G,
                                                                 _host_ptr(table), env, out.data_ptr(), torch.cuda.current_stream(out.device).cuda_stream),
                   "tinsel_hip_render_light_groups_device")
        else:
            if out is None:
                out = np.zeros(shape, np.float32)
            elif out.dtype != np.float32 or out.shape != shape or not out.flags.c_contiguous:
                raise ValueError("light_groups: a C-contiguous float32 array %s is expected" % (shape,))
            _check(self._L.tinsel_hip_render_light_groups(self._h, C.byref(camera), C.byref(options), int(pass_begin), int(passes), G,
                                                          _host_ptr(table), env, out.ctypes.data_as(C.c_void_p)), "tinsel_hip_render_light_groups")
        return out

    def id_mattes(self, camera, options, pass_begin=0, passes=1, slots=6, out=None):
        slots = int(slots)
        H, W = int(options.height), int(options.width)
        ishape, wshape = (max(slots, 0), H, W), (max(slots, 0) + 2, H, W)
        if out is not None and len(out) != 2:
            raise ValueError("id_mattes: out is a pair (ids, weights)")
        if out is not None and hasattr(out[0], "data_ptr") and not isinstance(out[0], np.ndarray):
            import torch
            ids, weights = out
            for t, dtype, shape in ((ids, torch.int32, ishape), (weights, torch.float32, wshape)):
                if not hasattr(t, "data_ptr") or t.dtype != dtype or tuple(t.shape) != shape or not t.is_contiguous() or not t.is_cuda:
                    raise ValueError("id_mattes: contiguous tensors int32 %s and float32 %s on the GPU are expected" % (ishape, wshape))
                if t.device.index != self.device:
                    raise ValueError("id_mattes: the tensor is on %s, the renderer on device %d" % (t.device, self.device))
            _check(self._L.tinsel_hip_render_id_mattes_device(self._h, C.byref(camera), C.byref(options), int(pass_begin), int(passes), slots,
                                                              ids.data_ptr(), weights.data_ptr(), torch.cuda.current_stream(ids.device).cuda_stream),
                   "tinsel_hip_render_id_mattes_device")
        else:
            if out is None:
                ids, weights = np.zeros(ishape, np.int32), np.zeros(wshape, np.float32)
            else:
                ids, weights = out
                for a, dtype, shape in ((ids, np.int32, ishape), (weights, np.float32, wshape)):
                    if not isinstance(a, np.ndarray) or a.dtype != dtype or a.shape != shape or not a.flags.c_contiguous:
                        raise ValueError("id_mattes: C-contiguous arrays int32 %s and float32 %s are expected" % (ishape, wshape))
            _check(self._L.tinsel_hip_render_id_mattes(self._h, C.byref(camera), C.byref(options), int(pass_begin), int(passes), slots,
                                                       ids.ctypes.data_as(C.c_void_p), weights.ctypes.data_as(C.c_void_p)), "tinsel_hip_render_id_mattes")
        return {"ids": ids, "weights": weights[:slots], "residual": weights[slots], "total": weights[slots + 1]}

    def _image_tensor(self, who, t, shape):
        import torch
# ... 418 lines not shown
```

Baseline: 6660 Msamples/s.

## Pair opposite infinite planes so one intersection test serves both

Detects always-hit planes whose normals are exact negations (as in Cornell box walls) and packs them into pair blocks in the plane table. A single dot product and denominator then serve both planes, and a sign test picks which one the ray can hit, so roughly half the per-plane divides are saved. A leftover single plane rides in each 8-slot block, and the loop falls back to the old 4-wide path if any lane sees both planes hittable. This adds host-side table layout logic and a tuning knob, and keeps the old layout when pairing is disabled or when the scene has several non-HBM meshes.

```diff
diff --git a/include/tinsel_hip.h b/include/tinsel_hip.h
--- a/include/tinsel_hip.h
+++ b/include/tinsel_hip.h
@@ -170,6 +170,7 @@
     int32_t walk_grid_mult;
     int32_t quads_in_scan;
     int32_t bounce_fit;
+    int32_t plane_pairs;
 } tinsel_hip_tuning;
 enum { TINSEL_ACCUMULATE_AUTO = 0, TINSEL_ACCUMULATE_TILED = 1, TINSEL_ACCUMULATE_WIDE = 2, TINSEL_ACCUMULATE_PIPED = 3, TINSEL_ACCUMULATE_FULL_WINDOW = 4 };
 
@@ -348,6 +349,8 @@
 int tinsel_hip_queue_counts(tinsel_hip* r, uint32_t* out, int max_bounces);
 int tinsel_hip_bounce_plan(tinsel_hip* r, uint32_t* out2);
 unsigned int tinsel_hip_scene_features(const tinsel_scene_desc* scene);
+int tinsel_hip_scene_plane_pairs(const tinsel_scene_desc* scene, int32_t* out_pairs, int capacity, int* out_singles);
+int tinsel_hip_plane_table(tinsel_hip* r, int* out2);
 int tinsel_hip_scene_slim(const tinsel_scene_desc* scene);
 enum { TINSEL_BOUNCE_MEDIA = 1, TINSEL_BOUNCE_PROBE = 2, TINSEL_BOUNCE_MOTION = 4, TINSEL_BOUNCE_MESH_WALK = 8, TINSEL_BOUNCE_SPHERE = 16,
        TINSEL_BOUNCE_TRANSMISSION = 32, TINSEL_BOUNCE_POOLS = 64, TINSEL_BOUNCE_SHARE = 128, TINSEL_BOUNCE_SORT = 256, TINSEL_BOUNCE_ROULETTE = 512 };
diff --git a/tinsel_amd/abi.py b/tinsel_amd/abi.py
--- a/tinsel_amd/abi.py
+++ b/tinsel_amd/abi.py
@@ -179,12 +179,12 @@
                 ("tail_split", C.c_int32), ("tail_share", C.c_float), ("tail_divide", C.c_int32),
                 ("shade_sorted", C.c_int32), ("overlap", C.c_int32), ("scene_walk", C.c_int32), ("swalk_lds", C.c_int32), ("accumulate", C.c_int32),
                 ("walk_block", C.c_int32), ("walk_single", C.c_int32), ("walk_lds_stack", C.c_int32), ("walk_refill_min", C.c_int32), ("walk_leaf_min", C.c_int32),
-                ("walk_grid_mult", C.c_int32), ("quads_in_scan", C.c_int32), ("bounce_fit", C.c_int32)]
+                ("walk_grid_mult", C.c_int32), ("quads_in_scan", C.c_int32), ("bounce_fit", C.c_int32), ("plane_pairs", C.c_int32)]
     CREATE_FIELDS = ("flat_scan", "lds_scene", "walk", "inline_max_tris", "walk_min_tris", "small_mesh_bytes", "arena_lds_limit")
     _DEFAULTS = dict(flat_scan=-1, lds_scene=-1, walk=-1, inline_max_tris=-1, walk_min_tris=-1, small_mesh_bytes=-1, arena_lds_limit=-1,
                      batch_paths=0, grid_mult=0, bounce_share=-1, repack=-1, tail_split=-1, tail_share=0.0, tail_divide=4,
                      shade_sorted=-1, overlap=-1, scene_walk=-1, swalk_lds=-1, accumulate=0,
-                     walk_block=0, walk_single=-1, walk_lds_stack=-1, walk_refill_min=0, walk_leaf_min=0, walk_grid_mult=0, quads_in_scan=-1, bounce_fit=-1)
+                     walk_block=0, walk_single=-1, walk_lds_stack=-1, walk_refill_min=0, walk_leaf_min=0, walk_grid_mult=0, quads_in_scan=-1, bounce_fit=-1, plane_pairs=-1)
 
     def __init__(self, **over):
         super().__init__()
diff --git a/tinsel_amd/csrc/tn_host_api.h b/tinsel_amd/csrc/tn_host_api.h
--- a/tinsel_amd/csrc/tn_host_api.h
+++ b/tinsel_amd/csrc/tn_host_api.h
@@ -739,6 +739,13 @@
         r->batchSlotsExplicit = false;
     }
     free_batch(r);
+    if (pairs_planes(r, was) != pairs_planes(r, t) && !r->planeTablePrims.empty())
+    {
+        SceneLevel lvl;
+        if (!build_scene_level(r->sceneBvhHost, r->primsHost, r->planeTablePrims, pairs_planes(r, t), lvl))
+            return fail("set_tuning: the scene level could not be derived again");
+        return upload_scene_level(r, lvl);
+    }
     return 0;
 }
 
@@ -853,6 +860,45 @@
         }
     }
     return f;
+}
+
+int tinsel_hip_scene_plane_pairs(const tinsel_scene_desc* scene, int32_t* out_pairs, int capacity, int* out_singles)
+{
+    if (out_singles)
+        *out_singles = 0;
+    if (!scene || !scene->primitives || !scene->bvh_nodes || capacity < 0)
+        return 0;
+    std::vector<int32_t> planes;
+    std::vector<float> eqs;
+    for (int n = 0; n < scene->num_bvh_nodes; ++n)
+    {
+        const tinsel_bvh_node& nd = scene->bvh_nodes[n];
+        if (!ref_is_leaf(nd) || nd.left_index >= (uint32_t)scene->num_primitives || scene->primitives[nd.left_index].type != TINSEL_GEOM_PLANE)
+            continue;
+        if (make_prim_box(nd).alwaysHit && std::find(planes.begin(), planes.end(), (int32_t)nd.left_index) == planes.end())
+            planes.push_back((int32_t)nd.left_index);
+    }
+    std::sort(planes.begin(), planes.end());
+    for (const int32_t k : planes)
+        eqs.insert(eqs.end(), scene->primitives[k].geo.plane.plane, scene->primitives[k].geo.plane.plane + 4);
+    const std::vector<std::pair<int, int>> pairs = pair_planes(eqs);
+    for (size_t q = 0; q < pairs.size() && out_pairs && (int)q < capacity; ++q)
+    {
+        out_pairs[2*q] = planes[(size_t)pairs[q].first];
+        out_pairs[2*q + 1] = planes[(size_t)pairs[q].second];
+    }
+    if (out_singles)
+        *out_singles = (int)planes.size() - 2*(int)pairs.size();
+    return (int)pairs.size();
+}
+
+int tinsel_hip_plane_table(tinsel_hip* r, int* out2)
+{
+    if (!r || !out2)
+        return fail("plane_table: bad arguments");
+    out2[0] = r->planePairs;
+    out2[1] = r->planeSingles;
+    return 0;
 }
 
 int tinsel_hip_scene_slim(const tinsel_scene_desc* scene)
diff --git a/tinsel_amd/csrc/tn_host_create.h b/tinsel_amd/csrc/tn_host_create.h
--- a/tinsel_amd/csrc/tn_host_create.h
+++ b/tinsel_amd/csrc/tn_host_create.h
@@ -201,7 +201,7 @@
 
 int SceneBuild::scene_level()
 {
-    if (!build_scene_level(std::vector<tinsel_bvh_node>(desc->bvh_nodes, desc->bvh_nodes + desc->num_bvh_nodes), prims, {}, lvl))
+    if (!build_scene_level(std::vector<tinsel_bvh_node>(desc->bvh_nodes, desc->bvh_nodes + desc->num_bvh_nodes), prims, {}, false, lvl))
         return fail("create: malformed scene BVH");
     const int need = lvl.bvh.maxLeafDepth + 1 + maxMeshNeed;
     r->stackNeed = pick_stack(need);
@@ -270,15 +270,14 @@
         for (int k = 0; k < P; ++k)
             if (prims[(size_t)k].type == kPrimPlane && lvl.boxes[(size_t)k].alwaysHit)
                 r->planeTablePrims.push_back(k);
-        mark_plane_table(lvl, prims, r->planeTablePrims);
-    }
-    std::vector<float> planeEq = lvl.planeEq;
-    std::vector<int32_t> planeIdx = r->planeTablePrims;
-    while (planeIdx.size() % 4)
-    {
-        planeEq.insert(planeEq.end(), { 0.0f, 0.0f, 0.0f, 0.0f });
-        planeIdx.push_back(0);
-    }
+        int meshPrimCount = 0;
+        for (int k = 0; k < P; ++k)
+            meshPrimCount += prims[(size_t)k].type == kPrimMesh ? 1 : 0;
+        r->pairablePlanes = !(meshPrimCount >= 2 && !anyMeshInHbm);
+        mark_plane_table(lvl, prims, r->planeTablePrims, pairs_planes(r, tune));
+    }
+    const std::vector<float>& planeEq = lvl.planeEq;
+    const std::vector<int32_t>& planeIdx = lvl.planeIdx;
     const size_t offBoxes = arena.add(lvl.boxes.data(), lvl.boxes.size());
     const size_t offPlaneEq = arena.add(planeEq.data(), planeEq.size());
     const size_t offPlaneIdx = arena.add(planeIdx.data(), planeIdx.size());
@@ -317,7 +316,6 @@
     sc.primBoxes = reinterpret_cast<const PrimBox*>(arenaDev + offBoxes);
     sc.planeEq = reinterpret_cast<const float4*>(arenaDev + offPlaneEq);
     sc.planeIdx = reinterpret_cast<const int32_t*>(arenaDev + offPlaneIdx);
-    sc.numPlanes = (int32_t)r->planeTablePrims.size();
     adopt_scene_level(r, lvl);
     r->arenaOffNodes = offNodes;
     r->arenaOffBoxes = offBoxes;
diff --git a/tinsel_amd/csrc/tn_host_scene.h b/tinsel_amd/csrc/tn_host_scene.h
--- a/tinsel_amd/csrc/tn_host_scene.h
+++ b/tinsel_amd/csrc/tn_host_scene.h
@@ -70,30 +70,111 @@
     ConvertedBvh bvh;
     std::vector<PrimBox> boxes;
     std::vector<float> planeEq;
+    std::vector<int32_t> planeIdx;
+    int32_t numPlanes = 0, planePairEnd = 0;
+    int planePairs = 0, planeSingles = 0;
     unsigned long long scanMask = 0;
     bool everyPrimHasALeaf = true;
 };
 
-void mark_plane_table(SceneLevel& lvl, const std::vector<Prim64>& prims, const std::vector<int32_t>& planeTable)
-{
-    lvl.planeEq.assign(planeTable.size()*4, 0.0f);
-    for (size_t t = 0; t < planeTable.size(); ++t)
-    {
-        const int32_t k = planeTable[t];
+bool plane_pair_ok(const float a[4], const float b[4])
+{
+    for (int c = 0; c < 4; ++c)
+        if (!std::isfinite(a[c]) || !std::isfinite(b[c]))
+            return false;
+    for (int c = 0; c < 3; ++c)
+    {
+        uint32_t ua, ub;
+        memcpy(&ua, &a[c], 4); memcpy(&ub, &b[c], 4);
+        if (ub != (ua ^ 0x80000000u) && !(a[c] == 0.0f && b[c] == 0.0f))
+            return false;
+    }
+    return true;
+}
+
+std::vector<std::pair<int, int>> pair_planes(const std::vector<float>& eqs)
+{
+    const int n = (int)(eqs.size()/4);
+    std::vector<char> used((size_t)n, 0);
+    std::vector<std::pair<int, int>> out;
+    for (int a = 0; a < n; ++a)
+        for (int b = a + 1; b < n && !used[(size_t)a]; ++b)
+            if (!used[(size_t)b] && plane_pair_ok(&eqs[(size_t)a*4], &eqs[(size_t)b*4]))
+            {
+                used[(size_t)a] = used[(size_t)b] = 1;
+                out.emplace_back(a, b);
+            }
+    return out;
+}
+
+int plane_table_slots(int pairs, int singles)
+{
+    const int blocks = (pairs + 1)/2, riders = std::min(blocks, singles);
+    return 8*blocks + (singles - riders + 3)/4*4;
+}
+
+void mark_plane_table(SceneLevel& lvl, const std::vector<Prim64>& prims, const std::vector<int32_t>& planeTable, bool pairPlanes)
+{
+    std::vector<int32_t> live;
+    std::vector<float> eqs;
+    for (const int32_t k : planeTable)
         if (lvl.boxes[(size_t)k].alwaysHit)
         {
             lvl.boxes[(size_t)k].alwaysHit = 2u;
             const Prim64& pp = prims[(size_t)k];
-            lvl.planeEq[t*4 + 0] = pp.g0; lvl.planeEq[t*4 + 1] = pp.g1; lvl.planeEq[t*4 + 2] = pp.g2; lvl.planeEq[t*4 + 3] = pp.g3;
-        }
-    }
+            live.push_back(k);
+            eqs.insert(eqs.end(), { pp.g0, pp.g1, pp.g2, pp.g3 });
+        }
+    std::vector<float> all;
+    for (const int32_t k : planeTable)
+        all.insert(all.end(), { prims[(size_t)k].g0, prims[(size_t)k].g1, prims[(size_t)k].g2, prims[(size_t)k].g3 });
+    const int allPairs = (int)pair_planes(all).size();
+    const size_t cap = (size_t)std::max(plane_table_slots(0, (int)planeTable.size()), plane_table_slots(allPairs, (int)planeTable.size() - 2*allPairs));
+    std::vector<std::pair<int, int>> pairs = pairPlanes ? pair_planes(eqs) : std::vector<std::pair<int, int>>();
+    while ((size_t)plane_table_slots((int)pairs.size(), (int)live.size() - 2*(int)pairs.size()) > cap)
+        pairs.pop_back();
+    std::vector<char> paired(live.size(), 0);
+    for (const auto& ab : pairs)
+        paired[(size_t)ab.first] = paired[(size_t)ab.second] = 1;
+    std::vector<int> singles;
+    for (size_t t = 0; t < live.size(); ++t)
+        if (!paired[t])
+            singles.push_back((int)t);
+
+    lvl.planeEq.assign(cap*4, 0.0f);
+    lvl.planeIdx.assign(cap, 0);
+    auto put = [&](size_t slot, int t) {
+        std::copy(eqs.begin() + (size_t)t*4, eqs.begin() + (size_t)t*4 + 4, lvl.planeEq.begin() + slot*4);
+        lvl.planeIdx[slot] = live[(size_t)t];
+    };
+    size_t slot = 0, nextSingle = 0;
+    for (size_t q = 0; q < pairs.size(); q += 2, slot += 8)
+    {
+        put(slot, pairs[q].first); put(slot + 1, pairs[q].second);
+        if (q + 1 < pairs.size())
+        {
+            put(slot + 2, pairs[q + 1].first); put(slot + 3, pairs[q + 1].second);
+        }
+        if (nextSingle < singles.size())
+            put(slot + 4, singles[nextSingle++]);
+        lvl.planeIdx[slot + 5] = lvl.planeIdx[slot] | (lvl.planeIdx[slot + 1] << 8) | (lvl.planeIdx[slot + 2] << 16) | (lvl.planeIdx[slot + 3] << 24);
+    }
+    lvl.planePairEnd = (int32_t)slot;
+    while (nextSingle < singles.size())
+        put(slot++, singles[nextSingle++]);
+    lvl.numPlanes = (int32_t)slot;
+    lvl.planePairs = (int)pairs.size();
+    lvl.planeSingles = (int)singles.size();
+
     lvl.scanMask = 0;
     for (size_t k = 0; k < lvl.boxes.size() && k < 64; ++k)
         if (lvl.boxes[k].alwaysHit != 2u)
             lvl.scanMask |= 1ull << k;
 }
 
-bool build_scene_level(std::vector<tinsel_bvh_node> tree, const std::vector<Prim64>& prims, const std::vector<int32_t>& planeTable, SceneLevel& out)
+bool pairs_planes(const tinsel_hip* r, const tinsel_hip_tuning& tune) { return tune.plane_pairs != 0 && r->pairablePlanes; }
+
+bool build_scene_level(std::vector<tinsel_bvh_node> tree, const std::vector<Prim64>& prims, const std::vector<int32_t>& planeTable, bool pairPlanes, SceneLevel& out)
 {
     const int P = (int)prims.size();
     if (!convert_bvh(tree.data(), (int)tree.size(), P, 0, out.bvh))
@@ -107,7 +188,7 @@
             seen[nd.left_index] = 1;
         }
     out.everyPrimHasALeaf = std::find(seen.begin(), seen.end(), 0) == seen.end();
-    mark_plane_table(out, prims, planeTable);
+    mark_plane_table(out, prims, planeTable, pairPlanes);
     out.tree = std::move(tree);
     return true;
 }
@@ -116,6 +197,10 @@
 {
     r->scene.root = lvl.bvh.root;
     r->scene.scanMask = lvl.scanMask;
+    r->scene.numPlanes = lvl.numPlanes;
+    r->scene.planePairEnd = lvl.planePairEnd;
+    r->planePairs = lvl.planePairs;
+    r->planeSingles = lvl.planeSingles;
     r->sceneStackNeed = lvl.bvh.maxLeafDepth + 1;
     r->sceneBvhHost = std::move(lvl.tree);
 }
@@ -127,7 +212,10 @@
         HIP_TRY(hipMemcpy(arenaDev + r->arenaOffNodes, lvl.bvh.nodes.data(), sizeof(Node64)*lvl.bvh.nodes.size(), hipMemcpyHostToDevice));
     HIP_TRY(hipMemcpy(arenaDev + r->arenaOffBoxes, lvl.boxes.data(), sizeof(PrimBox)*lvl.boxes.size(), hipMemcpyHostToDevice));
     if (!lvl.planeEq.empty())
+    {
         HIP_TRY(hipMemcpy(const_cast<float4*>(r->scene.planeEq), lvl.planeEq.data(), sizeof(float)*lvl.planeEq.size(), hipMemcpyHostToDevice));
+        HIP_TRY(hipMemcpy(const_cast<int32_t*>(r->scene.planeIdx), lvl.planeIdx.data(), sizeof(int32_t)*lvl.planeIdx.size(), hipMemcpyHostToDevice));
+    }
     adopt_scene_level(r, lvl);
     return 0;
 }
@@ -279,7 +367,7 @@
         }
     union_ancestors(tree);
     SceneLevel lvl;
-    if (!build_scene_level(std::move(tree), r->primsHost, r->planeTablePrims, lvl))
+    if (!build_scene_level(std::move(tree), r->primsHost, r->planeTablePrims, pairs_planes(r, r->tune), lvl))
         return fail("refit_mesh: the scene BVH could not be refitted");
     return upload_scene_level(r, lvl);
 }
@@ -365,7 +453,7 @@
     }
 
     SceneLevel lvl;
-    if (!build_scene_level(std::move(ref), r->primsHost, r->planeTablePrims, lvl))
+    if (!build_scene_level(std::move(ref), r->primsHost, r->planeTablePrims, pairs_planes(r, r->tune), lvl))
         return fail("rebuild_scene: malformed scene BVH");
     if ((int)lvl.bvh.nodes.size() != (P > 1 ? P - 1 : 0))
         return fail("rebuild_scene: the scene BVH must have one leaf per primitive");
diff --git a/tinsel_amd/csrc/tn_host_state.h b/tinsel_amd/csrc/tn_host_state.h
--- a/tinsel_amd/csrc/tn_host_state.h
+++ b/tinsel_amd/csrc/tn_host_state.h
@@ -14,7 +14,7 @@
     t.tail_divide = 4;
     t.accumulate = TINSEL_ACCUMULATE_AUTO;
     t.walk_block = 0;
-    t.walk_single = t.walk_lds_stack = t.quads_in_scan = t.bounce_fit = -1;
+    t.walk_single = t.walk_lds_stack = t.quads_in_scan = t.bounce_fit = t.plane_pairs = -1;
     t.walk_refill_min = t.walk_leaf_min = t.walk_grid_mult = 0;
     return t;
 }
@@ -54,6 +54,8 @@
     std::vector<tinsel_bvh_node> sceneBvhHost;
     size_t arenaOffNodes = 0, arenaOffBoxes = 0;
     std::vector<int32_t> planeTablePrims;
+    bool pairablePlanes = true;
+    int planePairs = 0, planeSingles = 0;
     int sceneStackNeed = 1;
     std::string prepRefused;
     bool sceneEnclosed = false;
diff --git a/tinsel_amd/csrc/tn_isect.h b/tinsel_amd/csrc/tn_isect.h
--- a/tinsel_amd/csrc/tn_isect.h
+++ b/tinsel_amd/csrc/tn_isect.h
@@ -1,6 +1,7 @@
 #pragma once
 
 #include "tn_scene.h"
+#include "tn_plane.h"
 
 namespace tn {
 
@@ -115,11 +116,7 @@
 
 TN_D bool ray_plane(V3 p, V3 dir, float px, float py, float pz, float pw, float& t)
 {
-    float d = px*dir.x + py*dir.y + pz*dir.z + pw*0.0f;
-    if (d == 0.0f)
-        return false;
-    t = -(px*p.x + py*p.y + pz*p.z + pw*1.0f)/d;
-    return t > 0.0f;
+    return ray_plane_eq(p.x, p.y, p.z, dir.x, dir.y, dir.z, px, py, pz, pw, t);
 }
 
 TN_D bool ray_tri(V3 p, V3 dir, V3 a, V3 b, V3 c, float& t, float& u, float& v, float& w, float& sign, V3& n)
@@ -461,6 +458,37 @@
                                  finite_bits(o.x) && finite_bits(o.y) && finite_bits(o.z));
     const int numPlanes = sc.numPlanes;
     int pk = 0;
+    auto accept_of_pair = [&](const PlanePair& pp, const ConstF4V& ea, const ConstF4V& eb, int ia, int ib) {
+        float t;
+        if (plane_pair_hit(pp, t))
+        {
+            if (fabsf(t - minT) <= 1e-5f*fabsf(t))
+                tie = true;
+            if (t < minT)
+            {
+                minT = t;
+                if (pp.b) { closest = ib; cn = V3(eb.x, eb.y, eb.z); }
+                else      { closest = ia; cn = V3(ea.x, ea.y, ea.z); }
+            }
+        }
+    };
+    typedef const __attribute__((address_space(4))) uint32_t* ConstU32;
+    constexpr bool kCompactSingles = SC::kFeatures != kFeatAll && SC::kDefer != 1;
+    const int pairEnd = SC::kDefer != 1 ? (kCompactSingles ? min(sc.planePairEnd, 8) : sc.planePairEnd) : 0;
+    for (; pk + 8 <= pairEnd; pk += 8)
+    {
+        const ConstF4V e0 = sc.kPlaneEq[pk], e1 = sc.kPlaneEq[pk + 1], e2 = sc.kPlaneEq[pk + 2], e3 = sc.kPlaneEq[pk + 3], e4 = sc.kPlaneEq[pk + 4];
+        const uint32_t idr = ((ConstU32)sc.kPlaneIdx)[pk + 4], ids = ((ConstU32)sc.kPlaneIdx)[pk + 5];
+        const PlanePair p0 = plane_pair_pick(o.x, o.y, o.z, d.x, d.y, d.z, e0.x, e0.y, e0.z, e0.w, e1.w);
+        const PlanePair p1 = plane_pair_pick(o.x, o.y, o.z, d.x, d.y, d.z, e2.x, e2.y, e2.z, e2.w, e3.w);
+        if (__any(p0.both || p1.both))
+            break;
+        float t4;
+        const bool h4 = ray_plane(o, d, e4.x, e4.y, e4.z, e4.w, t4);
+        accept_of_pair(p0, e0, e1, (int)(ids & 255u), (int)((ids >> 8) & 255u));
+        accept_of_pair(p1, e2, e3, (int)((ids >> 16) & 255u), (int)(ids >> 24));
+        if (h4) accept((int)idr, t4, V3(e4.x, e4.y, e4.z));
+    }
     for (; pk + 4 <= numPlanes; pk += 4)
     {
         const ConstF4V e0 = sc.kPlaneEq[pk], e1 = sc.kPlaneEq[pk + 1], e2 = sc.kPlaneEq[pk + 2], e3 = sc.kPlaneEq[pk + 3];
@@ -475,7 +503,18 @@
         if (h2) accept(__float_as_int(id.z), t2, V3(e2.x, e2.y, e2.z));
         if (h3) accept(__float_as_int(id.w), t3, V3(e3.x, e3.y, e3.z));
     }
-    if (pk < numPlanes)
+    if constexpr (kCompactSingles)
+    {
+        for (; pk < numPlanes; ++pk)
+        {
+            const ConstF4V e0 = sc.kPlaneEq[pk];
+            const uint32_t id = ((ConstU32)sc.kPlaneIdx)[pk];
+            float t0;
+            if (ray_plane(o, d, e0.x, e0.y, e0.z, e0.w, t0))
+                accept((int)id, t0, V3(e0.x, e0.y, e0.z));
+        }
+    }
+    else if (pk < numPlanes)
     {
         const ConstF4V id = sc.kPlaneIdx[pk >> 2];
         const int left = numPlanes - pk;
diff --git a/tinsel_amd/csrc/tn_plane.h b/tinsel_amd/csrc/tn_plane.h
--- /dev/null
+++ b/tinsel_amd/csrc/tn_plane.h
@@ -0,0 +1,53 @@
+#pragma once
+
+#include <stdint.h>
+#include <string.h>
+
+#ifndef TN_HD
+#define TN_HD inline
+#endif
+
+namespace tn {
+
+TN_HD uint32_t plane_bits(float f) { uint32_t u; memcpy(&u, &f, 4); return u; }
+
+TN_HD bool ray_plane_eq(float ox, float oy, float oz, float dx, float dy, float dz, float px, float py, float pz, float pw, float& t)
+{
+    float d = px*dx + py*dy + pz*dz + pw*0.0f;
+    if (d == 0.0f)
+        return false;
+    t = -(px*ox + py*oy + pz*oz + pw*1.0f)/d;
+    return t > 0.0f;
+}
+
+struct PlanePair
+{
+    float den;
+    float q;
+    bool b;
+    bool both;
+};
+
+TN_HD PlanePair plane_pair_pick(float ox, float oy, float oz, float dx, float dy, float dz, float ax, float ay, float az, float aw, float bw)
+{
+    PlanePair r;
+    r.den = ax*dx + ay*dy + az*dz + aw*0.0f;
+    const float S = ax*ox + ay*oy + az*oz;
+    const float qa = -(S + aw*1.0f);
+    const float qb = -S + bw*1.0f;
+    const uint32_t sd = plane_bits(r.den), xa = plane_bits(qa) ^ sd, xb = plane_bits(qb) ^ sd;
+    r.both = (int32_t)(xa | xb) >= 0;
+    r.b = (int32_t)xb >= 0;
+    r.q = r.b ? qb : qa;
+    return r;
+}
+
+TN_HD bool plane_pair_hit(const PlanePair& r, float& t)
+{
+    if (r.den == 0.0f)
+        return false;
+    t = r.q/r.den;
+    return t > 0.0f;
+}
+
+}
diff --git a/tinsel_amd/csrc/tn_scene.h b/tinsel_amd/csrc/tn_scene.h
--- a/tinsel_amd/csrc/tn_scene.h
+++ b/tinsel_amd/csrc/tn_scene.h
@@ -159,6 +159,7 @@
     const float4* planeEq;
     const int32_t* planeIdx;
     int32_t numPlanes;
+    int32_t planePairEnd;
     unsigned long long scanMask;
 };
 
diff --git a/tinsel_amd/renderer.py b/tinsel_amd/renderer.py
--- a/tinsel_amd/renderer.py
+++ b/tinsel_amd/renderer.py
@@ -121,6 +121,9 @@
         L.tinsel_hip_scene_features.argtypes = [C.POINTER(abi.SceneDesc)]
     if hasattr(L, "tinsel_hip_scene_slim"):
         L.tinsel_hip_scene_slim.argtypes = [C.POINTER(abi.SceneDesc)]
+    if hasattr(L, "tinsel_hip_scene_plane_pairs"):
+        L.tinsel_hip_scene_plane_pairs.argtypes = [C.POINTER(abi.SceneDesc), C.POINTER(C.c_int32), C.c_int, C.POINTER(C.c_int)]
+        L.tinsel_hip_plane_table.argtypes = [vp, C.POINTER(C.c_int)]
     if hasattr(L, "tinsel_hip_queue_counts"):
         L.tinsel_hip_queue_counts.argtypes = [vp, C.POINTER(C.c_uint32), C.c_int]
     L.tinsel_hip_set_lookahead.argtypes = [vp, ci]
@@ -158,7 +161,7 @@
 
 
 EXPORTED_SYMBOLS = [
-    "tinsel_hip_bounce_plan", "tinsel_hip_scene_features", "tinsel_hip_scene_slim", "tinsel_hip_create", "tinsel_hip_destroy", "tinsel_hip_init", "tinsel_hip_init_external", "tinsel_hip_render",
+    "tinsel_hip_bounce_plan", "tinsel_hip_scene_features", "tinsel_hip_scene_slim", "tinsel_hip_scene_plane_pairs", "tinsel_hip_plane_table", "tinsel_hip_create", "tinsel_hip_destroy", "tinsel_hip_init", "tinsel_hip_init_external", "tinsel_hip_render",
     "tinsel_hip_render_async", "tinsel_hip_accum_device_ptr", "tinsel_hip_read_accum", "tinsel_hip_set_shard",
     "tinsel_hip_set_pipeline", "tinsel_hip_set_pass_index", "tinsel_hip_get_pass_index", "tinsel_hip_stats",
     "tinsel_hip_reset_stats", "tinsel_hip_stats_detail", "tinsel_hip_set_detail_counters", "tinsel_hip_render_cost", "tinsel_hip_kernel_times", "tinsel_hip_kernel_time_bytes",
@@ -453,6 +456,13 @@
 
     def bounce_slim(self):
         return bool(load_library().tinsel_hip_scene_slim(C.byref(self.desc)))
+
+    def plane_pairs(self):
+        n = max(1, self.num_primitives//2)
+        out = (C.c_int32*(2*n))()
+        singles = C.c_int(0)
+        k = load_library().tinsel_hip_scene_plane_pairs(C.byref(self.desc), out, n, C.byref(singles))
+        return [(out[2*q], out[2*q + 1]) for q in range(k)], singles.value
 
 
 def _bytes_at(ptr, n):
@@ -612,6 +622,11 @@
     def set_tuning(self, tuning=None, **fields):
         t = (tuning if tuning is not None else self.get_tuning()).replace(**fields)
         _check(self._L.tinsel_hip_set_tuning(self._h, C.byref(t)), "tinsel_hip_set_tuning")
+
+    def plane_table(self):
+        out = (C.c_int*2)()
+        _check(self._L.tinsel_hip_plane_table(self._h, out), "tinsel_hip_plane_table")
+        return out[0], out[1]
 
     def get_tuning(self):
         t = abi.Tuning()
```

New measurement: 6903 Msamples/s, median of 6. 1.04x the previous value.
